# johncai117/Meta-Fine-Tuning

Measured on AMD Instinct MI355X. Metric: episodes/sec at 5-way N-shot (ResNet10+GNN) per GPU and 1/2/4/8-GPU node, higher is better.
Workload: dtype f32

## Files before the change

include/mft_hip.h:

```cpp
#ifndef MFT_HIP_H
#define MFT_HIP_H

#ifdef __cplusplus
extern "C" {
#endif

#define MFT_EINVAL (-22)

enum { MFT_ACT_NONE = 0, MFT_ACT_RELU = 1, MFT_ACT_LRELU = 2 };
enum { MFT_BN_AFFINE_FMA = 0x100 };

int mft_version(void);
int mft_device_info(int* cu_count, int* gcn_arch_is_gfx950);

int mft_stream_create_cumask(const unsigned* mask_words, int n_words, void** stream_out);
int mft_stream_create_priority(int priority, void** stream_out, int* range_out);
int mft_stream_destroy(void* stream);
int mft_stream_probe(float* w, float* m, float* v, long long n, void* stream);
int mft_event_create(void** event_out);
int mft_event_record(void* event, void* stream);
int mft_event_elapsed_ms(void* start, void* stop, float* ms_out);
int mft_event_destroy(void* event);
int mft_probe_placement(unsigned* out, int n_blocks, int spin_cycles, void* stream);

int mft_augment_views(const unsigned char* src, int n_img, int Hs, int Ws, const float* params, int n_views, float* out,
                      long long view_stride, long long img_stride, int size, const float* mean3, const float* std3,
                      void* stream);

int mft_nchw_to_nhwc(const float* src, float* dst, int n_img, int C, int H, int W, void* stream);

long long mft_conv2d_wgrad_adam_dgrad_ws_floats(int n_img, int H, int W, int Cin);
int mft_conv2d_wgrad_adam_dgrad_nhwc(const float* x, int ldx, const float* dy, int ldy, float* w, float* m, float* v,
                                     float* dx_partials, int n_img, int H, int W, int Cin, int Cout, int imgs_per_group,
                                     long long group_stride, int step, float lr, float beta1, float beta2, float eps, void* stream);
int mft_conv2d_wgrad_adam_dgrad_nhwc_dev(const float* x, int ldx, const float* dy, int ldy, float* w, float* m, float* v,
                                         float* dx_partials, int n_img, int H, int W, int Cin, int Cout, int imgs_per_group,
                                         long long group_stride, const float* hyper, float beta1, float beta2, float eps,
                                         void* stream);
int mft_col2im_bn_backward_small(const float* dx_partials, const float* x_raw, const float* relu_out, float* dx, int n_img, int H,
                                 int W, int C, int imgs_per_group, const float* mean, const float* rstd, const float* gamma,
                                 long long gb_group_stride, float* dgamma, float* dbeta, void* stream);

int mft_ce_pool_bn_backward2(const float* feat, const int* labels, int imgs_per_group, int n_groups, int C, int hw,
                             const float* out, const float* xa, const float* xb, float* dxa, float* dxb, const float* mean_a,
                             const float* rstd_a, const float* gamma_a, const float* mean_b, const float* rstd_b,
                             const float* gamma_b, long long gb_group_stride, float* dgamma_a, float* dbeta_a, float* dgamma_b,
                             float* dbeta_b, float* loss, void* stream);

int mft_stem_cache_fill(const float* in, const float* w, int w_ld, int n_img, int H, int W, float* pmax, float* pmin,
                        float* mean_img, float* m2_img, void* stream);
int mft_pool_window_minmax(const float* x, float* ymax, float* ymin, long long n_img, int H, int W, int C, void* stream);
int mft_bn_relu_pooled_gather(const float* pmax, const float* pmin, const int* src_idx, float* y, int n_img, int OH, int OW, int C,
                              int imgs_per_group, const float* mean, const float* rstd, const float* gamma, const float* beta,
                              void* stream);

int mft_bn_apply_planes(const float* x, int ldx, float* y, int ldy, unsigned short* planes, long long plane_stride, int C,
                        int rows_per_group, int n_groups, const float* mean, const float* rstd, const float* gamma,
                        const float* beta, long long gb_group_stride, const float* res, int ldr, const float* res_mean,
                        const float* res_rstd, const float* res_gamma, const float* res_beta, int act, float slope,
                        void* stream);
int mft_bn_relu_maxpool_gather_planes(const float* x, const int* src_idx, float* y, unsigned short* planes,
                                      long long plane_stride, int n_img, int H, int W, int C, int imgs_per_group,
                                      const float* mean, const float* rstd, const float* gamma, const float* beta, void* stream);
int mft_conv2d_nhwc_x3p_bnstats(const unsigned short* in_planes, long long in_plane_elems, int ldi, const unsigned short* w3,
                                long long plane_elems, float* out, int ldo, int n_img, int H, int W, int Cin, int Cout, int KH,
                                int KW, int stride, int pad, int imgs_per_group, float eps, float* stats_ws, float* mean,
                                float* rstd, void* stream);

int mft_ingest_episode_views(const float* const* views, int n_views, int double_first, int n_way, int per_class, int n_support,
                             int C, int H, int W, float* support_store, float* all_store, void* stream);
int mft_pack_oihw(const float* w_oihw, float* w_pk, int Cout, int Cin, int KH, int KW, int k_pad, void* stream);
int mft_pack_oihw_multi(const void* jobs, int n_jobs, long long total_elements, void* stream);
int mft_unpack_oihw(const float* w_pk, float* w_oihw, int Cout, int Cin, int KH, int KW, int k_pad, void* stream);
int mft_pack_dgrad(const float* w_pk, float* wt_pk, int Cout, int Cin, int KH, int KW,
                   int groups, long long w_stride, long long wt_stride, void* stream);

int mft_conv2d_nhwc(const float* in, int ldi, const float* w, const float* bias, float* out, int ldo,
                    int n_img, int H, int W, int Cin, int Cout, int KH, int KW, int stride, int pad,
                    int imgs_per_group, long long w_group_stride, void* stream);

int mft_split_bf16x3(const float* w, unsigned short* planes, long long n, void* stream);
int mft_split_bf16x3_multi(const void* jobs, int n_jobs, long long total_elements, void* stream);
int mft_conv2d_nhwc_x3(const float* in, int ldi, const unsigned short* w3, long long plane_elems, float* out, int ldo,
                       int n_img, int H, int W, int Cin, int Cout, int KH, int KW, int stride, int pad, void* stream);
long long mft_conv2d_x3_stats_ws_floats(int n_img, int H, int W, int Cout, int KH, int KW, int stride, int pad);
int mft_conv2d_nhwc_x3_bnstats(const float* in, int ldi, const unsigned short* w3, long long plane_elems, float* out, int ldo,
                               int n_img, int H, int W, int Cin, int Cout, int KH, int KW, int stride, int pad,
                               int imgs_per_group, float eps, float* stats_ws, float* mean, float* rstd, void* stream);
int mft_conv2d_nhwc_x3_bnin_bnstats(const float* in, int ldi, const float* in_ws, const float* in_gamma, const float* in_beta,
                                    const unsigned short* w3, long long plane_elems, float* out, int ldo, int n_img, int H, int W,
                                    int Cin, int Cout, int imgs_per_group, float eps, float* stats_ws, float* mean, float* rstd,
                                    void* stream);
int mft_split_f16x2(const float* w, unsigned short* planes, long long n, void* stream);
int mft_conv2d_nhwc_h2(const float* in, int ldi, const unsigned short* w2, long long plane_elems, float* out, int ldo,
                       int n_img, int H, int W, int Cin, int Cout, int KH, int KW, int stride, int pad, void* stream);
int mft_conv2d_nhwc_h2_bnstats(const float* in, int ldi, const unsigned short* w2, long long plane_elems, float* out, int ldo,
                               int n_img, int H, int W, int Cin, int Cout, int KH, int KW, int stride, int pad,
                               int imgs_per_group, float eps, float* stats_ws, float* mean, float* rstd, void* stream);
int mft_conv2d_nhwc_h2_bnin_bnstats(const float* in, int ldi, const float* in_ws, const float* in_gamma, const float* in_beta,
                                    const unsigned short* w2, long long plane_elems, float* out, int ldo, int n_img, int H, int W,
                                    int Cin, int Cout, int imgs_per_group, float eps, float* stats_ws, float* mean, float* rstd,
                                    void* stream);
int mft_bn_apply_x3ws(const float* x, int ldx, float* y, int ldy, int C, int rows_per_group, int n_groups, const float* ws,
                      const float* gamma, const float* beta, const float* res, int ldr, const float* res_ws,
                      const float* res_gamma, const float* res_beta, int act, float slope, float eps, float* mean, float* rstd,
                      float* res_mean, float* res_rstd, void* stream);
int mft_bn_running_ema(const float* mean_a, const float* rstd_a, int rows_a, const float* mean_b, const float* rstd_b, int rows_b,
                       const int* order, int n_steps, int C, float eps, float momentum, float* running_mean, float* running_var,
                       void* stream);
int mft_bn_apply_x3ws_fits(int C, int rows_per_group, int with_res_bn);
int mft_bn_relu_pooled_gather_moments(const float* pmax, const float* pmin, const int* src_idx, float* y, int n_img, int OH, int OW,
                                      int C, int imgs_per_group, const float* mean_img, const float* m2_img, int rows_per_img,
                                      float eps, const float* gamma, const float* beta, float* mean, float* rstd, void* stream);

int mft_has_experiments(void);

int mft_conv2d_dgrad_nhwc(const float* dy, int ldy, const float* w, float* dx, int ldx,
                          int n_img, int H, int W, int Cin, int Cout, int KH, int KW, int stride, int pad,
                          int imgs_per_group, long long w_group_stride, void* stream);

long long mft_conv_ksplit_ws_floats(long long rows, int cols, int K);
long long mft_conv_ksplit_grouped_ws_floats(long long rows_per_group, int cols, int K, int groups);
int mft_conv2d_nhwc_ksplit_grouped(const float* in, int ldi, const float* w, float* out, int ldo, int n_img, int H, int W, int Cin,
                                   int Cout, int KH, int KW, int stride, int pad, int imgs_per_group, long long w_group_stride,
                                   float* ws, void* stream);
int mft_conv2d_dgrad_nhwc_ksplit_grouped(const float* dy, int ldy, const float* w, float* dx, int ldx, int n_img, int H, int W, int Cin,
                                         int Cout, int KH, int KW, int stride, int pad, int imgs_per_group, long long w_group_stride,
                                         float* ws, void* stream);
int mft_conv2d_nhwc_ksplit(const float* in, int ldi, const float* w, const float* bias, float* out, int ldo, int n_img, int H, int W,
                           int Cin, int Cout, int KH, int KW, int stride, int pad, float* ws, void* stream);
int mft_conv2d_dgrad_nhwc_ksplit(const float* dy, int ldy, const float* w, float* dx, int ldx, int n_img, int H, int W, int Cin,
                                 int Cout, int KH, int KW, int stride, int pad, float* ws, void* stream);
long long mft_conv2d_wgrad_ws_floats(int n_img, int H, int W, int Cin, int Cout, int KH, int KW, int stride, int pad,
                                     int imgs_per_group);
int mft_conv2d_wgrad_nhwc(const float* in, int ldi, const float* dy, int ldy, float* dw,
                          int n_img, int H, int W, int Cin, int Cout, int KH, int KW, int stride, int pad,
                          int imgs_per_group, long long dw_group_stride, float* ws, void* stream);

long long mft_conv2d_wgrad_oihw_ws_floats(int n_img, int H, int W, int Cin, int Cout, int KH, int KW, int stride, int pad);
int mft_conv2d_wgrad_oihw(const float* in, int ldi, const float* dy, int ldy, float* dw_oihw, int n_img, int H, int W, int Cin,
                          int Cout, int KH, int KW, int stride, int pad, int cin_valid, int cout_valid, float* ws, void* stream);

typedef struct MftWgradJob {
    const float* in; const float* dy; float* dw_oihw; float* ws;
    int ldi, ldy, n_img, H, W, Cin, Cout, KH, KW, stride, pad, cin_valid, cout_valid, reserved;
} MftWgradJob;
int mft_conv2d_wgrad_oihw_multi(const MftWgradJob* jobs, int n_jobs, void* stream);

int mft_conv2d_wgrad_adam_nhwc(const float* in, int ldi, const float* dy, int ldy, float* w, float* m, float* v,
                               float* dw_or_null, int n_img, int H, int W, int Cin, int Cout, int KH, int KW,
                               int stride, int pad, int imgs_per_group, long long group_stride,
                               int step, float lr, float beta1, float beta2, float eps, void* stream);

int mft_wgrad_adam_next_forward(const float* x, int ldx, const float* dy, int ldy, float* w, float* m, float* v,
                                float* dw_or_null, int n_img, int H, int W, int Cin, int Cout, int KH, int KW, int stride,
                                int pad, int imgs_per_group, long long group_stride, int step, const float* hyper, float lr,
                                float beta1, float beta2, float eps, const float* x_next, int mode, float* raw, float* act,
                                const float* gamma, const float* beta, long long gb_group_stride, float* mean, float* rstd,
                                const float* sc_raw, const float* gamma_s, const float* beta_s, float* mean_s, float* rstd_s,
                                float* pooled, float bn_eps, void* stream);


long long mft_bn_stats_ws_floats(int C, int rows_per_group, int n_groups);
int mft_bn_stats(const float* x, int ldx, int C, int rows_per_group, int n_groups, float eps,
                 float* mean, float* rstd, float* ws,
                 float* running_mean, float* running_var, float momentum, long long* num_batches_tracked, void* stream);
typedef struct MftBnStatsJob {
    const float* x; float* mean; float* rstd; float* ws; float* running_mean; float* running_var; long long* num_batches_tracked;
    int ldx, C, rows_per_group, n_groups; float eps, momentum;
} MftBnStatsJob;
int mft_bn_stats_multi(const MftBnStatsJob* jobs, int n_jobs, void* stream);
typedef struct MftBnFwdJob {
    const float* x; float* y; const float* gamma; const float* beta; float* mean; float* rstd;
    float* running_mean; float* running_var; long long* num_batches_tracked;
    const float* res; const float* res_gamma; const float* res_beta; float* res_mean; float* res_rstd;
    float* res_running_mean; float* res_running_var; long long* res_num_batches_tracked;
    int ldx, ldy, ldr, C, rows_per_group, n_groups, act; float eps, momentum, slope;
} MftBnFwdJob;
int mft_bn_forward_small(const MftBnFwdJob* job, void* stream);
int mft_bn_forward_small_max_rows(void);
typedef struct MftBnApplyJob {
    const float* x; float* y; const float* mean; const float* rstd; const float* gamma; const float* beta;
    int ldx, ldy, C, rows_per_group, n_groups, act; float slope; int reserved;
} MftBnApplyJob;
int mft_bn_apply_multi(const MftBnApplyJob* jobs, int n_jobs, void* stream);
// ... 175 lines not shown
```

meta-fine-tuning_amd/_lib.py:

```python
import ctypes
import os

PKG = os.path.dirname(os.path.abspath(__file__))
LIB_PATH = os.path.join(PKG, "libmft_hip.so")

_P = ctypes.c_void_p
_I = ctypes.c_int
_L = ctypes.c_longlong
_F = ctypes.c_float

SIGNATURES = {
    "mft_version": [],
    "mft_device_info": [_P, _P],
    "mft_stream_create_cumask": [_P, _I, _P],
    "mft_stream_destroy": [_P],
    "mft_stream_probe": [_P, _P, _P, _L, _P],
    "mft_probe_placement": [_P, _I, _I, _P],
    "mft_event_create": [_P],
    "mft_event_record": [_P, _P],
    "mft_event_elapsed_ms": [_P, _P, _P],
    "mft_event_destroy": [_P],
    "mft_augment_views": [_P, _I, _I, _I, _P, _I, _P, _L, _L, _I, _P, _P, _P],
    "mft_nchw_to_nhwc": [_P, _P, _I, _I, _I, _I, _P],
    "mft_pack_oihw": [_P, _P, _I, _I, _I, _I, _I, _P],
    "mft_unpack_oihw": [_P, _P, _I, _I, _I, _I, _I, _P],
    "mft_pack_dgrad": [_P, _P, _I, _I, _I, _I, _I, _L, _L, _P],
    "mft_conv2d_nhwc": [_P, _I, _P, _P, _P, _I, _I, _I, _I, _I, _I, _I, _I, _I, _I, _I, _L, _P],
    "mft_has_experiments": [],
    "mft_split_bf16x3": [_P, _P, _L, _P],
    "mft_split_bf16x3_multi": [_P, _I, _L, _P],
    "mft_conv2d_nhwc_x3": [_P, _I, _P, _L, _P, _I, _I, _I, _I, _I, _I, _I, _I, _I, _I, _P],
    "mft_conv2d_x3_stats_ws_floats": [_I, _I, _I, _I, _I, _I, _I, _I],
    "mft_conv2d_nhwc_x3_bnstats": [_P, _I, _P, _L, _P, _I, _I, _I, _I, _I, _I, _I, _I, _I, _I, _I, _F, _P, _P, _P, _P],
    "mft_conv2d_dgrad_nhwc": [_P, _I, _P, _P, _I, _I, _I, _I, _I, _I, _I, _I, _I, _I, _I, _L, _P],
    "mft_conv_ksplit_ws_floats": [_L, _I, _I],
    "mft_conv_ksplit_grouped_ws_floats": [_L, _I, _I, _I],
    "mft_conv2d_nhwc_ksplit_grouped": [_P, _I, _P, _P, _I, _I, _I, _I, _I, _I, _I, _I, _I, _I, _I, _L, _P, _P],
    "mft_conv2d_dgrad_nhwc_ksplit_grouped": [_P, _I, _P, _P, _I, _I, _I, _I, _I, _I, _I, _I, _I, _I, _I, _L, _P, _P],
    "mft_conv2d_nhwc_ksplit": [_P, _I, _P, _P, _P, _I, _I, _I, _I, _I, _I, _I, _I, _I, _I, _P, _P],
    "mft_conv2d_dgrad_nhwc_ksplit": [_P, _I, _P, _P, _I, _I, _I, _I, _I, _I, _I, _I, _I, _I, _P, _P],
    "mft_conv2d_wgrad_oihw_ws_floats": [_I, _I, _I, _I, _I, _I, _I, _I, _I],
    "mft_conv2d_wgrad_oihw": [_P, _I, _P, _I, _P, _I, _I, _I, _I, _I, _I, _I, _I, _I, _I, _I, _P, _P],
    "mft_conv2d_wgrad_oihw_multi": [_P, _I, _P],
    "mft_conv2d_wgrad_ws_floats": [_I, _I, _I, _I, _I, _I, _I, _I, _I, _I],
    "mft_conv2d_wgrad_nhwc": [_P, _I, _P, _I, _P, _I, _I, _I, _I, _I, _I, _I, _I, _I, _I, _L, _P, _P],
    "mft_conv2d_wgrad_adam_nhwc": [_P, _I, _P, _I, _P, _P, _P, _P, _I, _I, _I, _I, _I, _I, _I, _I, _I, _I, _L, _I, _F, _F, _F,
                                   _F, _P],
    "mft_pair_softmax_ut_backward": [_P, _P, _P, _P, _P, _I, _I, _I, _P, _P],
    "mft_pair_bwd_stats_ws_floats": [_L, _I],
    "mft_pair_bn_act_backward": [_P, _I, _P, _I, _P, _P, _P, _P, _P, _P, _I, _L, _I, _L, _F, _P, _P, _P, _P, _P, _P],
    "mft_pair_absdiff_ut": [_P, _I, _P, _P, _I, _I, _I, _L, _L, _P],
    "mft_pair_dx_gather": [_P, _I, _P, _I, _P, _I, _I, _I, _I, _L, _L, _P],
    "mft_pack_oihw_multi": [_P, _I, _L, _P],
    "mft_wgrad_adam_next_forward": [_P, _I, _P, _I, _P, _P, _P, _P, _I, _I, _I, _I, _I, _I, _I, _I, _I, _I, _L, _I, _P, _F, _F, _F,
                                    _F, _P, _I, _P, _P, _P, _P, _L, _P, _P, _P, _P, _P, _P, _P, _P, _F, _P],
    "mft_bn_stats_ws_floats": [_I, _I, _I],
    "mft_bn_stats": [_P, _I, _I, _I, _I, _F, _P, _P, _P, _P, _P, _F, _P, _P],
    "mft_bn_apply": [_P, _I, _P, _I, _I, _I, _I, _P, _P, _P, _P, _L, _P, _I, _P, _P, _P, _P, _I, _F, _P],
    "mft_bn_apply_multi": [_P, _I, _P],
    "mft_bn_stats_multi": [_P, _I, _P],
    "mft_bn_relu_maxpool": [_P, _P, _I, _I, _I, _I, _I, _P, _P, _P, _P, _P],
    "mft_bn_relu_maxpool_gather": [_P, _P, _P, _I, _I, _I, _I, _I, _P, _P, _P, _P, _P],
    "mft_bn_image_moments": [_P, _I, _I, _I, _L, _P, _P, _P],
    "mft_bn_combine_moments": [_P, _P, _P, _I, _I, _I, _I, _F, _P, _P, _P],
    "mft_global_avgpool": [_P, _P, _I, _I, _I, _P],
    "mft_bn_small_forward": [_P, _I, _P, _I, _P, _I, _P, _I, _I, _I, _I, _P, _P, _P, _P, _L, _P, _P, _P, _P, _I, _F, _F, _P, _I, _P],
    "mft_bn_backward2": [_P, _P, _I, _P, _I, _P, _P, _I, _I, _I, _I, _P, _P, _P, _P, _P, _P, _L, _P, _P, _P, _P, _P],
    "mft_ce_pool_backward": [_P, _P, _I, _I, _I, _I, _P, _P, _P, _P],
    "mft_bn_backward": [_P, _I, _P, _I, _P, _I, _P, _I, _I, _I, _I, _P, _P, _P, _L, _P, _P, _P],
    "mft_avgpool_relu_backward": [_P, _P, _P, _I, _I, _I, _P],
    "mft_cross_entropy": [_P, _I, _P, _I, _I, _I, _P, _P, _P],
    "mft_softmax_rows": [_P, _I, _P, _I, _I, _I, _P],
    "mft_proto_scores": [_P, _I, _I, _I, _I, _I, _I, _P, _I, _P],
    "mft_proto_backward": [_P, _I, _I, _I, _I, _I, _I, _P, _I, _P, _I, _P],
    "mft_cross_entropy_mean": [_P, _I, _P, _I, _I, _I, _P, _P, _P],
    "mft_cross_entropy_mean_backward": [_P, _I, _P, _I, _I, _I, _P, _P, _I, _P],
    "mft_adam_step": [_P, _P, _P, _P, _L, _I, _F, _F, _F, _F, _F, _P],
    "mft_sgd_step": [_P, _P, _P, _L, _I, _F, _F, _F, _F, _P],
    "mft_maml_delta": [_P, _P, _P, _L, _P],
    "mft_conv2d_wgrad_adam_dgrad_ws_floats": [_I, _I, _I, _I],
    "mft_conv2d_wgrad_adam_dgrad_nhwc": [_P, _I, _P, _I, _P, _P, _P, _P, _I, _I, _I, _I, _I, _I, _L, _I, _F, _F, _F, _F, _P],
    "mft_conv2d_wgrad_adam_dgrad_nhwc_dev": [_P, _I, _P, _I, _P, _P, _P, _P, _I, _I, _I, _I, _I, _I, _L, _P, _F, _F, _F, _P],
    "mft_col2im_bn_backward_small": [_P, _P, _P, _P, _I, _I, _I, _I, _I, _P, _P, _P, _L, _P, _P, _P],
    "mft_stream_create_priority": [_I, _P, _P],
    "mft_ce_pool_bn_backward2": [_P, _P, _I, _I, _I, _I, _P, _P, _P, _P, _P, _P, _P, _P, _P, _P, _P, _L, _P, _P, _P, _P, _P, _P],
    "mft_pool_window_minmax": [_P, _P, _P, _L, _I, _I, _I, _P],
    "mft_stem_cache_fill": [_P, _P, _I, _I, _I, _I, _P, _P, _P, _P, _P],
    "mft_conv2d_nhwc_x3_bnin_bnstats": [_P, _I, _P, _P, _P, _P, _L, _P, _I, _I, _I, _I, _I, _I, _I, _F, _P, _P, _P, _P],
    "mft_split_f16x2": [_P, _P, _L, _P],
    "mft_conv2d_nhwc_h2": [_P, _I, _P, _L, _P, _I, _I, _I, _I, _I, _I, _I, _I, _I, _I, _P],
    "mft_conv2d_nhwc_h2_bnstats": [_P, _I, _P, _L, _P, _I, _I, _I, _I, _I, _I, _I, _I, _I, _I, _I, _F, _P, _P, _P, _P],
    "mft_conv2d_nhwc_h2_bnin_bnstats": [_P, _I, _P, _P, _P, _P, _L, _P, _I, _I, _I, _I, _I, _I, _I, _F, _P, _P, _P, _P],
    "mft_bn_apply_x3ws": [_P, _I, _P, _I, _I, _I, _I, _P, _P, _P, _P, _I, _P, _P, _P, _I, _F, _F, _P, _P, _P, _P, _P],
    "mft_bn_apply_x3ws_fits": [_I, _I, _I],
    "mft_bn_running_ema": [_P, _P, _I, _P, _P, _I, _P, _I, _I, _F, _F, _P, _P, _P],
    "mft_bn_relu_pooled_gather_moments": [_P, _P, _P, _P, _I, _I, _I, _I, _I, _P, _P, _I, _F, _P, _P, _P, _P, _P],
    "mft_bn_relu_pooled_gather": [_P, _P, _P, _P, _I, _I, _I, _I, _I, _P, _P, _P, _P, _P],
    "mft_bn_apply_planes": [_P, _I, _P, _I, _P, _L, _I, _I, _I, _P, _P, _P, _P, _L, _P, _I, _P, _P, _P, _P, _I, _F, _P],
    "mft_bn_relu_maxpool_gather_planes": [_P, _P, _P, _P, _L, _I, _I, _I, _I, _I, _P, _P, _P, _P, _P],
    "mft_conv2d_nhwc_x3p_bnstats": [_P, _L, _I, _P, _L, _P, _I, _I, _I, _I, _I, _I, _I, _I, _I, _I, _I, _F, _P, _P, _P, _P],
    "mft_ingest_episode_views": [_P, _I, _I, _I, _I, _I, _I, _I, _I, _P, _P, _P],
    "mft_block_entry_small_forward": [_P, _I, _P, _L, _P, _L, _P, _P, _P, _I, _I, _I, _I, _I, _I, _I, _P, _P, _L, _P, _P, _F, _P],
    "mft_block_exit_small_forward": [_P, _P, _L, _P, _P, _P, _P, _I, _I, _I, _I, _I, _P, _P, _P, _P, _L, _P, _P, _P, _P, _F, _P],
    "mft_conv2d_dgrad_bn_backward_small": [_P, _I, _P, _P, _I, _I, _I, _I, _I, _I, _I, _I, _I, _I, _L, _P, _P, _P, _P, _P, _L,
                                           _P, _P, _P],
    "mft_linear_head_sgd_run": [_P, _P, _P, _I, _I, _I, _I, _I, _I, _P, _P, _F, _F, _F, _F, _P],
    "mft_linear_head_adam_run": [_P, _P, _P, _I, _I, _I, _I, _I, _I, _P, _P, _F, _F, _F, _F, _F, _P],
    "mft_adam_multi": [_P, _I, _I, _F, _F, _F, _F, _F, _F, _P],
    "mft_adam_hyper_advance": [_P, _P, _F, _F, _F, _P],
    "mft_adam_step_dev": [_P, _P, _P, _P, _L, _P, _F, _F, _F, _F, _P],
    "mft_conv2d_wgrad_adam_nhwc_dev": [_P, _I, _P, _I, _P, _P, _P, _P, _I, _I, _I, _I, _I, _I, _I, _I, _I, _I, _L, _P, _F, _F,
                                       _F, _P],
    "mft_linear_head_step": [_P, _I, _P, _I, _I, _I, _I, _P, _P, _P, _P, _P, _P, _P, _I, _P, _I, _F, _F, _F, _F, _F, _P],
    "mft_linear_head_scores": [_P, _I, _I, _I, _I, _I, _P, _P, _P, _P],
    "mft_pair_absdiff": [_P, _I, _P, _I, _I, _I, _I, _P],
    "mft_masked_softmax": [_P, _I, _P, _I, _I, _P],
    "mft_pair_mlp_tiles_m": [_I, _I],
    "mft_pair_mlp_layer": [_P, _I, _I, _P, _P, _P, _P, _I, _I, _P, _P, _I, _I, _I, _I, _F, _P, _P, _P, _I, _P],
    "mft_bn_forward_small": [_P, _P],
    "mft_bn_forward_small_max_rows": [],
    "mft_gemm_rk": [_P, _I, _P, _I, _I, _P, _P, _I, _I, _I, _P],
    "mft_pair_mlp_tiles_m_rk": [_I, _I],
    "mft_pair_mlp_layer_rk": [_P, _I, _I, _P, _P, _P, _P, _I, _I, _P, _P, _I, _I, _I, _I, _F, _P, _P, _P, _P],
    "mft_pair_mlp_stats_finalize_rk": [_P, _P, _P, _I, _I, _I, _P, _P, _F, _P, _P, _P, _P, _P],
    "mft_pair_mlp_stats_finalize": [_P, _P, _P, _I, _I, _I, _P, _P, _F, _P, _P, _P, _P, _P],
    "mft_pair_mlp_score": [_P, _I, _P, _P, _P, _P, _F, _P, _I, _I, _I, _P],
    "mft_masked_softmax_ut": [_P, _P, _I, _I, _P],
    "mft_graph_aggregate": [_P, _P, _I, _P, _I, _I, _I, _I, _P],
    "mft_copy_cols": [_P, _I, _P, _I, _I, _I, _I, _I, _F, _P],
    "mft_build_graph_nodes": [_P, _I, _P, _I, _I, _I, _I, _I, _I, _P],
    "mft_gather_query_scores": [_P, _I, _P, _I, _I, _I, _I, _P],
    "mft_gather_rows": [_P, _P, _P, _I, _L, _P],
    "mft_var_to_rstd": [_P, _P, _I, _F, _P],
    "mft_bn_backward_ws_floats": [_I, _I, _I],
    "mft_bn_backward_act": [_P, _I, _P, _I, _P, _I, _P, _I, _I, _I, _I, _P, _P, _P, _L, _P, _P, _I, _F, _P, _P, _P, _P, _P],
    "mft_bn_backward_act_multi": [_P, _I, _P],
    "mft_act_backward": [_P, _I, _P, _I, _P, _I, _I, _L, _I, _F, _I, _P],
    "mft_colsum": [_P, _I, _I, _L, _P, _P, _P],
    "mft_bn_relu_maxpool_arg": [_P, _P, _P, _I, _I, _I, _I, _I, _P, _P, _P, _P, _P],
    "mft_maxpool_relu_backward": [_P, _P, _P, _P, _I, _I, _I, _I, _P],
    "mft_masked_softmax_backward": [_P, _P, _P, _I, _I, _I, _P],
    "mft_pair_absdiff_backward": [_P, _I, _P, _I, _P, _I, _I, _I, _I, _P],
    "mft_graph_aggregate_backward": [_P, _P, _I, _P, _I, _P, _I, _P, _I, _I, _I, _I, _P],
    "mft_build_graph_nodes_backward": [_P, _I, _P, _I, _I, _I, _I, _I, _I, _P],
    "mft_gather_query_scores_backward": [_P, _P, _I, _I, _I, _I, _I, _P, _P],
}
TESTING_SIGNATURES = {
    "mft_debug_set_conv_tile": [_I],
    "mft_debug_set_x3_tile": [_I],
    "mft_debug_reset": [],
    "mft_wgrad_fwd_set_exact": [_I],
    "mft_wgrad_fwd_set_xcd": [_I],
}
_RESTYPE = {"mft_conv2d_x3_stats_ws_floats": _L, "mft_bn_stats_ws_floats": _L, "mft_conv2d_wgrad_ws_floats": _L, "mft_bn_backward_ws_floats": _L,
            "mft_conv2d_wgrad_adam_dgrad_ws_floats": _L, "mft_pair_bwd_stats_ws_floats": _L, "mft_conv_ksplit_ws_floats": _L, "mft_conv2d_wgrad_oihw_ws_floats": _L, "mft_conv_ksplit_grouped_ws_floats": _L}

_lib = None


def lib():
    global _lib
    if _lib is None:
        if not os.path.exists(LIB_PATH):
            raise RuntimeError(
                "libmft_hip.so not found at %s -- build it with `python -c 'import __graft_entry__ as g; g.build()'`; "
                "this package has no CPU or PyTorch fallback" % LIB_PATH)
        import torch
        if torch.cuda.is_available():
            torch.cuda.init()
            torch.empty(1, device="cuda")
        h = ctypes.CDLL(LIB_PATH)
        for name, argtypes in list(SIGNATURES.items()) + list(TESTING_SIGNATURES.items()):
            fn = getattr(h, name)
# ... 87 lines not shown
```

meta-fine-tuning_amd/csrc/bn.hip:

```cpp
#include "mft_common.h"
#include "bn_fold.h"

namespace {

constexpr int ST_ROWS = 16;

__device__ __forceinline__ void bn_stats_partial_body(const float* __restrict__ x, int ldx, int C,
                                                      int rows_per_group, int rows_per_chunk, int chunks,
                                                      float* __restrict__ ws, const int bx, const int by, const int bz) {
    const int cq = threadIdx.x & 15;
    const int rl = threadIdx.x >> 4;
    const int c = by * 64 + cq * 4;
    const int g = bz;
    const int chunk = bx;
    const long long row0 = (long long)g * rows_per_group;
    __shared__ f32x4 red1[ST_ROWS][16];
    __shared__ f32x4 red2[ST_ROWS][16];
    f32x4 s1 = {0.f, 0.f, 0.f, 0.f}, s2 = {0.f, 0.f, 0.f, 0.f};
    if (c < C) {
        const f32x4 sh = *(const f32x4*)(x + row0 * ldx + c);
        const int rbeg = chunk * rows_per_chunk;
        const int rend = min(rbeg + rows_per_chunk, rows_per_group);
#pragma unroll 4
        for (int rr = rbeg + rl; rr < rend; rr += ST_ROWS) {
// ... 369 lines not shown
            if (p.ro) {
                const f32x4 o = *(const f32x4*)(p.ro + (row0 + rr) * p.ldro + c);
#pragma unroll
                for (int e = 0; e < 4; ++e) d[e] = o[e] > 0.f ? d[e] : 0.f;
            }
            const f32x4 xh = (*(const f32x4*)(p.x + (row0 + rr) * p.ldx + c) - mu) * rs;
            s1 += d;
            s2 += d * xh;
        }
    }
    red1[rl][cq] = s1;
    red2[rl][cq] = s2;
    __syncthreads();
    s1 = red1[0][cq];
    s2 = red2[0][cq];
#pragma unroll
    for (int k = 1; k < ST_ROWS; ++k) {
        s1 += red1[k][cq];
        s2 += red2[k][cq];
    }
    if (!ok) return;
    if (rl == 0) {
        if (p.dgamma) *(f32x4*)(p.dgamma + (long long)g * p.C + c) = s2;
        if (p.dbeta) *(f32x4*)(p.dbeta + (long long)g * p.C + c) = s1;
    }
    if (!p.dx) return;
    const float inv = 1.f / (float)p.rows_per_group;
    const f32x4 m1 = s1 * inv, m2 = s2 * inv;
    const f32x4 k = ga * rs;
    for (int rr = rl; rr < p.rows_per_group; rr += ST_ROWS) {
        f32x4 d = *(const f32x4*)(p.dy + (row0 + rr) * p.lddy + c);
        if (p.ro) {
            const f32x4 o = *(const f32x4*)(p.ro + (row0 + rr) * p.ldro + c);
#pragma unroll
            for (int e = 0; e < 4; ++e) d[e] = o[e] > 0.f ? d[e] : 0.f;
        }
        const f32x4 xh = (*(const f32x4*)(p.x + (row0 + rr) * p.ldx + c) - mu) * rs;
        *(f32x4*)(p.dx + (row0 + rr) * p.lddx + c) = k * (d - m1 - xh * m2);
    }
}

__global__ __launch_bounds__(256) void bn_image_moments_kernel(const float* __restrict__ x, int ldx, int C, int rows,
                                                               float* __restrict__ mean_img,
                                                               float* __restrict__ m2_img) {
    const int cq = threadIdx.x & 15;
    const int rl = threadIdx.x >> 4;
    const int c = blockIdx.y * 64 + cq * 4;
    const long long img = blockIdx.x;
    const long long row0 = img * rows;
    __shared__ f32x4 red1[ST_ROWS][16];
    __shared__ f32x4 red2[ST_ROWS][16];
    f32x4 s1 = {0.f, 0.f, 0.f, 0.f}, s2 = {0.f, 0.f, 0.f, 0.f}, sh = s1;
    if (c < C) {
        sh = *(const f32x4*)(x + row0 * ldx + c);
        for (int rr = rl; rr < rows; rr += ST_ROWS) {
            f32x4 v = *(const f32x4*)(x + (row0 + rr) * ldx + c);
            v -= sh;
            s1 += v;
            s2 += v * v;
        }
    }
    red1[rl][cq] = s1;
    red2[rl][cq] = s2;
    __syncthreads();
    if (rl == 0 && c < C) {
#pragma unroll
        for (int k = 1; k < ST_ROWS; ++k) {
            s1 += red1[k][cq];
            s2 += red2[k][cq];
        }
        const float inv = 1.f / (float)rows;
        f32x4 mu, m2;
#pragma unroll
        for (int e = 0; e < 4; ++e) {
            const float d = s1[e] * inv;
            mu[e] = sh[e] + d;
            m2[e] = fmaxf(s2[e] - s1[e] * d, 0.f);
        }
        *(f32x4*)(mean_img + img * C + c) = mu;
        *(f32x4*)(m2_img + img * C + c) = m2;
    }
}

template <class MeanOf, class M2Of>
__device__ __forceinline__ void combine_moments_impl(MeanOf mean_of, M2Of m2_of, int rows_per_img, int imgs_per_group, float eps,
                                                     float& mean, float& rstd) {
    float mu = 0.f;
    for (int i = 0; i < imgs_per_group; ++i) mu += mean_of(i);
    mu /= (float)imgs_per_group;
    float m2 = 0.f, dev = 0.f;
    for (int i = 0; i < imgs_per_group; ++i) {
        const float d = mean_of(i) - mu;
        m2 += m2_of(i);
        dev += d * d;
    }
    const float var = (m2 + (float)rows_per_img * dev) / ((float)rows_per_img * (float)imgs_per_group);
    mean = mu;
    rstd = 1.0f / sqrtf(var + eps);
}

__device__ __forceinline__ void combine_moments(const float* __restrict__ mean_img, const float* __restrict__ m2_img,
                                                const int* __restrict__ id, int C, int c, int rows_per_img, int imgs_per_group,
                                                float eps, float& mean, float& rstd) {
    combine_moments_impl([&](int i) { return mean_img[(long long)id[i] * C + c]; },
                         [&](int i) { return m2_img[(long long)id[i] * C + c]; }, rows_per_img, imgs_per_group, eps, mean, rstd);
}

__device__ __forceinline__ void combine_moments_lds(const float* smean, const float* sm2, int C, int c, int rows_per_img,
                                                    int imgs_per_group, float eps, float& mean, float& rstd) {
    combine_moments_impl([&](int i) { return smean[i * C + c]; }, [&](int i) { return sm2[i * C + c]; }, rows_per_img,
                         imgs_per_group, eps, mean, rstd);
}

__global__ void bn_combine_moments_kernel(const float* __restrict__ mean_img, const float* __restrict__ m2_img,
                                          const int* __restrict__ idx, int C, int rows_per_img, int imgs_per_group,
                                          float eps, float* __restrict__ mean, float* __restrict__ rstd) {
    const int c = blockIdx.x * blockDim.x + threadIdx.x;
    const int g = blockIdx.y;
    if (c >= C) return;
    float mu, rs;
    combine_moments(mean_img, m2_img, idx + (long long)g * imgs_per_group, C, c, rows_per_img, imgs_per_group, eps, mu, rs);
    mean[(long long)g * C + c] = mu;
    rstd[(long long)g * C + c] = rs;
}

inline int grid_for(long long total, int block = 256, int cap = 256 * 8) {
    long long b = (total + block - 1) / block;
    if (b < 1) b = 1;
    if (b > cap) b = cap;
    return (int)b;
}

inline int stats_chunks(int rows_per_group, int n_groups, int C) {
    const int tiles = (C + 63) / 64;
    long long want = (1024 + (long long)n_groups * tiles - 1) / ((long long)n_groups * tiles);
    int maxc = (rows_per_group + 63) / 64;
    if (want > maxc) want = maxc;
    if (want < 1) want = 1;
    return (int)want;
}

struct BnFwdSmallArgs {
    const float* x; float* y; const float* gamma; const float* beta; float* mean; float* rstd;
    float* running_mean; float* running_var; long long* nbt;
    const float* res; const float* rgamma; const float* rbeta; float* rmean; float* rrstd;
    float* rrunning_mean; float* rrunning_var; long long* rnbt;
    int ldx, ldy, ldr, C, rows_per_group, n_groups, act;
    float eps, momentum, slope;
    int y_scalar;
};

__device__ __forceinline__ void bn_small_block_sum(f32x4& a, f32x4& b, float (*red)[8]) {
    const int lane = threadIdx.x & 63, wave = threadIdx.x >> 6;
#pragma unroll
    for (int off = 32; off > 0; off >>= 1)
#pragma unroll
        for (int e = 0; e < 4; ++e) {
            a[e] += __shfl_xor(a[e], off, 64);
            b[e] += __shfl_xor(b[e], off, 64);
        }
    if (lane == 0) {
#pragma unroll
        for (int e = 0; e < 4; ++e) { red[wave][e] = a[e]; red[wave][4 + e] = b[e]; }
    }
    __syncthreads();
#pragma unroll
    for (int e = 0; e < 4; ++e) {
        a[e] = ((red[0][e] + red[1][e]) + red[2][e]) + red[3][e];
        b[e] = ((red[0][4 + e] + red[1][4 + e]) + red[2][4 + e]) + red[3][4 + e];
    }
}

__device__ __forceinline__ void bn_small_finish(const f32x4 s1, const f32x4 s2, const f32x4 pivot, int rows, float eps, f32x4& mu,
                                                f32x4& rs, f32x4& var) {
    const float inv = 1.f / (float)rows;
#pragma unroll
    for (int e = 0; e < 4; ++e) {
        const float d = s1[e] * inv;
        mu[e] = pivot[e] + d;
        var[e] = fmaxf(s2[e] * inv - d * d, 0.f);
        rs[e] = 1.0f / sqrtf(var[e] + eps);
    }
}

__global__ __launch_bounds__(256) void bn_forward_small_kernel(BnFwdSmallArgs p) {
    __shared__ float red[2][4][8];
    const int c = blockIdx.x * 4, g = blockIdx.y, t = threadIdx.x;
    const long long row0 = (long long)g * p.rows_per_group;
    const bool rbn = p.res != nullptr && p.rgamma != nullptr;
    const f32x4 zero4 = {0.f, 0.f, 0.f, 0.f};
    const f32x4 pv = *(const f32x4*)(p.x + row0 * p.ldx + c);
    const f32x4 pr = rbn ? *(const f32x4*)(p.res + row0 * p.ldr + c) : zero4;
    f32x4 s1 = zero4, s2 = zero4, q1 = zero4, q2 = zero4;
    if (rbn) {
// ... 199 lines not shown
                                      const int* __restrict__ order, int n_steps, int C, float eps, float momentum,
                                      float* __restrict__ running_mean, float* __restrict__ running_var) {
    const int c = blockIdx.x * blockDim.x + threadIdx.x;
    if (c >= C) return;
    float rm = running_mean[c], rv = running_var[c];
    for (int t = 0; t < n_steps; ++t) {
        const int o = order[t], g = o & 0xffffff;
        const bool b = (o >> 24) != 0;
        const float m = (b ? mean_b : mean_a)[(long long)g * C + c];
        const float rs = (b ? rstd_b : rstd_a)[(long long)g * C + c];
        const float var = fmaxf(1.0f / (rs * rs) - eps, 0.f);
        rm = (1.f - momentum) * rm + momentum * m;
        rv = (1.f - momentum) * rv + momentum * (var * (b ? unb_b : unb_a));
    }
    running_mean[c] = rm;
    running_var[c] = rv;
}
}

extern "C" int mft_bn_running_ema(const float* mean_a, const float* rstd_a, int rows_a, const float* mean_b, const float* rstd_b,
                                  int rows_b, const int* order, int n_steps, int C, float eps, float momentum, float* running_mean,
                                  float* running_var, void* stream) {
    if (!mean_a || !rstd_a || rows_a < 1 || !order || n_steps < 1 || C < 1 || !running_mean || !running_var) return MFT_EINVAL;
    const float ua = (float)rows_a / (float)(rows_a > 1 ? rows_a - 1 : 1);
    const float ub = (float)rows_b / (float)(rows_b > 1 ? rows_b - 1 : 1);
    hipLaunchKernelGGL(bn_running_ema_kernel, dim3((C + 63) / 64), dim3(64), 0, (hipStream_t)stream, mean_a, rstd_a, ua, mean_b, rstd_b, ub,
                       order, n_steps, C, eps, momentum, running_mean, running_var);
    return mft_launch_status();
}

extern "C" int mft_bn_apply_x3ws_fits(int C, int rows_per_group, int with_res_bn) {
    if (C % 4 != 0 || C > 1024 || rows_per_group < 128) return 0;
    return (size_t)4 * C * sizeof(float) + (with_res_bn ? 2 : 1) * mft_x3_stage_bytes_host(mft_x3_max_group_tiles(rows_per_group, 128), C) <=
           64 * 1024;
}

extern "C" int mft_bn_apply_planes(const float* x, int ldx, float* y, int ldy, unsigned short* planes, long long plane_stride,
                                   int C, int rows_per_group, int n_groups, const float* mean, const float* rstd,
                                   const float* gamma, const float* beta, long long gb_group_stride, const float* res, int ldr,
                                   const float* res_mean, const float* res_rstd, const float* res_gamma,
                                   const float* res_beta, int act, float slope, void* stream) {
    if (C % 4 != 0 || ldx % 4 != 0 || (y && ldy % 4 != 0) || (res && ldr % 4 != 0) || !planes) return MFT_EINVAL;
    if (plane_stride < (long long)n_groups * rows_per_group * C) return MFT_EINVAL;
    ApplyArgs p{x, y, ldx, ldy, C, rows_per_group, n_groups, mean, rstd, gamma, beta, gb_group_stride,
                res, ldr, res_mean, res_rstd, res_gamma, res_beta, act, slope, planes, plane_stride};
    const long long total = (long long)n_groups * rows_per_group * (C / 4);
    hipLaunchKernelGGL(bn_apply_kernel<true>, dim3(grid_for(total)), dim3(256), 0, (hipStream_t)stream, p);
    return mft_launch_status();
}

namespace {
__global__ __launch_bounds__(256) void pool_window_minmax_kernel(const float* __restrict__ x, float* __restrict__ ymax,
                                                                 float* __restrict__ ymin, long long n_img, int H, int W, int C,
                                                                 int OH, int OW) {
    const int cq = C >> 2;
    const long long total = n_img * OH * OW * cq;
    for (long long i = (long long)blockIdx.x * blockDim.x + threadIdx.x; i < total; i += (long long)gridDim.x * blockDim.x) {
        const int c = (int)(i % cq) * 4;
        long long t = i / cq;
        const int ow = (int)(t % OW); t /= OW;
        const int oh = (int)(t % OH);
        const long long n = t / OH;
        f32x4 hi = {-3.4e38f, -3.4e38f, -3.4e38f, -3.4e38f}, lo = {3.4e38f, 3.4e38f, 3.4e38f, 3.4e38f};
#pragma unroll
        for (int dh = 0; dh < 3; ++dh) {
            const int ih = oh * 2 - 1 + dh;
            if (ih < 0 || ih >= H) continue;
#pragma unroll
            for (int dw = 0; dw < 3; ++dw) {
                const int iw = ow * 2 - 1 + dw;
                if (iw < 0 || iw >= W) continue;
                const f32x4 v = *(const f32x4*)(x + ((n * H + ih) * W + iw) * C + c);
#pragma unroll
                for (int e = 0; e < 4; ++e) { hi[e] = fmaxf(hi[e], v[e]); lo[e] = fminf(lo[e], v[e]); }
            }
        }
        *(f32x4*)(ymax + i * 4) = hi;
        *(f32x4*)(ymin + i * 4) = lo;
    }
}

__device__ __forceinline__ f32x4 pooled_bn_relu(const float* __restrict__ pmax, const float* __restrict__ pmin, long long src,
                                                const f32x4 mu, const f32x4 rs, const f32x4 ga, const f32x4 be) {
    const bool all_pos = ga[0] >= 0.f && ga[1] >= 0.f && ga[2] >= 0.f && ga[3] >= 0.f;
    const bool all_neg = ga[0] < 0.f && ga[1] < 0.f && ga[2] < 0.f && ga[3] < 0.f;
    f32x4 v;
    if (all_pos) v = *(const f32x4*)(pmax + src);
    else if (all_neg) v = *(const f32x4*)(pmin + src);
    else {
        const f32x4 a = *(const f32x4*)(pmax + src), b = *(const f32x4*)(pmin + src);
#pragma unroll
        for (int e = 0; e < 4; ++e) v[e] = ga[e] >= 0.f ? a[e] : b[e];
    }
    f32x4 o = __builtin_elementwise_fma((v - mu) * rs, ga, be);
#pragma unroll
    for (int e = 0; e < 4; ++e) o[e] = fmaxf(o[e], 0.f);
    return o;
}

__global__ __launch_bounds__(256) void bn_relu_pooled_gather_kernel(const float* __restrict__ pmax, const float* __restrict__ pmin,
                                                                    const int* __restrict__ src_idx, float* __restrict__ y,
                                                                    int n_img, int HW, int C, int imgs_per_group,
                                                                    const float* __restrict__ mean, const float* __restrict__ rstd,
                                                                    const float* __restrict__ gamma, const float* __restrict__ beta) {
    const int cq = C >> 2;
    const long long total = (long long)n_img * HW * cq;
    for (long long i = (long long)blockIdx.x * blockDim.x + threadIdx.x; i < total; i += (long long)gridDim.x * blockDim.x) {
        const int c = (int)(i % cq) * 4;
        const long long t = i / cq;
        const int pix = (int)(t % HW);
        const int n = (int)(t / HW);
        const int g = n / imgs_per_group;
        const long long src = ((long long)src_idx[n] * HW + pix) * C + c;
        const f32x4 mu = *(const f32x4*)(mean + (long long)g * C + c);
        const f32x4 rs = *(const f32x4*)(rstd + (long long)g * C + c);
        *(f32x4*)(y + i * 4) = pooled_bn_relu(pmax, pmin, src, mu, rs, *(const f32x4*)(gamma + c), *(const f32x4*)(beta + c));
    }
}

__global__ __launch_bounds__(256) void bn_relu_pooled_gather_moments_kernel(
    const float* __restrict__ pmax, const float* __restrict__ pmin, const int* __restrict__ src_idx, float* __restrict__ y, int HW,
    int C, int imgs_per_group, const float* __restrict__ mean_img, const float* __restrict__ m2_img, int rows_per_img, float eps,
    const float* __restrict__ gamma, const float* __restrict__ beta, float* __restrict__ mean, float* __restrict__ rstd) {
    extern __shared__ __attribute__((aligned(16))) float tab[];
    const int g = blockIdx.y;
    const int* id = src_idx + (long long)g * imgs_per_group;
    float* smean = tab + 2 * C;
    float* sm2 = smean + imgs_per_group * C;
    for (int i = threadIdx.x; i < imgs_per_group * C; i += 256) {
        const int im = i / C, c = i - im * C;
        const long long src = (long long)id[im] * C + c;
        smean[i] = mean_img[src];
        sm2[i] = m2_img[src];
    }
    __syncthreads();
    for (int c = threadIdx.x; c < C; c += 256) {
        float mu, rs;
        combine_moments_lds(smean, sm2, C, c, rows_per_img, imgs_per_group, eps, mu, rs);
        tab[c] = mu; tab[C + c] = rs;
        if (blockIdx.x == 0 && mean) { mean[(long long)g * C + c] = mu; rstd[(long long)g * C + c] = rs; }
    }
    __syncthreads();
    const int cq = C >> 2;
    const int total = imgs_per_group * HW * cq;
    for (int i = blockIdx.x * 256 + threadIdx.x; i < total; i += gridDim.x * 256) {
        const int c = (i % cq) * 4;
        const int t = i / cq;
        const int pix = t % HW;
        const int n = t / HW;
        const long long src = ((long long)id[n] * HW + pix) * C + c;
        const long long dst = ((long long)g * imgs_per_group * HW * cq + i) * 4;
        *(f32x4*)(y + dst) = pooled_bn_relu(pmax, pmin, src, *(const f32x4*)(tab + c), *(const f32x4*)(tab + C + c),
                                            *(const f32x4*)(gamma + c), *(const f32x4*)(beta + c));
    }
}
}

extern "C" int mft_pool_window_minmax(const float* x, float* ymax, float* ymin, long long n_img, int H, int W, int C, void* stream) {
    if (C % 4 != 0 || n_img <= 0) return MFT_EINVAL;
    const int OH = (H + 2 - 3) / 2 + 1, OW = (W + 2 - 3) / 2 + 1;
    const long long total = n_img * OH * OW * (C / 4);
    hipLaunchKernelGGL(pool_window_minmax_kernel, dim3(grid_for(total, 256, 256 * 16)), dim3(256), 0, (hipStream_t)stream, x, ymax,
                       ymin, n_img, H, W, C, OH, OW);
    return mft_launch_status();
}

extern "C" int mft_bn_relu_pooled_gather(const float* pmax, const float* pmin, const int* src_idx, float* y, int n_img, int OH,
                                         int OW, int C, int imgs_per_group, const float* mean, const float* rstd,
                                         const float* gamma, const float* beta, void* stream) {
    if (C % 4 != 0 || !src_idx) return MFT_EINVAL;
    if (imgs_per_group <= 0) imgs_per_group = n_img;
    const long long total = (long long)n_img * OH * OW * (C / 4);
    hipLaunchKernelGGL(bn_relu_pooled_gather_kernel, dim3(grid_for(total, 256, 256 * 16)), dim3(256), 0, (hipStream_t)stream, pmax,
                       pmin, src_idx, y, n_img, OH * OW, C, imgs_per_group, mean, rstd, gamma, beta);
    return mft_launch_status();
}

extern "C" int mft_bn_relu_pooled_gather_moments(const float* pmax, const float* pmin, const int* src_idx, float* y, int n_img,
                                                 int OH, int OW, int C, int imgs_per_group, const float* mean_img,
                                                 const float* m2_img, int rows_per_img, float eps, const float* gamma,
                                                 const float* beta, float* mean, float* rstd, void* stream) {
    if (C % 4 != 0 || C > 1024 || !src_idx || imgs_per_group <= 0 || n_img % imgs_per_group != 0 || rows_per_img <= 0 ||
        (mean == nullptr) != (rstd == nullptr))
        return MFT_EINVAL;
    const int groups = n_img / imgs_per_group;
    const long long per_group = (long long)imgs_per_group * OH * OW * (C / 4);
    if (per_group > 0x7fffffffLL) return MFT_EINVAL;
    int sub = (int)((per_group + 256 * 16 - 1) / (256 * 16));
    const int cap = (2048 + groups - 1) / groups;
    if (sub > cap) sub = cap;
    if (sub < 1) sub = 1;
    const size_t lds = (size_t)(2 + 2 * imgs_per_group) * C * sizeof(float);
    if (lds > 64 * 1024) return MFT_EINVAL;
    hipLaunchKernelGGL(bn_relu_pooled_gather_moments_kernel, dim3(sub, groups), dim3(256), lds, (hipStream_t)stream,
                       pmax, pmin, src_idx, y, OH * OW, C, imgs_per_group, mean_img, m2_img, rows_per_img, eps, gamma, beta, mean,
                       rstd);
    return mft_launch_status();
}

extern "C" int mft_bn_relu_maxpool_gather_planes(const float* x, const int* src_idx, float* y, unsigned short* planes,
                                                 long long plane_stride, int n_img, int H, int W, int C, int imgs_per_group,
                                                 const float* mean, const float* rstd, const float* gamma, const float* beta,
                                                 void* stream) {
    if (C % 4 != 0) return MFT_EINVAL;
    if (imgs_per_group <= 0) imgs_per_group = n_img;
    const int OH = (H + 2 - 3) / 2 + 1, OW = (W + 2 - 3) / 2 + 1;
    const long long total = (long long)n_img * OH * OW * (C / 4);
    if (planes)
        hipLaunchKernelGGL(bn_relu_maxpool_kernel<true>, dim3(grid_for(total, 256, 256 * 16)), dim3(256), 0, (hipStream_t)stream,
                           x, y, n_img, H, W, C, OH, OW, imgs_per_group, mean, rstd, gamma, beta, src_idx, planes, plane_stride);
    else
        hipLaunchKernelGGL(bn_relu_maxpool_kernel<false>, dim3(grid_for(total, 256, 256 * 16)), dim3(256), 0, (hipStream_t)stream,
                           x, y, n_img, H, W, C, OH, OW, imgs_per_group, mean, rstd, gamma, beta, src_idx, planes, plane_stride);
    return mft_launch_status();
}

extern "C" int mft_bn_relu_maxpool_gather(const float* x, const int* src_idx, float* y, int n_img, int H, int W, int C,
                                          int imgs_per_group, const float* mean, const float* rstd, const float* gamma,
                                          const float* beta, void* stream) {
    return mft_bn_relu_maxpool_gather_planes(x, src_idx, y, nullptr, 0, n_img, H, W, C, imgs_per_group, mean, rstd, gamma, beta,
                                             stream);
// ... 347 lines not shown
```

meta-fine-tuning_amd/csrc/bn_fold.h:

```cpp
#pragma once
#include "mft_common.h"

typedef float mft_f32x2 __attribute__((ext_vector_type(2)));

struct MftTileSpan { int t0, t1; };
struct MftTileW { float inv_nt, w1, w2, pad; };

__device__ __forceinline__ MftTileSpan mft_x3_group_tiles(int g, int M, int R, int BM) {
    const int r0 = g * R, r1 = min(r0 + R, M);
    return {r0 / BM, (r1 - 1) / BM};
}

__device__ __forceinline__ int mft_x3_tile_seg(int t, int g, int R, int BM) { return ((t * BM) / R == g) ? 0 : 1; }

__device__ __forceinline__ MftTileW mft_x3_tile_weights(int t, int g, int M, int R, int BM) {
    const int r0 = g * R, r1 = min(r0 + R, M);
    const int lo = max(t * BM, r0), hi = min(t * BM + BM, r1);
    const float nt = (float)(hi - lo), n = (float)(lo - r0), tot = (float)(hi - r0);
    return {1.0f / nt, nt / tot, n * nt / tot, 0.f};
}

template <class Get, class Weights>
__device__ __forceinline__ void mft_x3_stats_chain(Get get, Weights weights, int g, int M, int R, int BM, float eps, float& mean,
                                                   float& rstd) {
    const int r0 = g * R, r1 = min(r0 + R, M);
    const MftTileSpan sp = mft_x3_group_tiles(g, M, R, BM);
    float mu = 0.f, m2 = 0.f;
    for (int t = sp.t0; t <= sp.t1; ++t) {
        const MftTileW w = weights(t);
        const mft_f32x2 o = get(t, mft_x3_tile_seg(t, g, R, BM));
        const float mt = o[0] * w.inv_nt;
        const float m2t = fmaxf(__builtin_fmaf(-o[0], mt, o[1]), 0.f);
        const float d = mt - mu;
        m2 += __builtin_fmaf(d * d, w.w2, m2t);
        mu = __builtin_fmaf(d, w.w1, mu);
    }
    mean = mu;
    rstd = 1.0f / sqrtf(m2 / (float)(r1 - r0) + eps);
}

__device__ __forceinline__ void mft_x3_stats_merge(const float* __restrict__ ws, int C, int c, int g, int M, int R, int BM,
                                                   float eps, float& mean, float& rstd) {
    mft_x3_stats_chain([&](int t, int seg) { return *(const mft_f32x2*)(ws + (((long long)t * 2 + seg) * C + c) * 2); },
                       [&](int t) { return mft_x3_tile_weights(t, g, M, R, BM); }, g, M, R, BM, eps, mean, rstd);
}

__device__ __forceinline__ size_t mft_x3_stage_bytes(int max_tiles, int C) {
    return (size_t)max_tiles * (sizeof(MftTileW) + (size_t)C * sizeof(mft_f32x2));
}

__device__ __forceinline__ void mft_x3_stats_stage(const float* __restrict__ ws, int C, int g, int M, int R, int BM, int max_tiles,
                                                   void* stage, int tid, int nthreads) {
    MftTileW* wt = reinterpret_cast<MftTileW*>(stage);
    mft_f32x2* part = reinterpret_cast<mft_f32x2*>(wt + max_tiles);
    const MftTileSpan sp = mft_x3_group_tiles(g, M, R, BM);
    const int nt = sp.t1 - sp.t0 + 1;
    for (int i = tid; i < nt; i += nthreads) wt[i] = mft_x3_tile_weights(sp.t0 + i, g, M, R, BM);
    const int total = nt * C;
    for (int i = tid; i < total; i += nthreads) {
        const int tt = i / C, c = i - tt * C, t = sp.t0 + tt;
        part[i] = *(const mft_f32x2*)(ws + (((long long)t * 2 + mft_x3_tile_seg(t, g, R, BM)) * C + c) * 2);
    }
}

__device__ __forceinline__ void mft_x3_stats_staged(const void* stage, int max_tiles, int C, int c, int g, int M, int R, int BM,
                                                    float eps, float& mean, float& rstd) {
    const MftTileW* wt = reinterpret_cast<const MftTileW*>(stage);
    const mft_f32x2* part = reinterpret_cast<const mft_f32x2*>(wt + max_tiles);
    const int t0 = mft_x3_group_tiles(g, M, R, BM).t0;
    mft_x3_stats_chain([&](int t, int) { return part[(t - t0) * C + c]; }, [&](int t) { return wt[t - t0]; }, g, M, R, BM, eps, mean,
                       rstd);
}

inline int mft_x3_max_group_tiles(int R, int BM) { return (R + BM - 1) / BM + 1; }
inline size_t mft_x3_stage_bytes_host(int max_tiles, int C) { return (size_t)max_tiles * (16 + (size_t)C * 8); }

__device__ __forceinline__ void mft_bn_fold(float mean, float rstd, float gamma, float beta, float& scale, float& shift) {
    scale = rstd * gamma;
    shift = __builtin_fmaf(-mean, scale, beta);
}

__device__ __forceinline__ f32x4 mft_bn_affine4(const f32x4 v, const f32x4 scale, const f32x4 shift) {
    return __builtin_elementwise_fma(v, scale, shift);
}

__device__ __forceinline__ void mft_bn_fold4(const f32x4 mean, const f32x4 rstd, const f32x4 gamma, const f32x4 beta, f32x4& scale,
                                             f32x4& shift) {
    scale = rstd * gamma;
    shift = __builtin_elementwise_fma(-mean, scale, beta);
}
```

meta-fine-tuning_amd/csrc/conv_x3.hip:

```cpp
#include "mft_common.h"
#include "bn_fold.h"

namespace {

typedef __bf16 bf16x8 __attribute__((ext_vector_type(8)));
typedef __bf16 bf16x2 __attribute__((ext_vector_type(2)));
typedef _Float16 f16x8 __attribute__((ext_vector_type(8)));
typedef _Float16 f16x4 __attribute__((ext_vector_type(4)));
typedef float f32x2 __attribute__((ext_vector_type(2)));
typedef unsigned u32x2 __attribute__((ext_vector_type(2)));
typedef unsigned u32x4 __attribute__((ext_vector_type(4)));

struct X3Args {
    const float* in;
    const unsigned short* w3;
    long long plane;
    float* out;
    int ldi, ldo;
    int H, W, Cin, OH, OW, Cout, KH, KW, stride, pad;
    int Kpad;
    int M;
    int tiles_n;
    unsigned in_bytes, w_bytes;
    int xcd_swizzle;
    int row_swz;
    const unsigned short* in3;
    unsigned in_plane_bytes;
    float* stats_ws;
    int rows_per_group;
    int s1_rows;
    const float* bn_ws; const float* bn_gamma; const float* bn_beta;
    float bn_eps;
    int bn_max_tiles;
};

constexpr int X3_RS = 40;

__device__ __forceinline__ unsigned pk_bf16(float a, float b) {
    f32x2 v = {a, b};
    return __builtin_bit_cast(unsigned, __builtin_convertvector(v, bf16x2));
}

__device__ __forceinline__ void split4(const f32x4 x, u32x2& p1, u32x2& p2, u32x2& p3) {
    f32x4 r;
    p1[0] = pk_bf16(x[0], x[1]);
    p1[1] = pk_bf16(x[2], x[3]);
    r[0] = x[0] - __builtin_bit_cast(float, p1[0] << 16);
    r[1] = x[1] - __builtin_bit_cast(float, p1[0] & 0xffff0000u);
    r[2] = x[2] - __builtin_bit_cast(float, p1[1] << 16);
    r[3] = x[3] - __builtin_bit_cast(float, p1[1] & 0xffff0000u);
    p2[0] = pk_bf16(r[0], r[1]);
    p2[1] = pk_bf16(r[2], r[3]);
    r[0] -= __builtin_bit_cast(float, p2[0] << 16);
    r[1] -= __builtin_bit_cast(float, p2[0] & 0xffff0000u);
    r[2] -= __builtin_bit_cast(float, p2[1] << 16);
    r[3] -= __builtin_bit_cast(float, p2[1] & 0xffff0000u);
    p3[0] = pk_bf16(r[0], r[1]);
    p3[1] = pk_bf16(r[2], r[3]);
}

__device__ __forceinline__ void split4_h2(const f32x4 x, u32x2& p1, u32x2& p2) {
    const f16x4 hi = __builtin_convertvector(x, f16x4);
    const f32x4 r = (x - __builtin_convertvector(hi, f32x4)) * 2048.f;
    const f16x4 lo = __builtin_convertvector(r, f16x4);
    p1 = __builtin_bit_cast(u32x2, hi);
    p2 = __builtin_bit_cast(u32x2, lo);
}
constexpr float X3_H2_LO_SCALE = 1.0f / 2048.f;

template <int BM, int BN, bool AP, bool DB, int HOIST = 0, int DBG = 0, bool XS = false, int NP = 3>
__global__ __launch_bounds__(256) __attribute__((amdgpu_waves_per_eu(NP == 2 ? 3 : 1))) void conv_x3_kernel(X3Args p) {
    static_assert(NP == 3 || (NP == 2 && !AP && !DB && HOIST == 0 && DBG == 0 && !XS), "f16x2: the plain single-buffer form only");
    constexpr int NACC = NP == 3 ? 1 : 2;
    constexpr int TM = BM / 64;
    constexpr int TN = BN / 64;
    constexpr int PA = AP ? BM / 64 : BM / 32;
    constexpr int PB = BN / 64;
    constexpr int RS = XS ? 32 : X3_RS;
    constexpr int A_PLANE = BM * RS;
    constexpr int B_PLANE = BN * RS;
    auto lo = [](int row, int c) -> int {
        if constexpr (XS) return row * 32 + ((((c >> 3) ^ (row >> 2)) & 3) << 3) + (c & 7);
        else return row * X3_RS + c;
    };
    extern __shared__ __attribute__((aligned(16))) unsigned short smem[];
    unsigned short* As = smem;
    unsigned short* Bs = smem + NP * A_PLANE;
    constexpr int BUF = NP * (A_PLANE + B_PLANE);

    const int tid = threadIdx.x;
    const int lane = tid & 63, wave = tid >> 6;
    const int wm = wave >> 1, wn = wave & 1;
    const int r = lane & 31, h = lane >> 5;
    const bool g_swz = !XS && p.row_swz != 0;
    int tile_id = blockIdx.x;
    if (p.xcd_swizzle) {
        const int nwg = gridDim.x, q = nwg >> 3, rmd = nwg & 7;
        const int xcd = tile_id & 7, slot = tile_id >> 3;
        tile_id = xcd * q + (xcd < rmd ? xcd : rmd) + slot;
    }
    const int nt = tile_id % p.tiles_n;
    const int mt = tile_id / p.tiles_n;
    const int m0 = mt * BM, n0 = nt * BN;

    const int g_id = AP ? tid >> 4 : tid >> 5;
    const int g_rr = AP ? (tid >> 2) & 3 : (tid >> 3) & 3;
    const int lrow = g_swz ? g_rr * 4 + (g_id & 3) + 16 * (g_id >> 2) : (AP ? tid >> 2 : tid >> 3);
    const int c4 = AP ? (tid & 3) * 8 : (tid & 7) * 4;
    constexpr int RPP = AP ? 64 : 32;
    constexpr int ESZ = AP ? 2 : 4;
    const int ohw = p.OH * p.OW;
    const __amdgpu_buffer_rsrc_t rA = AP ? __builtin_amdgcn_make_buffer_rsrc((void*)p.in3, 0, 3 * p.in_plane_bytes, 0x00020000)
                                         : __builtin_amdgcn_make_buffer_rsrc((void*)p.in, 0, p.in_bytes, 0x00020000);
    const __amdgpu_buffer_rsrc_t rB = __builtin_amdgcn_make_buffer_rsrc((void*)p.w3, 0, p.w_bytes, 0x00020000);
    int a_off[PA];
    int a_ih0[PA], a_iw0[PA];
    bool a_ok[PA];
#pragma unroll
    for (int j = 0; j < PA; ++j) {
        const int m = m0 + lrow + RPP * j;
        a_ok[j] = m < p.M;
        const int mm = a_ok[j] ? m : 0;
        const int img = mm / ohw;
        const int rem = mm - img * ohw;
        const int oh = rem / p.OW, ow = rem - oh * p.OW;
        a_ih0[j] = oh * p.stride - p.pad;
        a_iw0[j] = ow * p.stride - p.pad;
        a_off[j] = (((img * p.H + a_ih0[j]) * p.W + a_iw0[j]) * p.ldi + c4) * ESZ;
    }
    const int bseg = tid & 3;
    const int brow = g_swz ? ((tid >> 2) & 3) * 4 + ((tid >> 4) & 3) + 16 * (tid >> 6) : tid >> 2;
    int b_off[PB];
#pragma unroll
    for (int j = 0; j < PB; ++j) b_off[j] = ((n0 + brow + 64 * j) * p.Kpad + bseg * 8) * 2;
    const int plane_bytes = (int)(p.plane * 2);

    f32x16 accs[NACC][TM][TN];
#pragma unroll
    for (int q = 0; q < NACC; ++q)
#pragma unroll
        for (int i = 0; i < TM; ++i)
#pragma unroll
            for (int j = 0; j < TN; ++j)
#pragma unroll
                for (int e = 0; e < 16; ++e) accs[q][i][j][e] = 0.f;
    auto& acc = accs[0];
    auto val = [&](int i, int j, int e) -> float {
        if constexpr (NP == 3) return accs[0][i][j][e];
        else return __builtin_fmaf(accs[NACC - 1][i][j][e], X3_H2_LO_SCALE, accs[0][i][j][e]);
    };

    struct Stage {
        f32x4 ra[AP ? 1 : PA];
        u32x4 ra3[AP ? PA : 1][3];
        u32x4 rb[PB][NP];
    };
    Stage st0;
    const int nk = p.Kpad / 32;

    int t_kt = 0, t_ci0 = 0, t_kh = 0, t_kw = 0;
    auto load_tile = [&](int kt, Stage& S) {
        const int k0 = kt * 32;
        while (t_kt < kt) {
            ++t_kt;
            t_ci0 += 32;
            if (t_ci0 == p.Cin) { t_ci0 = 0; if (++t_kw == p.KW) { t_kw = 0; ++t_kh; } }
        }
        const int ci0 = t_ci0, kh = t_kh, kw = t_kw;
        const int tap_off = ((kh * p.W + kw) * p.ldi + ci0) * ESZ;
#pragma unroll
        for (int j = 0; j < PA; ++j) {
            const bool ok = a_ok[j] && (unsigned)(a_ih0[j] + kh) < (unsigned)p.H && (unsigned)(a_iw0[j] + kw) < (unsigned)p.W;
            const unsigned voff = ok ? (unsigned)(a_off[j] + tap_off) : 0x80000000u;
            if constexpr (AP) {
#pragma unroll
                for (int pl = 0; pl < 3; ++pl)
                    S.ra3[j][pl] = __builtin_amdgcn_raw_buffer_load_b128(rA, voff, pl * (int)p.in_plane_bytes, 0);
            } else {
                S.ra[j] = __builtin_bit_cast(f32x4, __builtin_amdgcn_raw_buffer_load_b128(rA, voff, 0, 0));
            }
// ... 167 lines not shown
            mm(1);
            __builtin_amdgcn_sched_barrier(0);
        }
    };
    if constexpr (DB) {
        load_tile(0, st0);
        store_tile(st0, 0);
        __syncthreads();
        load_tile(nk > 1 ? 1 : 0, st0);
        for (int kt = 0; kt + 1 < nk; ++kt) {
            compute(kt & 1);
            store_tile(st0, (kt + 1) & 1);
            load_tile(kt + 2 < nk ? kt + 2 : nk - 1, st0);
            __syncthreads();
        }
        compute((nk - 1) & 1);
    } else {
        load_tile(0, st0);
        store_tile(st0, 0);
        __syncthreads();
        for (int kt = 0; kt < nk; ++kt) {
            if constexpr (!(DBG & 4)) { if (kt + 1 < nk) load_tile(kt + 1, st0); }
            if constexpr (!(DBG & 16)) compute(0);
            if constexpr (!(DBG & 32)) __syncthreads();
            if constexpr (!(DBG & 8)) { if (kt + 1 < nk) store_tile(st0, 0); }
            if constexpr (!(DBG & 32)) __syncthreads();
        }
    }

#pragma unroll
    for (int i = 0; i < TM; ++i)
#pragma unroll
        for (int j = 0; j < TN; ++j) {
            const int n = n0 + wn * (BN / 2) + j * 32 + r;
#pragma unroll
            for (int e = 0; e < 16; ++e) {
                const int row = (e & 3) + 8 * (e >> 2) + 4 * h;
                const int m = m0 + wm * (BM / 2) + i * 32 + row;
                if (m < p.M) p.out[(long long)m * p.ldo + n] = val(i, j, e);
            }
        }
    if (p.stats_ws != nullptr) {
        static_assert(TN == 1 || TN == 2, "stats epilogue");
        const int split = (m0 / p.rows_per_group + 1) * p.rows_per_group;
        float* sred = reinterpret_cast<float*>(smem);
        __syncthreads();
#pragma unroll
        for (int j = 0; j < TN; ++j) {
            float a1 = 0.f, a2 = 0.f, b1 = 0.f, b2 = 0.f;
#pragma unroll
            for (int i = 0; i < TM; ++i)
#pragma unroll
                for (int e = 0; e < 16; ++e) {
                    const int m = m0 + wm * (BM / 2) + i * 32 + (e & 3) + 8 * (e >> 2) + 4 * h;
                    const float v = val(i, j, e);
                    if (m < p.M) {
                        if (m < split) { a1 += v; a2 += v * v; }
                        else { b1 += v; b2 += v * v; }
                    }
                }
            a1 += __shfl_xor(a1, 32, 64); a2 += __shfl_xor(a2, 32, 64);
            b1 += __shfl_xor(b1, 32, 64); b2 += __shfl_xor(b2, 32, 64);
            if (h == 0) {
                float* o = sred + ((((wm * 2 + wn) * TN + j) * 32 + r) << 2);
                o[0] = a1; o[1] = a2; o[2] = b1; o[3] = b2;
            }
        }
        __syncthreads();
        if (wm == 0 && h == 0) {
#pragma unroll
            for (int j = 0; j < TN; ++j) {
                const float* o0 = sred + ((((0 * 2 + wn) * TN + j) * 32 + r) << 2);
                const float* o1 = sred + ((((1 * 2 + wn) * TN + j) * 32 + r) << 2);
                const int n = n0 + wn * (BN / 2) + j * 32 + r;
                float* w0 = p.stats_ws + (((long long)mt * 2 + 0) * p.Cout + n) * 2;
                float* w1 = p.stats_ws + (((long long)mt * 2 + 1) * p.Cout + n) * 2;
                w0[0] = o0[0] + o1[0]; w0[1] = o0[1] + o1[1];
                w1[0] = o0[2] + o1[2]; w1[1] = o0[3] + o1[3];
            }
        }
    }
}

#ifdef MFT_EXPERIMENTS
#include "../../tools/experiments/conv_x3_pingpong.inc"
#endif

template <int BM, int BN, bool BNIN, int NP = 3, bool BDB = true>
__device__ __forceinline__ void conv_x3_s1_body(const X3Args& p) {
    static_assert(NP == 3 || NP == 2, "3 bf16 pieces (six products) or 2 fp16 pieces (three products)");
    constexpr int NACC = NP == 3 ? 1 : 2;
    constexpr int TM = BM / 64, TN = BN / 64;
    constexpr int PA = BM / 32, PB = BN / 64;
    constexpr int RS = X3_RS;
    constexpr int B_PLANE = BN * RS;
    const int A_PLANE = p.s1_rows * RS;
    extern __shared__ __attribute__((aligned(16))) unsigned short smem[];
    constexpr int NBB = (NP == 2 && BDB) ? 2 : 1;
    unsigned short* As = smem;
    unsigned short* Bs = smem + NP * A_PLANE;
    float* bn_tab = reinterpret_cast<float*>(Bs + NBB * NP * B_PLANE);

    const int tid = threadIdx.x;
    const int lane = tid & 63, wave = tid >> 6;
    const int wm = wave >> 1, wn = wave & 1;
    const int r = lane & 31, h = lane >> 5;
    int tile_id = blockIdx.x;
    if (p.xcd_swizzle) {
        const int nwg = gridDim.x, q = nwg >> 3, rmd = nwg & 7;
        const int xcd = tile_id & 7, slot = tile_id >> 3;
        tile_id = xcd * q + (xcd < rmd ? xcd : rmd) + slot;
    }
    const int nt = tile_id % p.tiles_n;
    const int mt = tile_id / p.tiles_n;
    const int m0 = mt * BM, n0 = nt * BN;
    const int W = p.W, H = p.H;
    const int fr0 = m0 / W;
    const int g0 = BNIN ? m0 / p.rows_per_group : 0;
    const bool bn_two = BNIN && (m0 + (BM < p.M - m0 ? BM : p.M - m0) - 1) / p.rows_per_group > g0;
    if constexpr (BNIN) {
        char* stage = reinterpret_cast<char*>(smem);
        const size_t gstride = mft_x3_stage_bytes(p.bn_max_tiles, p.Cin);
        const bool two = bn_two;
        mft_x3_stats_stage(p.bn_ws, p.Cin, g0, p.M, p.rows_per_group, BM, p.bn_max_tiles, stage, tid, 256);
        if (two) mft_x3_stats_stage(p.bn_ws, p.Cin, g0 + 1, p.M, p.rows_per_group, BM, p.bn_max_tiles, stage + gstride, tid, 256);
        __syncthreads();
        for (int i = tid; i < 2 * p.Cin; i += 256) {
            const int gi = i >= p.Cin ? 1 : 0, c = i - gi * p.Cin;
            if (gi == 0 || two) {
                float mu, rs, sc, sh;
                mft_x3_stats_staged(stage + gi * gstride, p.bn_max_tiles, p.Cin, c, g0 + gi, p.M, p.rows_per_group, BM, p.bn_eps, mu, rs);
                mft_bn_fold(mu, rs, p.bn_gamma[c], p.bn_beta[c], sc, sh);
                bn_tab[(gi * 2 + 0) * p.Cin + c] = sc;
                bn_tab[(gi * 2 + 1) * p.Cin + c] = sh;
            }
        }
        __syncthreads();
    }
    const int g_id = tid >> 5, g_rr = (tid >> 3) & 3;
    const int lrow = p.row_swz ? g_rr * 4 + (g_id & 3) + 16 * (g_id >> 2) : tid >> 3;
    const int c4 = (tid & 7) * 4;
    const __amdgpu_buffer_rsrc_t rA = __builtin_amdgcn_make_buffer_rsrc((void*)p.in, 0, p.in_bytes, 0x00020000);
    const __amdgpu_buffer_rsrc_t rB = __builtin_amdgcn_make_buffer_rsrc((void*)p.w3, 0, p.w_bytes, 0x00020000);
    int a_off[PA], a_oh[PA], a_lds[PA], a_tab[PA];
    bool a_ok[PA];
#pragma unroll
    for (int j = 0; j < PA; ++j) {
        const int t = lrow + 32 * j, m = m0 + t;
        const int fr = m / W;
        a_ok[j] = m < p.M;
        a_oh[j] = fr - (fr / H) * H;
        a_off[j] = ((a_ok[j] ? m : 0) * p.ldi + c4) * 4;
        a_lds[j] = (t + 1) * RS + c4;
        a_tab[j] = BNIN ? ((a_ok[j] ? m / p.rows_per_group - g0 : 0) * 2 * p.Cin + c4) : 0;
    }
    const int hside = (tid >> 3) & 1;
    const int mh = hside ? m0 + BM : m0 - 1;
    const int frh = (mh > 0 ? mh : 0) / W;
    const bool h_ok = tid < 16 && (hside ? (mh < p.M && mh - frh * W != 0) : (m0 > 0 && m0 - fr0 * W != 0));
    const int h_oh = frh - (frh / H) * H;
    const int h_off = ((h_ok ? mh : 0) * p.ldi + c4) * 4;
    const int h_lds = (hside ? BM + 1 : 0) * RS + c4;
    const int h_tab = BNIN ? (((hside && h_ok) ? (m0 + BM - 1) / p.rows_per_group - g0 : 0) * 2 * p.Cin + c4) : 0;

    const int bseg = tid & 3;
    const int brow = p.row_swz ? ((tid >> 2) & 3) * 4 + ((tid >> 4) & 3) + 16 * (tid >> 6) : tid >> 2;
    int b_off[PB];
#pragma unroll
    for (int j = 0; j < PB; ++j) b_off[j] = ((n0 + brow + 64 * j) * p.Kpad + bseg * 8) * 2;
    const int plane_bytes = (int)(p.plane * 2);

    int fa[TM], fl[TM], fr_[TM];
    constexpr int Z0 = BM + 2;
#pragma unroll
    for (int i = 0; i < TM; ++i) {
        const int t = wm * (BM / 2) + i * 32 + r;
        const int ow = (m0 + t) - ((m0 + t) / W) * W;
        fa[i] = (t + 1) * RS;
        fl[i] = ow == 0 ? (Z0 + ((t - Z0) & 15)) * RS : fa[i] - RS;
        fr_[i] = ow == W - 1 ? (Z0 + ((t + 2 - Z0) & 15)) * RS : fa[i] + RS;
    }

    f32x16 acc[NACC][TM][TN];
#pragma unroll
    for (int q = 0; q < NACC; ++q)
#pragma unroll
        for (int i = 0; i < TM; ++i)
#pragma unroll
            for (int j = 0; j < TN; ++j)
#pragma unroll
                for (int e = 0; e < 16; ++e) acc[q][i][j][e] = 0.f;
    auto val = [&](int i, int j, int e) -> float {
        if constexpr (NP == 3) return acc[0][i][j][e];
        else return __builtin_fmaf(acc[1][i][j][e], X3_H2_LO_SCALE, acc[0][i][j][e]);
    };

    struct Stage {
        f32x4 ra[PA];
        f32x4 rh;
        u32x4 rb[PB][NP];
    };
    Stage st;
    const int n_ci = p.Cin / 32;
    const int n_ms = 3 * n_ci;
    auto load_a = [&](int ms, Stage& S) {
        const int kh = ms / n_ci, ci0 = (ms - kh * n_ci) * 32;
        const int shift = ((kh - 1) * W * p.ldi + ci0) * 4;
#pragma unroll
        for (int j = 0; j < PA; ++j) {
            const bool ok = a_ok[j] && (unsigned)(a_oh[j] + kh - 1) < (unsigned)H;
            S.ra[j] = __builtin_bit_cast(f32x4, __builtin_amdgcn_raw_buffer_load_b128(rA, ok ? (unsigned)(a_off[j] + shift) : 0x80000000u, 0, 0));
        }
        const bool okh = h_ok && (unsigned)(h_oh + kh - 1) < (unsigned)H;
        S.rh = __builtin_bit_cast(f32x4, __builtin_amdgcn_raw_buffer_load_b128(rA, okh ? (unsigned)(h_off + shift) : 0x80000000u, 0, 0));
    };
    auto load_b = [&](int ms, int kw, Stage& S) {
        const int kh = ms / n_ci, ci0 = (ms - kh * n_ci) * 32;
        const int k0 = (kh * 3 + kw) * p.Cin + ci0;
#pragma unroll
        for (int j = 0; j < PB; ++j)
#pragma unroll
            for (int pl = 0; pl < NP; ++pl)
                S.rb[j][pl] = __builtin_amdgcn_raw_buffer_load_b128(rB, b_off[j] + pl * plane_bytes, k0 * 2, 0);
    };
    auto put_a = [&](const f32x4 v, int off) {
        if constexpr (NP == 3) {
            u32x2 p1, p2, p3;
            split4(v, p1, p2, p3);
            *(u32x2*)(As + off) = p1;
            *(u32x2*)(As + A_PLANE + off) = p2;
            *(u32x2*)(As + 2 * A_PLANE + off) = p3;
        } else {
            u32x2 p1, p2;
            split4_h2(v, p1, p2);
            *(u32x2*)(As + off) = p1;
            *(u32x2*)(As + A_PLANE + off) = p2;
        }
    };
    auto bn_relu = [&](const f32x4 v, const f32x4 sc, const f32x4 sh, bool ok) {
        f32x4 o = mft_bn_affine4(v, sc, sh);
#pragma unroll
        for (int e = 0; e < 4; ++e) o[e] = ok ? fmaxf(o[e], 0.f) : 0.f;
        return o;
    };
    auto store_a = [&](const Stage& S, int ms) {
        if constexpr (BNIN) {
            const int kh = ms / n_ci, ci0 = (ms - kh * n_ci) * 32;
            const bool okh = h_ok && (unsigned)(h_oh + kh - 1) < (unsigned)H;
            if (!bn_two) {
                const f32x4 sc = *(const f32x4*)(bn_tab + ci0 + c4), sh = *(const f32x4*)(bn_tab + p.Cin + ci0 + c4);
#pragma unroll
                for (int j = 0; j < PA; ++j)
                    put_a(bn_relu(S.ra[j], sc, sh, a_ok[j] && (unsigned)(a_oh[j] + kh - 1) < (unsigned)H), a_lds[j]);
                if (tid < 16) put_a(bn_relu(S.rh, sc, sh, okh), h_lds);
            } else {
#pragma unroll
                for (int j = 0; j < PA; ++j)
                    put_a(bn_relu(S.ra[j], *(const f32x4*)(bn_tab + a_tab[j] + ci0), *(const f32x4*)(bn_tab + a_tab[j] + p.Cin + ci0),
                                  a_ok[j] && (unsigned)(a_oh[j] + kh - 1) < (unsigned)H), a_lds[j]);
                if (tid < 16)
                    put_a(bn_relu(S.rh, *(const f32x4*)(bn_tab + h_tab + ci0), *(const f32x4*)(bn_tab + h_tab + p.Cin + ci0), okh), h_lds);
            }
        } else {
#pragma unroll
            for (int j = 0; j < PA; ++j) put_a(S.ra[j], a_lds[j]);
            if (tid < 16) put_a(S.rh, h_lds);
        }
    };
    auto store_b = [&](const Stage& S, int bb = 0) {
#pragma unroll
        for (int j = 0; j < PB; ++j)
#pragma unroll
            for (int pl = 0; pl < NP; ++pl)
                *(u32x4*)(Bs + (bb * NP + pl) * B_PLANE + (brow + 64 * j) * RS + bseg * 8) = S.rb[j][pl];
    };
    auto compute = [&](int kw, int bb = 0) {
        const unsigned short* const Bc = Bs + bb * NP * B_PLANE;
#pragma unroll
        for (int kk = 0; kk < 2; ++kk) {
            if constexpr (NP == 3) {
                bf16x8 a[TM][3], b[TN][3];
#pragma unroll
                for (int i = 0; i < TM; ++i)
#pragma unroll
                    for (int pl = 0; pl < 3; ++pl)
                        a[i][pl] = *(const bf16x8*)(As + pl * A_PLANE + (kw == 0 ? fl[i] : (kw == 1 ? fa[i] : fr_[i])) + kk * 16 + h * 8);
#pragma unroll
                for (int j = 0; j < TN; ++j)
#pragma unroll
                    for (int pl = 0; pl < 3; ++pl)
                        b[j][pl] = *(const bf16x8*)(Bc + pl * B_PLANE + (wn * (BN / 2) + j * 32 + r) * RS + kk * 16 + h * 8);
                constexpr int TA[6] = {2, 0, 1, 1, 0, 0};
                constexpr int TB[6] = {0, 2, 1, 0, 1, 0};
#pragma unroll
                for (int t = 0; t < 6; ++t)
#pragma unroll
                    for (int i = 0; i < TM; ++i)
#pragma unroll
                        for (int j = 0; j < TN; ++j)
                            acc[0][i][j] = __builtin_amdgcn_mfma_f32_32x32x16_bf16(a[i][TA[t]], b[j][TB[t]], acc[0][i][j], 0, 0, 0);
            } else {
                f16x8 a[TM][2], b[TN][2];
#pragma unroll
                for (int i = 0; i < TM; ++i)
#pragma unroll
                    for (int pl = 0; pl < 2; ++pl)
                        a[i][pl] = *(const f16x8*)(As + pl * A_PLANE + (kw == 0 ? fl[i] : (kw == 1 ? fa[i] : fr_[i])) + kk * 16 + h * 8);
#pragma unroll
                for (int j = 0; j < TN; ++j)
#pragma unroll
                    for (int pl = 0; pl < 2; ++pl)
                        b[j][pl] = *(const f16x8*)(Bc + pl * B_PLANE + (wn * (BN / 2) + j * 32 + r) * RS + kk * 16 + h * 8);
                constexpr int TA[3] = {0, 1, 0};
                constexpr int TB[3] = {1, 0, 0};
                constexpr int TQ[3] = {1, 1, 0};
#pragma unroll
                for (int t = 0; t < 3; ++t)
#pragma unroll
                    for (int i = 0; i < TM; ++i)
#pragma unroll
                        for (int j = 0; j < TN; ++j)
                            acc[TQ[t]][i][j] = __builtin_amdgcn_mfma_f32_32x32x16_f16(a[i][TA[t]], b[j][TB[t]], acc[TQ[t]][i][j], 0, 0, 0);
            }
        }
    };

    for (int i = tid; i < NP * A_PLANE / 8; i += 256) ((u32x4*)As)[i] = (u32x4){0u, 0u, 0u, 0u};
    load_a(0, st);
    load_b(0, 0, st);
// ... 29 lines not shown
            compute(0);
            __syncthreads();
            store_b(st);
            __syncthreads();
            load_b(ms, 2, st);
            compute(1);
            __syncthreads();
            store_b(st);
            __syncthreads();
            load_a(msn, st);
            load_b(msn, 0, st);
            compute(2);
            __syncthreads();
            store_a(st, msn);
            store_b(st);
            __syncthreads();
        }
    }

#pragma unroll
    for (int i = 0; i < TM; ++i)
#pragma unroll
        for (int j = 0; j < TN; ++j) {
            const int n = n0 + wn * (BN / 2) + j * 32 + r;
#pragma unroll
            for (int e = 0; e < 16; ++e) {
                const int row = (e & 3) + 8 * (e >> 2) + 4 * h;
                const int m = m0 + wm * (BM / 2) + i * 32 + row;
                if (m < p.M) p.out[(long long)m * p.ldo + n] = val(i, j, e);
            }
        }
    if (p.stats_ws != nullptr) {
        static_assert(TN == 1 || TN == 2, "stats epilogue");
        const int split = (m0 / p.rows_per_group + 1) * p.rows_per_group;
        float* sred = reinterpret_cast<float*>(smem);
        __syncthreads();
#pragma unroll
        for (int j = 0; j < TN; ++j) {
            float a1 = 0.f, a2 = 0.f, b1 = 0.f, b2 = 0.f;
#pragma unroll
            for (int i = 0; i < TM; ++i)
#pragma unroll
                for (int e = 0; e < 16; ++e) {
                    const int m = m0 + wm * (BM / 2) + i * 32 + (e & 3) + 8 * (e >> 2) + 4 * h;
                    const float v = val(i, j, e);
                    if (m < p.M) {
                        if (m < split) { a1 += v; a2 += v * v; }
                        else { b1 += v; b2 += v * v; }
                    }
                }
            a1 += __shfl_xor(a1, 32, 64); a2 += __shfl_xor(a2, 32, 64);
            b1 += __shfl_xor(b1, 32, 64); b2 += __shfl_xor(b2, 32, 64);
            if (h == 0) {
                float* o = sred + ((((wm * 2 + wn) * TN + j) * 32 + r) << 2);
                o[0] = a1; o[1] = a2; o[2] = b1; o[3] = b2;
            }
        }
        __syncthreads();
        if (wm == 0 && h == 0) {
#pragma unroll
            for (int j = 0; j < TN; ++j) {
                const float* o0 = sred + ((((0 * 2 + wn) * TN + j) * 32 + r) << 2);
                const float* o1 = sred + ((((1 * 2 + wn) * TN + j) * 32 + r) << 2);
                const int n = n0 + wn * (BN / 2) + j * 32 + r;
                float* w0 = p.stats_ws + (((long long)mt * 2 + 0) * p.Cout + n) * 2;
                float* w1 = p.stats_ws + (((long long)mt * 2 + 1) * p.Cout + n) * 2;
                w0[0] = o0[0] + o1[0]; w0[1] = o0[1] + o1[1];
                w1[0] = o0[2] + o1[2]; w1[1] = o0[3] + o1[3];
            }
        }
    }
}

template <int BM, int BN, int NP = 3, bool BDB = true>
__global__ __launch_bounds__(256) __attribute__((amdgpu_waves_per_eu(NP == 2 ? 3 : 1))) void conv_x3_s1_kernel(X3Args p) {
    conv_x3_s1_body<BM, BN, false, NP, BDB>(p);
}

template <int BM, int BN, int NP = 3, bool BDB = true>
__global__ __launch_bounds__(256) __attribute__((amdgpu_waves_per_eu(3, 3))) void conv_x3_s1_bnin_kernel(X3Args p) {
    conv_x3_s1_body<BM, BN, true, NP, BDB>(p);
}

__global__ void x3_stats_finalize_kernel(const float* __restrict__ ws, int C, int M, int R, int BM, float eps,
                                         float* __restrict__ mean, float* __restrict__ rstd) {
    const int c = blockIdx.x * blockDim.x + threadIdx.x;
    const int g = blockIdx.y;
    if (c >= C) return;
    float mu, rs;
    mft_x3_stats_merge(ws, C, c, g, M, R, BM, eps, mu, rs);
    mean[(long long)g * C + c] = mu;
    rstd[(long long)g * C + c] = rs;
}

__global__ __launch_bounds__(256) void split_bf16x3_kernel(const float* __restrict__ w, unsigned short* __restrict__ out,
                                                           long long n) {
    for (long long i = (long long)blockIdx.x * blockDim.x + threadIdx.x; i < n; i += (long long)gridDim.x * blockDim.x) {
        const float x = w[i];
        const unsigned q1 = pk_bf16(x, 0.f) & 0xffffu;
        const float r1 = x - __builtin_bit_cast(float, q1 << 16);
        const unsigned q2 = pk_bf16(r1, 0.f) & 0xffffu;
        const float r2 = r1 - __builtin_bit_cast(float, q2 << 16);
        const unsigned q3 = pk_bf16(r2, 0.f) & 0xffffu;
        out[i] = (unsigned short)q1;
        out[n + i] = (unsigned short)q2;
        out[2 * n + i] = (unsigned short)q3;
    }
}

struct SplitJob { const float* src; unsigned short* dst; long long n, Cout, Cin, taps, transposed, start; };

__global__ __launch_bounds__(256) void split_bf16x3_multi_kernel(const SplitJob* __restrict__ jobs, int n_jobs, long long total) {
    for (long long i = (long long)blockIdx.x * blockDim.x + threadIdx.x; i < total; i += (long long)gridDim.x * blockDim.x) {
        int lo = 0, hi = n_jobs - 1;
        while (lo < hi) {
            const int mid = (lo + hi + 1) >> 1;
            if (jobs[mid].start <= i) lo = mid; else hi = mid - 1;
        }
        const SplitJob j = jobs[lo];
        const long long l = i - j.start;
        long long src = l;
        if (j.transposed) {
            const long long co = l % j.Cout, t = l / j.Cout;
            const long long tp = t % j.taps, ci = t / j.taps;
            src = (co * j.taps + (j.taps - 1 - tp)) * j.Cin + ci;
        }
        const float x = j.src[src];
        const unsigned q1 = pk_bf16(x, 0.f) & 0xffffu;
        const float r1 = x - __builtin_bit_cast(float, q1 << 16);
        const unsigned q2 = pk_bf16(r1, 0.f) & 0xffffu;
        const float r2 = r1 - __builtin_bit_cast(float, q2 << 16);
        const unsigned q3 = pk_bf16(r2, 0.f) & 0xffffu;
        j.dst[l] = (unsigned short)q1;
        j.dst[j.n + l] = (unsigned short)q2;
        j.dst[2 * j.n + l] = (unsigned short)q3;
    }
}

__global__ __launch_bounds__(256) void split_f16x2_kernel(const float* __restrict__ w, unsigned short* __restrict__ out, long long n) {
    for (long long i = (long long)blockIdx.x * blockDim.x + threadIdx.x; i < n; i += (long long)gridDim.x * blockDim.x) {
        const float x = w[i];
        const _Float16 hi = (_Float16)x;
        const _Float16 lo = (_Float16)((x - (float)hi) * 2048.f);
        out[i] = __builtin_bit_cast(unsigned short, hi);
        out[n + i] = __builtin_bit_cast(unsigned short, lo);
    }
}

int g_x3_db = 0;
int g_x3_dbg = 0;
int g_x3_hoist = 0;
int g_x3_row_swz = 1;
int g_x3_xcd = 1;
int g_x3_min_lds_kb = 0;

template <int BM, int BN, bool AP, bool DB>
int launch_x3(X3Args p, hipStream_t s, int np = 3) {
    const int tiles_m = (p.M + BM - 1) / BM;
    p.tiles_n = p.Cout / BN;
    p.xcd_swizzle = g_x3_xcd;
    p.row_swz = g_x3_row_swz;
    if (np == 2) {
        if constexpr (!AP && !DB) {
            p.row_swz = g_x3_row_swz != 0;
            const size_t lds2 = (size_t)2 * (BM + BN) * X3_RS * sizeof(unsigned short);
            hipLaunchKernelGGL((conv_x3_kernel<BM, BN, false, false, 0, 0, false, 2>), dim3((unsigned)(tiles_m * p.tiles_n)), dim3(256), lds2, s, p);
            return mft_launch_status();
        }
        return MFT_EINVAL;
    }
#ifdef MFT_EXPERIMENTS
    const bool xs = g_x3_row_swz == 2 && !AP && !DB && g_x3_hoist == 0 && g_x3_dbg == 0;
#else
    constexpr bool xs = false;
#endif
    size_t lds = (size_t)(DB ? 2 : 1) * 3 * (BM + BN) * (xs ? 32 : X3_RS) * sizeof(unsigned short);
#ifdef MFT_EXPERIMENTS
    if ((size_t)g_x3_min_lds_kb * 1024 > lds) lds = (size_t)g_x3_min_lds_kb * 1024;
    if (xs) {
        if constexpr (!AP && !DB) {
            hipLaunchKernelGGL((conv_x3_kernel<BM, BN, false, false, 0, 0, true>), dim3((unsigned)(tiles_m * (p.Cout / BN))), dim3(256), lds, s,
                               ([&] { X3Args q = p; q.tiles_n = p.Cout / BN; q.xcd_swizzle = g_x3_xcd; q.row_swz = 0; return q; })());
            return mft_launch_status();
        }
    }
    auto kern = g_x3_hoist == 1 ? conv_x3_kernel<BM, BN, AP, DB, 1> : (g_x3_hoist == 2 ? conv_x3_kernel<BM, BN, AP, DB, 2> : conv_x3_kernel<BM, BN, AP, DB, 0>);
    if (g_x3_dbg && !AP && !DB) {
        switch (g_x3_dbg) {
            case 1: kern = conv_x3_kernel<BM, BN, AP, DB, 0, 1>; break;
            case 2: kern = conv_x3_kernel<BM, BN, AP, DB, 0, 2>; break;
            case 4: kern = conv_x3_kernel<BM, BN, AP, DB, 0, 4>; break;
            case 8: kern = conv_x3_kernel<BM, BN, AP, DB, 0, 8>; break;
            case 12: kern = conv_x3_kernel<BM, BN, AP, DB, 0, 12>; break;
            case 13: kern = conv_x3_kernel<BM, BN, AP, DB, 0, 13>; break;
            case 16: kern = conv_x3_kernel<BM, BN, AP, DB, 0, 16>; break;
            case 28: kern = conv_x3_kernel<BM, BN, AP, DB, 0, 28>; break;
            case 32: kern = conv_x3_kernel<BM, BN, AP, DB, 0, 32>; break;
            case 34: kern = conv_x3_kernel<BM, BN, AP, DB, 0, 34>; break;
            case 36: kern = conv_x3_kernel<BM, BN, AP, DB, 0, 36>; break;
            case 33: kern = conv_x3_kernel<BM, BN, AP, DB, 0, 33>; break;
            default: break;
        }
    }
#else
    auto kern = conv_x3_kernel<BM, BN, AP, DB, 0>;
#endif
    if (lds > 64 * 1024) {
        hipError_t e = hipFuncSetAttribute((const void*)kern, hipFuncAttributeMaxDynamicSharedMemorySize, 160 * 1024);
        if (e != hipSuccess) return (int)e;
    }
    hipLaunchKernelGGL(kern, dim3((unsigned)(tiles_m * p.tiles_n)), dim3(256), lds, s, p);
    return mft_launch_status();
}

int g_x3_s1 = 1;

constexpr size_t X3_S1_LDS_3PER_CU = 160 * 1024 / 3;

int g_x3_bdb = 1;

inline size_t x3_s1_lds(int BM, int BN, int W, int bn_cin, int np = 3) {
    (void)W;
    return (size_t)np * (BM + 18 + ((np == 2 && g_x3_bdb) ? 2 : 1) * BN) * X3_RS * sizeof(unsigned short) + (size_t)4 * bn_cin * sizeof(float);
}

template <int BM, int BN>
int launch_x3_s1(X3Args p, hipStream_t s, int np = 3) {
    const int tiles_m = (p.M + BM - 1) / BM;
    p.tiles_n = p.Cout / BN;
    p.xcd_swizzle = g_x3_xcd;
    p.row_swz = g_x3_row_swz != 0;
    p.s1_rows = BM + 18;
    const size_t lds = x3_s1_lds(BM, BN, p.W, p.bn_ws ? p.Cin : 0, np);
    const dim3 grid((unsigned)(tiles_m * p.tiles_n));
    if (np == 2 && g_x3_bdb) {
        if (p.bn_ws) hipLaunchKernelGGL((conv_x3_s1_bnin_kernel<BM, BN, 2, true>), grid, dim3(256), lds, s, p);
        else hipLaunchKernelGGL((conv_x3_s1_kernel<BM, BN, 2, true>), grid, dim3(256), lds, s, p);
    } else if (np == 2) {
        if (p.bn_ws) hipLaunchKernelGGL((conv_x3_s1_bnin_kernel<BM, BN, 2, false>), grid, dim3(256), lds, s, p);
        else hipLaunchKernelGGL((conv_x3_s1_kernel<BM, BN, 2, false>), grid, dim3(256), lds, s, p);
    } else if (p.bn_ws) {
        hipLaunchKernelGGL((conv_x3_s1_bnin_kernel<BM, BN>), grid, dim3(256), lds, s, p);
    } else {
        hipLaunchKernelGGL((conv_x3_s1_kernel<BM, BN>), grid, dim3(256), lds, s, p);
    }
    return mft_launch_status();
}

int g_x3_pp = 0;
#ifdef MFT_EXPERIMENTS

template <int BM, int BN>
int launch_x3_pp(X3Args p, hipStream_t s) {
    const int tiles_m = (p.M + BM - 1) / BM;
    p.tiles_n = p.Cout / BN;
    p.xcd_swizzle = g_x3_xcd;
    p.row_swz = 1;
    const size_t lds = (size_t)2 * 3 * (BM + BN) * X3_RS * sizeof(unsigned short);
    static MftPerDeviceOnce attr_once;
    if (attr_once.need()) {
        hipError_t e = hipFuncSetAttribute((const void*)conv_x3_pp_kernel<BM, BN>, hipFuncAttributeMaxDynamicSharedMemorySize, 160 * 1024);
        if (e != hipSuccess) return (int)e;
        attr_once.mark();
    }
    hipLaunchKernelGGL((conv_x3_pp_kernel<BM, BN>), dim3((unsigned)(tiles_m * p.tiles_n)), dim3(512), lds, s, p);
    return mft_launch_status();
}

#endif

#ifdef MFT_EXPERIMENTS
#include "../../tools/experiments/conv3x3_patch_x3.inc"
#endif
int g_x3_patch = 0;
int g_x3_tile = 0;

}

extern "C" int mft_split_bf16x3(const float* w, unsigned short* planes, long long n, void* stream) {
    if (n <= 0) return MFT_EINVAL;
    long long blocks = (n + 255) / 256;
    if (blocks > 4096) blocks = 4096;
    hipLaunchKernelGGL(split_bf16x3_kernel, dim3((unsigned)blocks), dim3(256), 0, (hipStream_t)stream, w, planes, n);
    return mft_launch_status();
}

extern "C" int mft_split_bf16x3_multi(const void* jobs, int n_jobs, long long total_elements, void* stream) {
    if (n_jobs < 1 || total_elements < 1) return MFT_EINVAL;
    long long blocks = (total_elements + 255) / 256;
    if (blocks > 4096) blocks = 4096;
    hipLaunchKernelGGL(split_bf16x3_multi_kernel, dim3((unsigned)blocks), dim3(256), 0, (hipStream_t)stream, (const SplitJob*)jobs, n_jobs,
                       total_elements);
    return mft_launch_status();
}

extern "C" int mft_debug_set_x3_tile(int t) {
#ifndef MFT_EXPERIMENTS
    const bool off = (t == 10 || t == 60 || t == 70 || t == 80 || t == 100 || t == 200);
    if (!off && ((t >= 10 && t < 20) || t == 42 || (t >= 60 && t < 90) || t >= 100)) return MFT_EINVAL;
#endif
    if (t >= 200) g_x3_dbg = t - 200;
    else if (t >= 100) g_x3_min_lds_kb = t - 100;
    else if (t >= 90) g_x3_s1 = t - 90;
    else if (t >= 80) g_x3_hoist = t - 80;
    else if (t >= 70) g_x3_pp = t - 70;
    else if (t >= 60) g_x3_db = t - 60;
    else if (t >= 40) g_x3_row_swz = t - 40;
    else if (t >= 30) g_x3_bdb = t - 30;
    else if (t >= 20) g_x3_xcd = t - 20;
    else if (t >= 10) g_x3_patch = t - 10;
    else g_x3_tile = t;
    return 0;
}

static int x3_dispatch(const float* in, int ldi, const unsigned short* w3, long long plane_elems, float* out, int ldo,
                       int n_img, int H, int W, int Cin, int Cout, int KH, int KW, int stride, int pad, float* stats_ws,
                       int rows_per_group, void* stream, const unsigned short* in3 = nullptr, long long in_plane_elems = 0,
                       const float* bn_ws = nullptr, const float* bn_gamma = nullptr, const float* bn_beta = nullptr,
                       float bn_eps = 0.f, int np = 3) {
    if (n_img <= 0 || Cin % 32 != 0 || Cout % 64 != 0 || ldi % 4 != 0 || (np != 3 && np != 2)) return MFT_EINVAL;
    if (np == 2 && (in3 != nullptr || g_x3_tile > 1 || g_x3_db || g_x3_pp || g_x3_dbg || g_x3_hoist || g_x3_row_swz == 2 || g_x3_min_lds_kb ||
                    g_x3_patch))
        return MFT_EINVAL;
    X3Args p;
    p.bn_ws = bn_ws; p.bn_gamma = bn_gamma; p.bn_beta = bn_beta; p.bn_eps = bn_eps;
    p.bn_max_tiles = bn_ws ? mft_x3_max_group_tiles(rows_per_group, 128) : 0;
    if (bn_ws != nullptr && (in3 != nullptr || !bn_gamma || !bn_beta || rows_per_group < 128 || KH != 3 || KW != 3 || stride != 1 ||
                             pad != 1 || x3_s1_lds(128, 64, W, Cin, np) > X3_S1_LDS_3PER_CU ||
                             2 * mft_x3_stage_bytes_host(p.bn_max_tiles, Cin) >
                                 (size_t)np * (128 + 18) * X3_RS * sizeof(unsigned short)))
        return MFT_EINVAL;
    p.in3 = in3;
    p.in_plane_bytes = 0;
    p.stats_ws = stats_ws;
    p.rows_per_group = rows_per_group;
    p.in = in; p.w3 = w3; p.plane = plane_elems; p.out = out; p.ldi = ldi; p.ldo = ldo;
    p.H = H; p.W = W; p.Cin = Cin; p.Cout = Cout; p.KH = KH; p.KW = KW; p.stride = stride; p.pad = pad;
    p.OH = (H + 2 * pad - KH) / stride + 1;
    p.OW = (W + 2 * pad - KW) / stride + 1;
    p.Kpad = KH * KW * Cin;
    const long long M = (long long)n_img * p.OH * p.OW;
    if (M > 0x7fffffffLL) return MFT_EINVAL;
    p.M = (int)M;
    p.tiles_n = 0;
    hipStream_t s = (hipStream_t)stream;
    int G = 0, R = 0;
    double eff = 0.0;
    if (in3 != nullptr) {
        const long long need = (long long)n_img * H * W * ldi;
        if (ldi % 8 != 0 || in_plane_elems < need || 3 * in_plane_elems * 2 >= 0x7fff0000LL || 3 * plane_elems * 2 >= 0x7fff0000LL)
            return MFT_EINVAL;
        if (stats_ws != nullptr && rows_per_group < 128) return MFT_EINVAL;
        p.in_plane_bytes = (unsigned)(in_plane_elems * 2);
        p.in_bytes = 0;
        p.w_bytes = (unsigned)(3 * plane_elems * 2);
        return launch_x3<128, 64, true, false>(p, (hipStream_t)stream);
    }
#ifdef MFT_EXPERIMENTS
    if (stats_ws == nullptr && g_x3_patch && KH == 3 && KW == 3 && stride == 1 && pad == 1 && ldi == Cin && ldo == Cout &&
        patch_geometry(H, W, &G, &R, &eff) && (g_x3_patch >= 2 || eff >= 0.9)) {
        P3Args q;
        q.in = in; q.w3 = w3; q.plane = plane_elems; q.out = out;
        q.n_img = n_img; q.H = H; q.W = W; q.Cin = Cin; q.Cout = Cout; q.G = G; q.R = R;
        q.row_blocks = (H + R - 1) / R;
        q.tiles_n = Cout / 64;
        const int img_groups = (n_img + G - 1) / G;
        const size_t lds = (size_t)3 * G * (R + 2) * (W + 2) * X3_RS * sizeof(unsigned short);
        static MftPerDeviceOnce attr_once;
        if (attr_once.need()) {
            hipError_t e = hipFuncSetAttribute((const void*)conv3x3_patch_x3_kernel, hipFuncAttributeMaxDynamicSharedMemorySize,
                                               64 * 1024);
            if (e != hipSuccess) return (int)e;
            attr_once.mark();
        }
        if (lds <= 64 * 1024) {
            hipLaunchKernelGGL(conv3x3_patch_x3_kernel, dim3((unsigned)(img_groups * q.row_blocks * q.tiles_n)), dim3(256), lds, s, q);
            return mft_launch_status();
        }
    }
#else
    (void)G; (void)R; (void)eff;
#endif
    int tile = g_x3_tile;
    if (tile == 0) tile = 1;
    p.w_bytes = (unsigned)(np * plane_elems * 2);
    const long long img_bytes = (long long)H * W * ldi * 4;
    const long long max_imgs = 0x7fff0000LL / img_bytes;
    if (max_imgs < 1 || 3 * plane_elems * 2 >= 0x7fff0000LL) return MFT_EINVAL;
    if ((stats_ws != nullptr || bn_ws != nullptr) && (max_imgs < n_img || rows_per_group < 128)) return MFT_EINVAL;
    if (stats_ws != nullptr && tile != 3) tile = 1;
    if (stats_ws != nullptr && tile == 3 && rows_per_group < 64) return MFT_EINVAL;
    for (long long i0 = 0; i0 < n_img; i0 += max_imgs) {
        const long long ni = (n_img - i0 < max_imgs) ? (n_img - i0) : max_imgs;
        X3Args q = p;
        q.in = in + i0 * H * W * ldi;
        q.out = out + i0 * p.OH * p.OW * ldo;
        q.M = (int)(ni * p.OH * p.OW);
        q.in_bytes = (unsigned)(ni * img_bytes);
        const bool s1 = g_x3_s1 && tile == 1 && KH == 3 && KW == 3 && stride == 1 && pad == 1 && !g_x3_db && !g_x3_pp && !g_x3_dbg &&
                        g_x3_hoist == 0 && g_x3_row_swz != 2 && g_x3_min_lds_kb == 0 &&
                        x3_s1_lds(128, 64, W, 0, np) <= 64 * 1024;
        if (bn_ws != nullptr && !s1) return MFT_EINVAL;
        const int rc = s1 ? launch_x3_s1<128, 64>(q, s, np)
                       : np == 2 ? launch_x3<128, 64, false, false>(q, s, 2)
                       : (tile == 2 && Cout % 128 == 0) ? launch_x3<128, 128, false, false>(q, s)
                       : (tile == 3)                  ? launch_x3<64, 64, false, false>(q, s)
#ifdef MFT_EXPERIMENTS
                       : g_x3_db                      ? launch_x3<128, 64, false, true>(q, s)
                       : (g_x3_pp && !g_x3_dbg)       ? launch_x3_pp<128, 64>(q, s)
#endif
                                                      : launch_x3<128, 64, false, false>(q, s);
        if (rc != 0) return rc;
    }
    return 0;
}

extern "C" int mft_conv2d_nhwc_x3(const float* in, int ldi, const unsigned short* w3, long long plane_elems, float* out,
                                  int ldo, int n_img, int H, int W, int Cin, int Cout, int KH, int KW, int stride,
                                  int pad, void* stream) {
    return x3_dispatch(in, ldi, w3, plane_elems, out, ldo, n_img, H, W, Cin, Cout, KH, KW, stride, pad, nullptr, 0, stream);
}

extern "C" int mft_split_f16x2(const float* w, unsigned short* planes, long long n, void* stream) {
    if (n <= 0) return MFT_EINVAL;
    long long blocks = (n + 255) / 256;
    if (blocks > 4096) blocks = 4096;
    hipLaunchKernelGGL(split_f16x2_kernel, dim3((unsigned)blocks), dim3(256), 0, (hipStream_t)stream, w, planes, n);
    return mft_launch_status();
}

extern "C" int mft_conv2d_nhwc_h2(const float* in, int ldi, const unsigned short* w2, long long plane_elems, float* out,
                                  int ldo, int n_img, int H, int W, int Cin, int Cout, int KH, int KW, int stride,
                                  int pad, void* stream) {
    return x3_dispatch(in, ldi, w2, plane_elems, out, ldo, n_img, H, W, Cin, Cout, KH, KW, stride, pad, nullptr, 0, stream, nullptr, 0,
                       nullptr, nullptr, nullptr, 0.f, 2);
}

extern "C" long long mft_conv2d_x3_stats_ws_floats(int n_img, int H, int W, int Cout, int KH, int KW, int stride, int pad) {
    const long long OH = (H + 2 * pad - KH) / stride + 1, OW = (W + 2 * pad - KW) / stride + 1;
    return ((long long)n_img * OH * OW + 63) / 64 * 2 * Cout * 2;
}

static int x3_bnstats(int np, const float* in, int ldi, const unsigned short* w3, long long plane_elems,
                      float* out, int ldo, int n_img, int H, int W, int Cin, int Cout, int KH, int KW,
                      int stride, int pad, int imgs_per_group, float eps, float* stats_ws,
                      float* mean, float* rstd, void* stream) {
    if (imgs_per_group <= 0 || n_img % imgs_per_group != 0 || stats_ws == nullptr) return MFT_EINVAL;
    const int OH = (H + 2 * pad - KH) / stride + 1, OW = (W + 2 * pad - KW) / stride + 1;
    const int R = imgs_per_group * OH * OW;
    const int rc = x3_dispatch(in, ldi, w3, plane_elems, out, ldo, n_img, H, W, Cin, Cout, KH, KW, stride, pad, stats_ws, R,
                               stream, nullptr, 0, nullptr, nullptr, nullptr, 0.f, np);
    if (rc != 0) return rc;
    if (mean == nullptr && rstd == nullptr) return g_x3_tile == 3 ? MFT_EINVAL : 0;
    const int groups = n_img / imgs_per_group;
    hipLaunchKernelGGL(x3_stats_finalize_kernel, dim3((Cout + 63) / 64, groups), dim3(64), 0, (hipStream_t)stream,
                       (const float*)stats_ws, Cout, n_img * OH * OW, R, g_x3_tile == 3 ? 64 : 128, eps, mean, rstd);
    return mft_launch_status();
}

extern "C" int mft_conv2d_nhwc_x3_bnstats(const float* in, int ldi, const unsigned short* w3, long long plane_elems,
                                          float* out, int ldo, int n_img, int H, int W, int Cin, int Cout, int KH, int KW,
                                          int stride, int pad, int imgs_per_group, float eps, float* stats_ws,
                                          float* mean, float* rstd, void* stream) {
    return x3_bnstats(3, in, ldi, w3, plane_elems, out, ldo, n_img, H, W, Cin, Cout, KH, KW, stride, pad, imgs_per_group, eps, stats_ws, mean,
                      rstd, stream);
}

extern "C" int mft_conv2d_nhwc_h2_bnstats(const float* in, int ldi, const unsigned short* w2, long long plane_elems,
                                          float* out, int ldo, int n_img, int H, int W, int Cin, int Cout, int KH, int KW,
                                          int stride, int pad, int imgs_per_group, float eps, float* stats_ws,
                                          float* mean, float* rstd, void* stream) {
    return x3_bnstats(2, in, ldi, w2, plane_elems, out, ldo, n_img, H, W, Cin, Cout, KH, KW, stride, pad, imgs_per_group, eps, stats_ws, mean,
                      rstd, stream);
}

static int x3_bnin_bnstats(int np, const float* in, int ldi, const float* in_ws, const float* in_gamma,
                           const float* in_beta, const unsigned short* w3, long long plane_elems, float* out,
                           int ldo, int n_img, int H, int W, int Cin, int Cout, int imgs_per_group, float eps,
                           float* stats_ws, float* mean, float* rstd, void* stream) {
    if (imgs_per_group <= 0 || n_img % imgs_per_group != 0 || stats_ws == nullptr || in_ws == nullptr ||
        (mean == nullptr) != (rstd == nullptr) || g_x3_tile == 3)
        return MFT_EINVAL;
    const int R = imgs_per_group * H * W;
    const int rc = x3_dispatch(in, ldi, w3, plane_elems, out, ldo, n_img, H, W, Cin, Cout, 3, 3, 1, 1, stats_ws, R, stream, nullptr, 0,
                               in_ws, in_gamma, in_beta, eps, np);
    if (rc != 0 || mean == nullptr) return rc;
    hipLaunchKernelGGL(x3_stats_finalize_kernel, dim3((Cout + 63) / 64, n_img / imgs_per_group), dim3(64), 0, (hipStream_t)stream,
                       (const float*)stats_ws, Cout, n_img * H * W, R, 128, eps, mean, rstd);
    return mft_launch_status();
}

extern "C" int mft_conv2d_nhwc_x3_bnin_bnstats(const float* in, int ldi, const float* in_ws, const float* in_gamma,
                                               const float* in_beta, const unsigned short* w3, long long plane_elems, float* out,
                                               int ldo, int n_img, int H, int W, int Cin, int Cout, int imgs_per_group, float eps,
                                               float* stats_ws, float* mean, float* rstd, void* stream) {
    return x3_bnin_bnstats(3, in, ldi, in_ws, in_gamma, in_beta, w3, plane_elems, out, ldo, n_img, H, W, Cin, Cout, imgs_per_group, eps,
                           stats_ws, mean, rstd, stream);
}

extern "C" int mft_conv2d_nhwc_h2_bnin_bnstats(const float* in, int ldi, const float* in_ws, const float* in_gamma,
                                               const float* in_beta, const unsigned short* w2, long long plane_elems, float* out,
                                               int ldo, int n_img, int H, int W, int Cin, int Cout, int imgs_per_group, float eps,
                                               float* stats_ws, float* mean, float* rstd, void* stream) {
    return x3_bnin_bnstats(2, in, ldi, in_ws, in_gamma, in_beta, w2, plane_elems, out, ldo, n_img, H, W, Cin, Cout, imgs_per_group, eps,
                           stats_ws, mean, rstd, stream);
}

extern "C" int mft_conv2d_nhwc_x3p_bnstats(const unsigned short* in_planes, long long in_plane_elems, int ldi,
                                           const unsigned short* w3, long long plane_elems, float* out, int ldo, int n_img,
                                           int H, int W, int Cin, int Cout, int KH, int KW, int stride, int pad,
                                           int imgs_per_group, float eps, float* stats_ws, float* mean, float* rstd,
                                           void* stream) {
    if (imgs_per_group <= 0 || n_img % imgs_per_group != 0 || stats_ws == nullptr || in_planes == nullptr) return MFT_EINVAL;
    const int OH = (H + 2 * pad - KH) / stride + 1, OW = (W + 2 * pad - KW) / stride + 1;
    const int R = imgs_per_group * OH * OW;
    const int rc = x3_dispatch(nullptr, ldi, w3, plane_elems, out, ldo, n_img, H, W, Cin, Cout, KH, KW, stride, pad, stats_ws, R,
                               stream, in_planes, in_plane_elems);
    if (rc != 0) return rc;
    const int groups = n_img / imgs_per_group;
    hipLaunchKernelGGL(x3_stats_finalize_kernel, dim3((Cout + 63) / 64, groups), dim3(64), 0, (hipStream_t)stream,
                       (const float*)stats_ws, Cout, n_img * OH * OW, R, 128, eps, mean, rstd);
    return mft_launch_status();
}
```

meta-fine-tuning_amd/functional.py:

```python
import os

import numpy as np

import torch

from . import ops
from . import settings

FUSED_DGRAD = settings.current().fused_dgrad
FUSED_LAST_BLOCK = settings.current().fused_last_block
X3_PLANES = settings.current().x3_planes
X3_FUSED_STATS = settings.current().x3_fused_stats
X3_FOLD_BN = settings.current().x3_fold_bn
TRUNK_F16X2 = settings.current().trunk_f16x2
TRAIN_X3 = settings.current().train_x3
TRAIN_X3_MIN_ROWS = settings.current().train_x3_min_rows
FUSE_NEXT_C2_ONLY = settings.current().fuse_next_c2_only
F16X2_BOUND = 3.0e4
F16X2_FLOOR = 2.0 ** -10
F16X2_MAX_ROWS = 1 << 20


def stem_rows_bound(ipg, image_size):
    oh = (image_size + 6 - 7) // 2 + 1
    ph = (oh + 2 - 3) // 2 + 1
    h6 = (ph + 2 - 3) // 2 + 1
    side = max(oh, 2 * ph, 4 * h6)
    return int(ipg) * side * side


def f16x2_safe(sd, prefix="", max_rows=None):
    import math
    max_rows = F16X2_MAX_ROWS if max_rows is None else int(max_rows)

    def arr(key):
        return np.abs(sd[prefix + key].detach().float().cpu().numpy())

    def g(name):
        w, b = arr(name + ".weight"), arr(name + ".bias")
        if not float(np.median(w)) >= F16X2_FLOOR:
            return float("inf")
        return float(w.max()) * math.sqrt(max_rows) + float(b.max())

    try:
        x_in = g("trunk.1")
        for idx, (cin, cout, _s) in STAGES.items():
            if idx == 7:
                break
            p = "trunk.%d" % idx
            for cname in (".C1", ".C2") + ((".shortcut",) if cin != cout else ()):
                w = arr(p + cname + ".weight")
                if not (float(w.max()) < F16X2_BOUND and float(np.sqrt(np.mean(np.square(w, dtype=np.float64)))) >= F16X2_FLOOR):
                    return False
            r1 = g(p + ".BN1")
            x_out = g(p + ".BN2") + (g(p + ".BNshortcut") if cin != cout else x_in)
            if not (x_in < F16X2_BOUND and r1 < F16X2_BOUND):
                return False
            x_in = x_out
        return True
    except KeyError:
        return False

STAGES = {4: (64, 64, 1), 5: (64, 128, 2), 6: (128, 256, 2), 7: (256, 512, 2)}

ADAPT_KEYS = [
    "trunk.7.C1.weight", "trunk.7.BN1.weight", "trunk.7.BN1.bias",
    "trunk.7.C2.weight", "trunk.7.BN2.weight", "trunk.7.BN2.bias",
    "trunk.7.shortcut.weight", "trunk.7.BNshortcut.weight", "trunk.7.BNshortcut.bias",
]
ADAPT_SHAPES = {
    "trunk.7.C1.weight": (512, 256, 3, 3), "trunk.7.C2.weight": (512, 512, 3, 3),
    "trunk.7.shortcut.weight": (512, 256, 1, 1),
    "trunk.7.BN1.weight": (512,), "trunk.7.BN1.bias": (512,), "trunk.7.BN2.weight": (512,),
    "trunk.7.BN2.bias": (512,), "trunk.7.BNshortcut.weight": (512,), "trunk.7.BNshortcut.bias": (512,),
}
ADAPT_NUMEL = sum(int(torch.Size(s).numel()) for s in ADAPT_SHAPES.values())


class Arena:

    def __init__(self, device):
        self.device = device
        self.bufs = {}

    def get(self, name, shape, dtype=torch.float32):
        key = (name, tuple(shape), dtype)
        t = self.bufs.get(key)
        if t is None:
            t = torch.empty(tuple(shape), device=self.device, dtype=dtype)
            self.bufs[key] = t
        return t

    def existing(self, name, shape, dtype=torch.float32):
        key = (name, tuple(shape), dtype)
        if key not in self.bufs:
            near = sorted(str(k) for k in self.bufs if k[0] == name)
# ... 80 lines not shown

    ORDER = [("c1w", 512 * 2304), ("c2w", 512 * 4608), ("scw", 512 * 256),
             ("bn1g", 512), ("bn1b", 512), ("bn2g", 512), ("bn2b", 512), ("bnsg", 512), ("bnsb", 512)]
    KEY = {"c1w": "trunk.7.C1.weight", "c2w": "trunk.7.C2.weight", "scw": "trunk.7.shortcut.weight",
           "bn1g": "trunk.7.BN1.weight", "bn1b": "trunk.7.BN1.bias", "bn2g": "trunk.7.BN2.weight",
           "bn2b": "trunk.7.BN2.bias", "bnsg": "trunk.7.BNshortcut.weight", "bnsb": "trunk.7.BNshortcut.bias"}

    def __init__(self, E, device, zero=True, flat=None):
        self.E = E
        total = E * ADAPT_NUMEL
        if flat is not None:
            assert flat.numel() == total and flat.dtype == torch.float32 and flat.is_contiguous()
            self.flat = flat.zero_() if zero else flat
        else:
            self.flat = torch.zeros(total, device=device) if zero else torch.empty(total, device=device)
        off = 0
        for name, n in self.ORDER:
            v = self.flat[off:off + E * n]
            if name.endswith("w"):
                cout = 512
                v = v.view(E, cout, n // cout)
            else:
                v = v.view(E, n)
            setattr(self, name, v)
            off += E * n
        assert off == total

    def load_shared(self, W):
        self.c1w.copy_(W.conv["trunk.7.C1"].unsqueeze(0).expand_as(self.c1w))
        self.c2w.copy_(W.conv["trunk.7.C2"].unsqueeze(0).expand_as(self.c2w))
        self.scw.copy_(W.conv["trunk.7.shortcut"].unsqueeze(0).expand_as(self.scw))
        for nm, bnname in (("bn1", "trunk.7.BN1"), ("bn2", "trunk.7.BN2"), ("bns", "trunk.7.BNshortcut")):
            g, b = W.bn[bnname]
            getattr(self, nm + "g").copy_(g.unsqueeze(0).expand(self.E, -1))
            getattr(self, nm + "b").copy_(b.unsqueeze(0).expand(self.E, -1))

    def export(self, e):
        out = {}
        for name, _ in self.ORDER:
            key = self.KEY[name]
            t = getattr(self, name)[e]
            if name.endswith("w"):
                out[key] = ops.unpack_conv_weight(t.contiguous(), ADAPT_SHAPES[key])
            else:
                out[key] = t.clone()
        return out


def _bn_stats4(arena, tag, x, ipg, groups, running=None, fixed=None):
    if fixed is not None:
        return fixed
    n, H, W, C = x.shape
    mean = arena.get(tag + ".mean", (groups, C))
    rstd = arena.get(tag + ".rstd", (groups, C))
    rows = ipg * H * W
    nws = max(int(ops._lib.lib().mft_bn_stats_ws_floats(C, rows, groups)), 1)
    ws = arena.get("bn.ws", (max(nws, 1 << 16),)) if nws <= (1 << 16) else arena.get(tag + ".ws", (nws,))
    rm = rv = nbt = None
    if running is not None:
        rm, rv, nbt = running if len(running) == 3 else (running + (None,))
    rc = ops._lib.lib().mft_bn_stats(ops._p(x), C, C, rows, groups, ops.BN_EPS, ops._p(mean), ops._p(rstd), ops._p(ws),
                                     ops._p(rm), ops._p(rv), 0.1, ops._p(nbt), ops._stream())
    ops._lib.check(rc, "mft_bn_stats")
    return mean, rstd


class StemCache:

    def __init__(self, W, n_slots, H, device, chunk=8192, pooled=None):
        self.W = W
        self.n_slots = n_slots
        self.OH = (H + 6 - 7) // 2 + 1
        self.PH = (self.OH + 2 - 3) // 2 + 1
        cfg = settings.current()
        self.pooled = cfg.stem_pooled if pooled is None else bool(pooled)
        chunk = chunk if cfg.stem_chunk is None else cfg.stem_chunk
        self.chunk = min(chunk, n_slots)
        self.mean = torch.empty((n_slots, 64), device=device)
        self.m2 = torch.empty((n_slots, 64), device=device)
        self.fused_fill = bool(self.pooled and cfg.stem_fused_fill and H == 84)
        if self.pooled:
            self.c0 = None
            self._buf = None if self.fused_fill else torch.empty((self.chunk, self.OH, self.OH, 64), device=device)
            self.pmax = torch.empty((n_slots, self.PH, self.PH, 64), device=device)
            self.pmin = torch.empty((n_slots, self.PH, self.PH, 64), device=device)
        else:
            self.c0 = torch.empty((n_slots, self.OH, self.OH, 64), device=device)

    def nbytes(self):
        ts = [self.mean, self.m2] + ([self._buf, self.pmax, self.pmin] if self.pooled else [self.c0])
        return sum(t.numel() * 4 for t in ts if t is not None)

    @staticmethod
    def bytes_needed(n_slots, H, pooled=None, chunk=8192):
        cfg = settings.current()
        pooled = cfg.stem_pooled if pooled is None else bool(pooled)
        chunk = min(chunk if cfg.stem_chunk is None else cfg.stem_chunk, n_slots)
        oh = (H + 6 - 7) // 2 + 1
        ph = (oh + 2 - 3) // 2 + 1
        per = 2 * 64 + (2 * ph * ph * 64 if pooled else oh * oh * 64)
        fused = bool(pooled and cfg.stem_fused_fill and H == 84)
        return 4 * (n_slots * per + (chunk * oh * oh * 64 if (pooled and not fused) else 0))

    def fill(self, x_nhwc):
        lib = ops._lib.lib()
        n = x_nhwc.shape[0]
        assert n == self.n_slots
        if self.fused_fill:
            wpk = self.W.conv["trunk.0"]
            rc = lib.mft_stem_cache_fill(ops._p(x_nhwc), ops._p(wpk), wpk.shape[-1], n, x_nhwc.shape[1], x_nhwc.shape[2],
                                         ops._p(self.pmax), ops._p(self.pmin), ops._p(self.mean), ops._p(self.m2), ops._stream())
            if rc != ops._lib.MFT_EINVAL:
                ops._lib.check(rc, "mft_stem_cache_fill")
                return
            self.fused_fill = False
            self._buf = torch.empty((self.chunk, self.OH, self.OH, 64), device=x_nhwc.device)
        for i in range(0, n, self.chunk):
            j = min(i + self.chunk, n)
            c0 = self._buf[:j - i] if self.pooled else self.c0[i:j]
            ops.conv2d(x_nhwc[i:j], self.W.conv["trunk.0"], 64, 7, 7, 2, 3, out=c0)
            ops._lib.check(lib.mft_bn_image_moments(ops._p(c0), 64, 64, self.OH * self.OH, j - i,
                                                    ops._p(self.mean[i:j]), ops._p(self.m2[i:j]), ops._stream()),
                           "mft_bn_image_moments")
            if self.pooled:
                ops._lib.check(lib.mft_pool_window_minmax(ops._p(c0), ops._p(self.pmax[i:j]), ops._p(self.pmin[i:j]), j - i,
                                                          self.OH, self.OH, 64, ops._stream()), "mft_pool_window_minmax")

    def gather(self, idx, n, m, s, g, b, ipg, out, planes=None):
        if self.pooled and planes is None:
            ops._lib.check(ops._lib.lib().mft_bn_relu_pooled_gather(ops._p(self.pmax), ops._p(self.pmin), ops._p(idx), ops._p(out), n,
                                                                    self.PH, self.PH, 64, ipg, ops._p(m), ops._p(s), ops._p(g),
                                                                    ops._p(b), ops._stream()), "mft_bn_relu_pooled_gather")
            return out
        assert self.c0 is not None, "this path needs the full-resolution stem cache (StemCache(pooled=False))"
        return ops.bn_relu_maxpool_gather(self.c0, idx, n, m, s, g, b, ipg, out=out, planes=planes)

    def gather_moments(self, idx, n, g, b, ipg, out, stats=None):
        assert self.pooled
        m, s = stats if stats is not None else (None, None)
        ops._lib.check(ops._lib.lib().mft_bn_relu_pooled_gather_moments(
            ops._p(self.pmax), ops._p(self.pmin), ops._p(idx), ops._p(out), n, self.PH, self.PH, 64, ipg, ops._p(self.mean),
            ops._p(self.m2), self.OH * self.OH, ops.BN_EPS, ops._p(g), ops._p(b), ops._p(m), ops._p(s), ops._stream()),
            "mft_bn_relu_pooled_gather_moments")
        return out


def resnet10_trunk(W, x, arena, ipg, upto=7, running=None, tag="t", stem=None, fixed=None):

    def run(name):
        return None if running is None else running.get(name)

    def fix(name):
        return None if fixed is None else fixed[name]

    g, b = W.bn["trunk.1"]
    if stem is not None:
        cache, idx = stem
        n = idx.numel()
        groups = n // ipg
        PH = (cache.OH + 2 - 3) // 2 + 1
        fold = X3_FOLD_BN and cache.pooled and not X3_PLANES and running is None and fixed is None
        if not fold:
            m = arena.get(tag + ".bn0.mean", (groups, 64))
            s = arena.get(tag + ".bn0.rstd", (groups, 64))
            ops.bn_combine_moments(cache.mean, cache.m2, idx, cache.OH * cache.OH, ipg, groups, mean=m, rstd=s)
        if (X3_PLANES and cache.c0 is not None and X3_FUSED_STATS and upto == 7 and running is None and fixed is None and ipg * ((PH + 3) // 4) ** 2 >= 128
                and all(("trunk.%d.C1" % i) in W.conv3 for i in (4, 5, 6))):
            ap = arena.get(tag + ".p0p", (3, n * PH * PH, 64), torch.int16)
            a = cache.gather(idx, n, m, s, g, b, ipg, arena.get(tag + ".p0", (n, PH, PH, 64)), planes=ap)
            shape = (n, PH, PH, 64)
            for bi in (4, 5, 6):
                cin, cout, stride = STAGES[bi]
                p = "trunk.%d" % bi
                mode = "f32" if bi == 6 else "planes"
                r = simple_block(W, p, a if bi == 4 else None, arena, ipg, cin, cout, stride, None, tag + "." + p, xp=ap,
                                 xshape=shape, out_mode=mode)
                if mode == "f32":
                    return r
                _, ap = r
                OHb = (shape[1] + 2 - 3) // stride + 1
                shape = (n, OHb, OHb, cout)
        if fold:
            a = cache.gather_moments(idx, n, g, b, ipg, arena.get(tag + ".p0", (n, PH, PH, 64)))
        else:
            a = cache.gather(idx, n, m, s, g, b, ipg, arena.get(tag + ".p0", (n, PH, PH, 64)))
    else:
        n = x.shape[0]
        groups = n // ipg
        c0 = ops.conv2d(x, W.conv["trunk.0"], 64, 7, 7, 2, 3, out=arena.get(tag + ".c0", (n, (x.shape[1] + 6 - 7) // 2 + 1, (x.shape[2] + 6 - 7) // 2 + 1, 64)))
        m, s = _bn_stats4(arena, tag + ".bn0", c0, ipg, groups, run("trunk.1"), fix("trunk.1"))
        a = ops.bn_relu_maxpool(c0, m, s, g, b, imgs_per_group=ipg)
    for idx in (4, 5, 6, 7):
        if idx >= upto:
            break
        cin, cout, stride = STAGES[idx]
        p = "trunk.%d" % idx
        a = simple_block(W, p, a, arena, ipg, cin, cout, stride, running, tag + "." + p, fixed=fixed)
    return a


def _bn_small(arena, tag, x1, g1, b1, rows, groups, C, gbs, out, x2=None, g2=None, b2=None, res=None, pooled=None, hw=0, stats=None,
              stats2=None):
    m1, s1 = stats if stats is not None else (arena.get(tag + ".mean", (groups, C)), arena.get(tag + ".rstd", (groups, C)))
    m2 = s2 = None
    if x2 is not None:
        m2, s2 = stats2 if stats2 is not None else (arena.get(tag + ".mean2", (groups, C)), arena.get(tag + ".rstd2", (groups, C)))
    rc = ops._lib.lib().mft_bn_small_forward(ops._p(x1), C, ops._p(x2), C, ops._p(res), C, ops._p(out), C, C, rows, groups,
                                             ops._p(g1), ops._p(b1), ops._p(g2), ops._p(b2), gbs, ops._p(m1), ops._p(s1),
                                             ops._p(m2), ops._p(s2), ops.ACT_RELU, 0.0, ops.BN_EPS, ops._p(pooled), hw,
                                             ops._stream())
    ops._lib.check(rc, "mft_bn_small_forward")
    return m1, s1, m2, s2


def simple_block(W, p, x, arena, ipg, cin, cout, stride, running=None, tag="b", slab=None, tape=None, pooled=None, fixed=None,
                 xp=None, xshape=None, out_mode="f32", stats_out=None):
    n, H, Wd, _ = x.shape if x is not None else xshape
    groups = n // ipg
    OH = (H + 2 - 3) // stride + 1

    def run(name):
        return None if running is None else running.get(name)

    def fix(name):
        return None if fixed is None else fixed[name]

    if slab is None:
        c1w, c2w = W.conv[p + ".C1"], W.conv[p + ".C2"]
        (g1, b1), (g2, b2) = W.bn[p + ".BN1"], W.bn[p + ".BN2"]
        scw = W.conv.get(p + ".shortcut")
        gs, bs = W.bn.get(p + ".BNshortcut", (None, None))
        gbs = 0
    else:
        c1w, c2w, scw = slab.c1w, slab.c2w, slab.scw
        g1, b1, g2, b2, gs, bs = slab.bn1g, slab.bn1b, slab.bn2g, slab.bn2b, slab.bnsg, slab.bnsb
        gbs = cout
    wipg = ipg if slab is not None else 0
    w3 = W.planes(p, ipg, H, fixed, running) if slab is None else {}

    def conv(name, inp, wpk, k, s, pd, out):
        if (p + name) in w3:
            return ops.conv2d_x3(inp, w3[p + name], cout, k, k, s, pd, out=out)
        return ops.conv2d(inp, wpk, cout, k, k, s, pd, imgs_per_group=wipg, out=out)

    rows = ipg * OH * OH
    if slab is not None and rows <= 64 and cout % 64 == 0 and cin != cout and running is None:
        so = stats_out or {}
        c1 = arena.get(tag + ".c1", (n, OH, OH, cout))
        r1 = arena.get(tag + ".r1", (n * OH * OH, cout))
        sc = arena.get(tag + ".sc", (n, OH, OH, cout))
        rc = ops._lib.MFT_EINVAL
        if FUSED_LAST_BLOCK and c1w.dim() == 3 and scw.dim() == 3 and groups > ops.SMALL_GROUPS and not so:
            m1 = arena.get(tag + ".bn1.mean", (groups, cout))
            s1 = arena.get(tag + ".bn1.rstd", (groups, cout))
            rc = ops._lib.lib().mft_block_entry_small_forward(
                ops._p(x), x.shape[-1], ops._p(c1w), c1w.shape[1] * c1w.shape[2], ops._p(scw), scw.shape[1] * scw.shape[2],
                ops._p(c1), ops._p(r1), ops._p(sc), n, H, Wd, cin, cout, stride, ipg, ops._p(g1), ops._p(b1), gbs, ops._p(m1),
                ops._p(s1), ops.BN_EPS, ops._stream())
            if rc != ops._lib.MFT_EINVAL:
                ops._lib.check(rc, "mft_block_entry_small_forward")
        if rc == ops._lib.MFT_EINVAL:
            conv(".C1", x, c1w, 3, stride, 1, c1)
            m1, s1, _, _ = _bn_small(arena, tag + ".bn1", c1, g1, b1, rows, groups, cout, gbs, r1, stats=so.get("bn1"))
            conv(".shortcut", x, scw, 1, stride, 0, sc)
        r1 = r1.view(n, OH, OH, cout)
        c2 = arena.get(tag + ".c2", (n, OH, OH, cout))
        out = arena.get(tag + ".out", (n * OH * OH, cout))
        rc = ops._lib.MFT_EINVAL
        if FUSED_LAST_BLOCK and pooled is not None and c2w.dim() == 3 and groups > ops.SMALL_GROUPS and not so:
            m2, s2, ms, ss = (arena.get(tag + ".bn2." + k, (groups, cout)) for k in ("mean", "rstd", "mean2", "rstd2"))
            rc = ops._lib.lib().mft_block_exit_small_forward(
                ops._p(r1), ops._p(c2w), c2w.shape[1] * c2w.shape[2], ops._p(sc), ops._p(c2), ops._p(out), ops._p(pooled), n, OH,
                OH, cout, ipg, ops._p(g2), ops._p(b2), ops._p(gs), ops._p(bs), gbs, ops._p(m2), ops._p(s2), ops._p(ms),
                ops._p(ss), ops.BN_EPS, ops._stream())
            if rc != ops._lib.MFT_EINVAL:
                ops._lib.check(rc, "mft_block_exit_small_forward")
        if rc == ops._lib.MFT_EINVAL:
# ... 2 lines not shown
                                       pooled=pooled, hw=OH * OH, stats=so.get("bn2"), stats2=so.get("bns"))
        out = out.view(n, OH, OH, cout)
        if tape is not None:
            tape.update(x=x, c1=c1, m1=m1, s1=s1, r1=r1, c2=c2, m2=m2, s2=s2, sc=sc, ms=ms, ss=ss, out=out,
                        pooled=pooled is not None)
        return out
    fuse_stats = (slab is None and running is None and fixed is None and rows >= 128 and X3_FUSED_STATS)

    def conv_bn(name, bnname, inp, wpk, k, s, pd, obuf, stag):
        if fuse_stats and (p + name) in w3:
            H_in = inp.shape[1]
            nws = int(ops._lib.lib().mft_conv2d_x3_stats_ws_floats(n, H_in, H_in, cout, k, k, s, pd))
            ws = arena.get("x3.statws", (max(nws, 1 << 20),)) if nws <= (1 << 20) else arena.get(stag + ".statws", (nws,))
            mean = arena.get(stag + ".mean", (groups, cout))
            rstd = arena.get(stag + ".rstd", (groups, cout))
            r = ops.conv2d_x3_bnstats(inp, w3[p + name], cout, k, k, s, pd, ipg, obuf, ws, mean, rstd)
            if r is not None:
                return r
        o = conv(name, inp, wpk, k, s, pd, obuf)
        mm, ss_ = _bn_stats4(arena, stag, o, ipg, groups, run(p + bnname), fix(p + bnname))
        return o, mm, ss_

    if (X3_FOLD_BN and xp is None and fuse_stats and tape is None and out_mode == "f32"
            and all((p + nm) in w3 for nm in ((".C1", ".C2", ".shortcut") if cin != cout else (".C1", ".C2")))):
        r = _frozen_block_folded(W, p, x, arena, ipg, cin, cout, stride, tag)
        if r is not None:
            return r

    if xp is not None and fuse_stats and tape is None and all((p + nm) in w3 for nm in ((".C1", ".C2", ".shortcut") if cin != cout
                                                                                      else (".C1", ".C2"))):
        def conv_bn_p(name, inp_p, h_in, k, s, pd, obuf, stag):
            nws = int(ops._lib.lib().mft_conv2d_x3_stats_ws_floats(n, h_in, h_in, cout, k, k, s, pd))
            ws = arena.get("x3.statws", (max(nws, 1 << 20),)) if nws <= (1 << 20) else arena.get(stag + ".statws", (nws,))
            mean = arena.get(stag + ".mean", (groups, cout))
            rstd = arena.get(stag + ".rstd", (groups, cout))
            return ops.conv2d_x3p_bnstats(inp_p, n, h_in, h_in, w3[p + name], cout, k, k, s, pd, ipg, obuf, ws, mean, rstd)

        c1, m1, s1 = conv_bn_p(".C1", xp, H, 3, stride, 1, arena.get(tag + ".c1", (n, OH, OH, cout)), tag + ".bn1")
        r1p = arena.get(tag + ".r1p", (3, n * OH * OH, cout), torch.int16)
        ops.bn_apply(c1.view(-1, cout), cout, rows, groups, m1, s1, g1, b1, act=ops.ACT_RELU, fma_affine=True, gb_group_stride=gbs, planes=r1p,
                     write_y=False)
        c2, m2, s2 = conv_bn_p(".C2", r1p, OH, 3, 1, 1, arena.get(tag + ".c2", (n, OH, OH, cout)), tag + ".bn2")
        want_f32 = out_mode in ("f32", "both")
        out = arena.get(tag + ".out", (n * OH * OH, cout)) if want_f32 else None
        outp = arena.get(tag + ".outp", (3, n * OH * OH, cout), torch.int16) if out_mode in ("planes", "both") else None
        if cin != cout:
            sc, ms, ss = conv_bn_p(".shortcut", xp, H, 1, stride, 0, arena.get(tag + ".sc", (n, OH, OH, cout)), tag + ".bns")
            res, res_bn = sc.view(-1, cout), (ms, ss, gs, bs)
        else:
            res, res_bn = x.view(-1, cin), None
        if outp is not None:
            ops.bn_apply(c2.view(-1, cout), cout, rows, groups, m2, s2, g2, b2, act=ops.ACT_RELU, fma_affine=True, res=res, res_bn=res_bn, out=out,
                         gb_group_stride=gbs, planes=outp, write_y=want_f32)
        else:
            ops.bn_apply(c2.view(-1, cout), cout, rows, groups, m2, s2, g2, b2, act=ops.ACT_RELU, fma_affine=True, res=res, res_bn=res_bn, out=out,
                         gb_group_stride=gbs)
        out = out.view(n, OH, OH, cout) if out is not None else None
        return out if out_mode == "f32" else (out, outp)
    assert out_mode == "f32" or xp is None or not fuse_stats, "planes output requested outside the pre-split chain"

    c1, m1, s1 = conv_bn(".C1", ".BN1", x, c1w, 3, stride, 1, arena.get(tag + ".c1", (n, OH, OH, cout)), tag + ".bn1")
    r1 = ops.bn_apply(c1.view(-1, cout), cout, rows, groups, m1, s1, g1, b1, act=ops.ACT_RELU, fma_affine=fuse_stats,
                      out=arena.get(tag + ".r1", (n * OH * OH, cout)), gb_group_stride=gbs).view(n, OH, OH, cout)
    c2, m2, s2 = conv_bn(".C2", ".BN2", r1, c2w, 3, 1, 1, arena.get(tag + ".c2", (n, OH, OH, cout)), tag + ".bn2")
    out = arena.get(tag + ".out", (n * OH * OH, cout))
    sc = ms = ss = None
    if cin != cout:
        sc, ms, ss = conv_bn(".shortcut", ".BNshortcut", x, scw, 1, stride, 0, arena.get(tag + ".sc", (n, OH, OH, cout)),
                             tag + ".bns")
        ops.bn_apply(c2.view(-1, cout), cout, rows, groups, m2, s2, g2, b2, act=ops.ACT_RELU, fma_affine=fuse_stats, res=sc.view(-1, cout),
                     res_bn=(ms, ss, gs, bs), out=out, gb_group_stride=gbs)
    else:
        ops.bn_apply(c2.view(-1, cout), cout, rows, groups, m2, s2, g2, b2, act=ops.ACT_RELU, fma_affine=fuse_stats, res=x.view(-1, cin),
                     out=out, gb_group_stride=gbs)
    out = out.view(n, OH, OH, cout)
    if tape is not None:
        tape.update(x=x, c1=c1, m1=m1, s1=s1, r1=r1, c2=c2, m2=m2, s2=s2, sc=sc, ms=ms, ss=ss, out=out)
    return out


_X3WS_FITS = {}


def _frozen_block_folded(W, p, x, arena, ipg, cin, cout, stride, tag):
    n, H, _, _ = x.shape
    groups = n // ipg
    OH = (H + 2 - 3) // stride + 1
    rows = ipg * OH * OH
    lib = ops._lib.lib()
    fits = _X3WS_FITS.get((cout, rows))
    if fits is None:
        fits = _X3WS_FITS[(cout, rows)] = bool(lib.mft_bn_apply_x3ws_fits(cout, rows, 1))
    if not fits:
        return None
    (g1, b1), (g2, b2) = W.bn[p + ".BN1"], W.bn[p + ".BN2"]
    w3 = W.conv3

    def partials(name, inp, k, s, pd, obuf, stag):
        ws = arena.get(stag + ".statws", (int(lib.mft_conv2d_x3_stats_ws_floats(n, inp.shape[1], inp.shape[1], cout, k, k, s, pd)),))
        r = ops.conv2d_x3_bnstats(inp, w3[p + name], cout, k, k, s, pd, ipg, obuf, ws, None, None)
        return None if r is None else ws

    c1 = arena.get(tag + ".c1", (n, OH, OH, cout))
    ws1 = partials(".C1", x, 3, stride, 1, c1, tag + ".bn1")
    if ws1 is None:
        return None
    c2 = arena.get(tag + ".c2", (n, OH, OH, cout))
    ws2 = arena.get(tag + ".bn2.statws", (int(lib.mft_conv2d_x3_stats_ws_floats(n, OH, OH, cout, 3, 3, 1, 1)),))
    if ops.conv2d_x3_bnin_bnstats(c1, ws1, g1, b1, w3[p + ".C2"], cout, ipg, c2, ws2) is None:
        r1 = ops.bn_apply_x3ws(c1.view(-1, cout), cout, rows, groups, ws1, g1, b1, arena.get(tag + ".r1", (n * OH * OH, cout)),
                               act=ops.ACT_RELU).view(n, OH, OH, cout)
        if ops.conv2d_x3_bnstats(r1, w3[p + ".C2"], cout, 3, 3, 1, 1, ipg, c2, ws2, None, None) is None:
            raise RuntimeError("frozen block %s: C2 outside the bf16x3 domain after C1 was inside it" % p)
    out = arena.get(tag + ".out", (n * OH * OH, cout))
    if cin != cout:
        gs, bs = W.bn[p + ".BNshortcut"]
        sc = arena.get(tag + ".sc", (n, OH, OH, cout))
        wss = partials(".shortcut", x, 1, stride, 0, sc, tag + ".bns")
        if wss is None:
            raise RuntimeError("frozen block %s: shortcut outside the bf16x3 domain after C1 was inside it" % p)
        ops.bn_apply_x3ws(c2.view(-1, cout), cout, rows, groups, ws2, g2, b2, out, act=ops.ACT_RELU, res=sc.view(-1, cout),
                          res_ws=wss, res_gamma=gs, res_beta=bs)
    else:
        ops.bn_apply_x3ws(c2.view(-1, cout), cout, rows, groups, ws2, g2, b2, out, act=ops.ACT_RELU, res=x.view(-1, cin))
    return out.view(n, OH, OH, cout)


def last_block_forward(W, a, arena, ipg, slab=None, tape=None, running=None, tag="f", fixed=None, stats_out=None):
    n = a.shape[0]
    feat = arena.get(tag + ".feat", (n, 512))
    info = tape if tape is not None else {}
    out = simple_block(W, "trunk.7", a, arena, ipg, 256, 512, 2, running, tag + ".trunk.7", slab=slab, tape=info, pooled=feat,
                       fixed=fixed, stats_out=stats_out)
    if not info.get("pooled", False):
        ops._lib.check(ops._lib.lib().mft_global_avgpool(ops._p(out), ops._p(feat), n, out.shape[1] * out.shape[2], 512,
                                                         ops._stream()), "mft_global_avgpool")
    return feat


def resnet10_forward(W, x, arena, ipg=0, slab=None, tape=None, running=None, tag="f", fixed=None):
    n = x.shape[0]
    if ipg <= 0 or fixed is not None:
        ipg = n
    a = resnet10_trunk(W, x, arena, ipg, upto=7, running=running, tag=tag, fixed=fixed)
    return last_block_forward(W, a, arena, ipg, slab=slab, tape=tape, running=running, tag=tag, fixed=fixed)


def _dgrad_c2_bn1(lib, tape, params, grads, arena, tag, dc2, c1, r1, n, oh, ow, C, ipg, bn_bwd):
    rc = ops._lib.MFT_EINVAL
    if FUSED_LAST_BLOCK and n // ipg > ops.SMALL_GROUPS:
        dc1 = arena.get(tag + ".dc1", tuple(c1.shape))
        w2 = params.c2w
        rc = lib.mft_conv2d_dgrad_bn_backward_small(ops._p(dc2), C, ops._p(w2), ops._p(dc1), C, n, oh, ow, C, C, 3, 3, 1, ipg,
                                                    w2.shape[1] * w2.shape[2], ops._p(c1), ops._p(r1), ops._p(tape["m1"]),
                                                    ops._p(tape["s1"]), ops._p(params.bn1g), C, ops._p(grads.bn1g),
                                                    ops._p(grads.bn1b), ops._stream())
        if rc != ops._lib.MFT_EINVAL:
            ops._lib.check(rc, "mft_conv2d_dgrad_bn_backward_small")
    if rc == ops._lib.MFT_EINVAL:
        dr1 = ops.conv2d_dgrad(dc2, params.c2w, 512, 3, 3, 1, imgs_per_group=ipg, out=arena.get(tag + ".dr1", (n, oh, ow, C)))
        dc1 = bn_bwd(c1, dr1, tape["m1"], tape["s1"], params.bn1g, grads.bn1g, grads.bn1b, r1, "dc1")
    return dc1


def next_step_tape(arena, tag, n, oh, ow, C, groups):
    rows = n * oh * ow
    t = {k: arena.get(tag + "." + k, (n, oh, ow, C)) for k in ("c1", "r1", "c2", "sc", "out")}
    for k in ("m1", "s1", "m2", "s2", "ms", "ss"):
        t[k] = arena.get(tag + "." + k, (groups, C))
    t["feat"] = arena.get(tag + ".feat", (n, C))
    t["pooled"] = True
    assert t["c1"].numel() == rows * C
    return t


def last_block_backward(tape, dfeat, params, grads, arena, ipg, tag="bw", adam=None, ce=None, nxt=None, before_next_read=None):
    x, c1, r1, c2, sc, out = tape["x"], tape["c1"], tape["r1"], tape["c2"], tape["sc"], tape["out"]
    n, oh, ow, C = out.shape
    groups = n // ipg
    rows = ipg * oh * ow
    lib = ops._lib.lib()
    fused_ce = FUSED_LAST_BLOCK and ce is not None and C % 64 == 0 and ipg <= 16
    d_out = None
    if fused_ce:
        pass
    elif ce is not None:
        d_out = arena.get(tag + ".dout", (n, oh, ow, C))
        feat, labels, loss = ce
        ops._lib.check(lib.mft_ce_pool_backward(ops._p(feat), ops._p(labels), ipg, groups, C, oh * ow, ops._p(out), ops._p(d_out),
                                                ops._p(loss), ops._stream()), "mft_ce_pool_backward")
    else:
        d_out = arena.get(tag + ".dout", (n, oh, ow, C))
        ops._lib.check(lib.mft_avgpool_relu_backward(ops._p(dfeat), ops._p(out), ops._p(d_out), n, oh * ow, C,
                                                     ops._stream()), "mft_avgpool_relu_backward")

    def bn_bwd(xraw, dy, mean, rstd, gamma, dgamma, dbeta, relu_out, name, need_dx=True):
        dx = arena.get(tag + "." + name, tuple(xraw.shape)) if need_dx else None
        rc = lib.mft_bn_backward(ops._p(xraw), C, ops._p(dy), C, ops._p(relu_out), C, ops._p(dx), C, C, rows, groups,
                                 ops._p(mean), ops._p(rstd), ops._p(gamma), C, ops._p(dgamma), ops._p(dbeta),
                                 ops._stream())
        ops._lib.check(rc, "mft_bn_backward")
# ... 311 lines not shown
```

meta-fine-tuning_amd/ops.py:

```python
import ctypes
import os

import torch

from . import _lib
from . import settings

ACT_NONE, ACT_RELU, ACT_LRELU = 0, 1, 2
BN_EPS = 1e-5
LRELU_SLOPE = 0.01


import threading

_tls = threading.local()


def _stream(t=None):
    dev = getattr(_tls, "dev", None)
    _tls.dev = None
    if t is not None:
        dev = t.device.index if torch.is_tensor(t) else (t.index if isinstance(t, torch.device) else int(t))
    return ctypes.c_void_p(torch.cuda.current_stream(dev).cuda_stream)

# ... 138 lines not shown


def conv2d(x, w_pk, Cout, KH, KW, stride, pad, imgs_per_group=0, bias=None, out=None):
    _f32c(x)
    n, H, W, Cin = x.shape
    OH = (H + 2 * pad - KH) // stride + 1
    OW = (W + 2 * pad - KW) // stride + 1
    if out is None:
        out = torch.empty((n, OH, OW, Cout), device=x.device, dtype=torch.float32)
    wgs = 0
    if w_pk.dim() == 3:
        wgs = w_pk.shape[1] * w_pk.shape[2]
        if imgs_per_group <= 0 or n // imgs_per_group != w_pk.shape[0]:
            raise RuntimeError("per-group weights need imgs_per_group with n/imgs_per_group == groups")
    if ((wgs == 0 and imgs_per_group <= 0) or (w_pk.dim() == 3 and w_pk.shape[0] == 1)) and Cin != 3:
        nws = _ksplit_ws(n * OH * OW, Cout, w_pk.shape[-1])
        if nws:
            ws = torch.empty((nws,), device=x.device, dtype=torch.float32)
            rc = _lib.lib().mft_conv2d_nhwc_ksplit(_p(x), Cin, _p(w_pk), _p(bias), _p(out), Cout, n, H, W, Cin, Cout, KH, KW,
                                                   stride, pad, _p(ws), _stream())
            _lib.check(rc, "mft_conv2d_nhwc_ksplit")
            return out
    if w_pk.dim() == 3 and 1 < w_pk.shape[0] <= SMALL_GROUPS and bias is None and Cin != 3:
        G = w_pk.shape[0]
        nws = _ksplit_ws(imgs_per_group * OH * OW, Cout, w_pk.shape[-1], G)
        if nws:
            ws = torch.empty((nws,), device=x.device, dtype=torch.float32)
            rc = _lib.lib().mft_conv2d_nhwc_ksplit_grouped(_p(x), Cin, _p(w_pk), _p(out), Cout, n, H, W, Cin, Cout, KH, KW, stride, pad,
                                                           imgs_per_group, wgs, _p(ws), _stream())
            _lib.check(rc, "mft_conv2d_nhwc_ksplit_grouped")
            return out
    rc = _lib.lib().mft_conv2d_nhwc(_p(x), Cin, _p(w_pk), _p(bias), _p(out), Cout, n, H, W, Cin, Cout, KH, KW,
                                    stride, pad, imgs_per_group, wgs, _stream())
    _lib.check(rc, "mft_conv2d_nhwc")
    return out


SMALL_GROUPS = settings.current().small_groups
_KSPLIT_WS = {}


def _ksplit_ws(rows, cols, K, groups=1):
    key = (rows, cols, K, groups)
    v = _KSPLIT_WS.get(key)
    if v is None:
        v = _KSPLIT_WS[key] = int(_lib.lib().mft_conv_ksplit_ws_floats(rows, cols, K) if groups == 1 else
                                  _lib.lib().mft_conv_ksplit_grouped_ws_floats(rows, cols, K, groups))
    return v


def split_weight_x3(w_pk):
    _f32c(w_pk)
    planes = torch.empty((3,) + tuple(w_pk.shape), device=w_pk.device, dtype=torch.int16)
    _lib.check(_lib.lib().mft_split_bf16x3(_p(w_pk), _p(planes), w_pk.numel(), _stream()), "mft_split_bf16x3")
    return planes


def split_weight_h2(w_pk):
    _f32c(w_pk)
    planes = torch.empty((2,) + tuple(w_pk.shape), device=w_pk.device, dtype=torch.int16)
    _lib.check(_lib.lib().mft_split_f16x2(_p(w_pk), _p(planes), w_pk.numel(), _stream()), "mft_split_f16x2")
    return planes


def _x3_fn(w3, stem):
    kind = {3: "x3", 2: "h2"}[int(w3.shape[0])]
    name = "mft_conv2d_nhwc_%s%s" % (kind, stem)
    return getattr(_lib.lib(), name), name


def conv2d_x3(x, w3, Cout, KH, KW, stride, pad, out=None):
    _f32c(x)
    n, H, W, Cin = x.shape
    OH = (H + 2 * pad - KH) // stride + 1
    OW = (W + 2 * pad - KW) // stride + 1
    if out is None:
        out = torch.empty((n, OH, OW, Cout), device=x.device, dtype=torch.float32)
    fn, name = _x3_fn(w3, "")
    rc = fn(_p(x), Cin, _p(w3), w3.shape[1] * w3.shape[2], _p(out), Cout, n, H, W, Cin, Cout, KH, KW, stride, pad, _stream())
    _lib.check(rc, name)
    return out


def conv2d_x3_bnstats(x, w3, Cout, KH, KW, stride, pad, imgs_per_group, out, ws, mean, rstd, eps=BN_EPS):
    _f32c(x)
    n, H, W, Cin = x.shape
    fn, name = _x3_fn(w3, "_bnstats")
    rc = fn(_p(x), Cin, _p(w3), w3.shape[1] * w3.shape[2], _p(out), Cout, n, H, W, Cin, Cout, KH, KW, stride, pad, imgs_per_group, eps,
            _p(ws), _p(mean), _p(rstd), _stream())
    if rc == _lib.MFT_EINVAL:
        return None
    _lib.check(rc, name)
    return out, mean, rstd


def conv2d_x3_bnin_bnstats(c_raw, in_ws, in_gamma, in_beta, w3, Cout, imgs_per_group, out, ws, mean=None, rstd=None, eps=BN_EPS):
    _f32c(c_raw)
    n, H, W, Cin = c_raw.shape
    fn, name = _x3_fn(w3, "_bnin_bnstats")
    rc = fn(_p(c_raw), Cin, _p(in_ws), _p(in_gamma), _p(in_beta), _p(w3), w3.shape[1] * w3.shape[2], _p(out), Cout, n, H, W, Cin, Cout,
            imgs_per_group, eps, _p(ws), _p(mean), _p(rstd), _stream())
    if rc == _lib.MFT_EINVAL:
        return None
    _lib.check(rc, name)
    return out


def bn_apply_x3ws(x2d, C, rows_per_group, n_groups, ws, gamma, beta, out, act=ACT_NONE, res=None, res_ws=None, res_gamma=None,
                  res_beta=None, slope=LRELU_SLOPE, eps=BN_EPS, stats=None, res_stats=None):
    _f32c(x2d)
    m, r = stats if stats is not None else (None, None)
    rm, rr = res_stats if res_stats is not None else (None, None)
    rc = _lib.lib().mft_bn_apply_x3ws(_p(x2d), x2d.shape[-1], _p(out), out.shape[-1], C, rows_per_group, n_groups, _p(ws), _p(gamma),
                                      _p(beta), _p(res), 0 if res is None else res.shape[-1], _p(res_ws), _p(res_gamma),
                                      _p(res_beta), act, slope, eps, _p(m), _p(r), _p(rm), _p(rr), _stream())
    _lib.check(rc, "mft_bn_apply_x3ws")
    return out


def conv2d_x3p_bnstats(xp, n, H, W, w3, Cout, KH, KW, stride, pad, imgs_per_group, out, ws, mean, rstd, eps=BN_EPS):
    Cin = xp.shape[2]
    if w3.shape[0] != 3:
        raise ValueError("pre-split activation planes exist for the bf16x3 kernels only")
    rc = _lib.lib().mft_conv2d_nhwc_x3p_bnstats(_p(xp), xp.shape[1] * Cin, Cin, _p(w3), w3.shape[1] * w3.shape[2], _p(out), Cout,
                                                n, H, W, Cin, Cout, KH, KW, stride, pad, imgs_per_group, eps, _p(ws), _p(mean),
                                                _p(rstd), _stream())
    _lib.check(rc, "mft_conv2d_nhwc_x3p_bnstats")
    return out, mean, rstd


def gemm(a, K, w_pk, N, bias=None, out=None, ldo=None, rows_per_group=0):
    _f32c(a)
    M, lda = a.shape
    if out is None:
        ldo = N if ldo is None else ldo
        out = torch.empty((M, ldo), device=a.device, dtype=torch.float32)
    else:
        ldo = out.shape[1]
    wgs = 0
    if w_pk.dim() == 3:
        wgs = w_pk.shape[1] * w_pk.shape[2]
    rc = _lib.lib().mft_conv2d_nhwc(_p(a), lda, _p(w_pk), _p(bias), _p(out), ldo, M, 1, 1, K, N, 1, 1, 1, 0,
                                    rows_per_group, wgs, _stream())
    _lib.check(rc, "mft_conv2d_nhwc(gemm)")
    return out


def gemm_rk(a, K, w_pk, N, bias=None, out=None, ldo=None):
    _f32c(a)
    M, lda = a.shape
    assert w_pk.dim() == 2 and w_pk.shape[1] == K and w_pk.shape[0] >= N and K % 16 == 0 and K <= 512, (tuple(w_pk.shape), K, N)
    if out is None:
        ldo = N if ldo is None else ldo
        out = torch.empty((M, ldo), device=a.device, dtype=torch.float32)
    else:
        ldo = out.shape[1]
    _lib.check(_lib.lib().mft_gemm_rk(_p(a), lda, _p(w_pk), w_pk.shape[0], K, _p(bias), _p(out), ldo, M, N, _stream()), "mft_gemm_rk")
    return out


def conv2d_dgrad(dy, w_pk, Cin, KH, KW, pad, imgs_per_group=0, out=None, stride=1, in_hw=None):
    _f32c(dy)
    n, OH, OW, Cout = dy.shape
    H, W = (OH, OW) if in_hw is None else in_hw
    if out is None:
        out = torch.empty((n, H, W, Cin), device=dy.device, dtype=torch.float32)
    wgs = w_pk.shape[1] * w_pk.shape[2] if w_pk.dim() == 3 else 0
    if ((wgs == 0 and imgs_per_group <= 0) or (w_pk.dim() == 3 and w_pk.shape[0] == 1)) and Cin % 64 == 0:
        nws = _ksplit_ws(n * H * W, Cin, KH * KW * Cout)
# ... 531 lines not shown
```

meta-fine-tuning_amd/settings.py:

```python
import dataclasses
import os


def _flag(v):
    lv = v.strip().lower()
    if lv in ("1", "true", "yes", "on"):
        return True
    if lv in ("0", "false", "no", "off"):
        return False
    raise ValueError("expected 0 / 1 (or true / false), got %r" % (v,))


def _opt_int(v):
    return None if v in ("", "none", "None") else int(v)


def _fuse(v):
    if v not in ("auto", "0", "1"):
        raise ValueError("expected auto, 0 or 1, got %r" % (v,))
    return v


KNOBS = (
    ("fuse_next", "MFT_FUSE_NEXT", _fuse, "auto", "fused weight-gradient + Adam + next-step forward launches: auto = engine.fuse_next_policy | 1 | 0"),
    ("wf_xcd", "MFT_WF_XCD", _flag, True, "fused launch: all workgroups of an episode on one XCD (A/B hook; read once per process)"),
    ("slab_candidates", "MFT_SLAB_CANDIDATES", _opt_int, None, "candidate buffers of the w/m/v placement scan (None: engine default 12; 0: off)"),
    ("slab_ballast_gb", "MFT_SLAB_BALLAST_GB", float, 12.0, "throw-away allocation between groups of placement candidates, GB"),
    ("slab_hints", "MFT_SLAB_HINTS", _flag, True, "re-use an earlier scan's placement when one probe confirms it"),
    ("trunk_chunk", "MFT_TRUNK_CHUNK", _opt_int, None, "inner steps per frozen-trunk launch set (None: 32 at E = 1, else 1)"),
    ("trunk_priority", "MFT_TRUNK_PRIORITY", int, 1, "HIP priority of the frozen-trunk stream (1 = the device's least)"),
    ("last_priority", "MFT_LAST_PRIORITY", int, -1, "torch priority of the last-block stream"),
    ("trunk_cus_per_xcd", "MFT_TRUNK_CUS_PER_XCD", int, 0, "CU-masked streams: CUs per XCD for the trunk stream (0 = no partition; measured slower)"),
    ("trunk_cus_only", "MFT_TRUNK_CUS_ONLY", _flag, False, "with trunk_cus_per_xcd: confine only the trunk stream"),
    ("debug_skip_trunk", "MFT_DEBUG_SKIP_TRUNK", _flag, False, "measurement aid: reuse one cached trunk output (results are WRONG)"),
    ("adapt_graph", "MFT_ADAPT_GRAPH", _flag, True, "adapt_last_block: replay the meta-fine-tuning inner loop from one hipGraph"),
    ("adapt_batched_trunk", "MFT_ADAPT_BATCHED_TRUNK", _flag, True, "adapt_last_block: frozen trunk of all steps as two grouped passes"),
    ("fused_dgrad", "MFT_FUSED_DGRAD", _flag, False, "one-pass trunk.7.C2 weight gradient + Adam + data gradient (measured slower in the step)"),
    ("x3_planes", "MFT_X3_PLANES", _flag, False, "trunk activations pre-split into bf16x3 planes (measured slower)"),
    ("x3_fused_stats", "MFT_X3_FUSED_STATS", _flag, True, "BatchNorm statistics from the split-precision convolution epilogue"),
    ("x3_fold_bn", "MFT_X3_FOLD_BN", _flag, True, "frozen blocks without helper launches (per-tile partials merged by the consumers)"),
    ("trunk_f16x2", "MFT_TRUNK_F16X2", _flag, True, "frozen trunk.4-6 on two fp16 pieces per operand (0: three bf16 pieces)"),
    ("fuse_next_c2_only", "MFT_FUSE_NEXT_C2_ONLY", _flag, False, "only trunk.7.C2's launch fused (measured slower)"),
    ("stem_pooled", "MFT_STEM_POOLED", _flag, True, "stem cache keeps per-window (max, min) instead of the full-resolution output"),
    ("stem_fused_fill", "MFT_STEM_FUSED_FILL", _flag, True, "stem cache filled by ONE launch (convolution + moments + window min/max; 0: three launches through a full-resolution buffer)"),
    ("stem_chunk", "MFT_STEM_CHUNK", _opt_int, None, "images per stem-cache fill launch (None: StemCache's default)"),
    ("fused_last_block", "MFT_FUSED_LAST_BLOCK", _flag, True, "conv + BatchNorm fusions of the adapted block (csrc/skinny.hip)"),
    ("small_groups", "MFT_SMALL_GROUPS", int, 12, "up to this many per-episode weight sets take the K-sliced GEMM route"),
    ("fused_pair_mlp", "MFT_FUSED_PAIR_MLP", _flag, True, "Wcompute on the fused upper-triangle pair-MLP kernels"),
    ("pair_mlp_gb", "MFT_PAIR_MLP_GB", float, 6.0, "memory budget of the fused pair-MLP's hidden activations per chunk, GB"),
    ("train_graph", "MFT_TRAIN_GRAPH", _flag, True, "MetaTemplate episode loop: loss + backward replayed from one hipGraph"),
    ("train_x3", "MFT_TRAIN_X3", _flag, True, "meta-training: 3x3 layers with >= 8192 output rows on the bf16x3 kernels, forward and stride-1 data gradient (0: fp32 MFMA everywhere)"),
    ("train_x3_min_rows", "MFT_TRAIN_X3_MIN_ROWS", int, 6000, "meta-training: output rows from which a 3x3 layer takes the bf16x3 kernels (below: fp32 MFMA with K slices; measured at 3,780 / 945 rows in profiles/r06_q_train_x3_min_rows.txt)"),
    ("wgrad_batch", "MFT_WGRAD_BATCH", _flag, True, "meta-training backward: every layer's weight gradient deferred to the end of the pass and run in one multi-problem launch pair per 16 layers (0: one launch pair per layer, as round 5; bit-identical)"),
    ("pair_f16x2", "MFT_PAIR_F16X2", _flag, False, "GNN pair-MLP layers (Wcompute) as f16x2 products on the fp16 matrix cores (fp32-accurate; 0: fp32 MFMA)"),
    ("gemm_rk_rows", "MFT_GEMM_RK_ROWS", int, 4096, "meta-training: head linear layers (fc, Gconv.fc) of at most this many rows take the skinny register-K GEMM (0: the tile kernel always)"),
    ("pair_rk_rows", "MFT_PAIR_RK_ROWS", int, 16384, "meta-training: Wcompute layers over at most this many pair rows (all episodes of the step) take the register-K small-problem kernel, 32-row tiles, no LDS staging (0: the 128-row tile kernel always)"),
    ("train_source", "MFT_TRAIN_SOURCE", str, "pool", "train.main --dataset miniImageNet: 'pool' = resident uint8 class pool, 'synthetic' = host fp32 episodes"),
    ("standin_weights", "MFT_STANDIN_WEIGHTS", _flag, False, "allow synthetic stand-in weights when no checkpoint is found (explicit opt-in)"),
    ("image_size", "MFT_IMAGE_SIZE", int, 84, "image side the CLI evaluates at (84 = BASELINE; 224 = the reference's)"),
    ("episodes", "MFT_EPISODES", _opt_int, None, "override of the CLI's episode count (None: 600)"),
    ("episodes_per_batch", "MFT_EPISODES_PER_BATCH", _opt_int, None, "override of the CLI's lockstep batch (None: 128 / 96 / 64 by n_shot)"),
    ("timings", "MFT_TIMINGS", _flag, False, "print the drivers' phase timings to stderr"),
    ("pool_per_class", "MFT_POOL_PER_CLASS", _opt_int, None, "images per class of the dataset-shaped resident pool (None: the dataset's)"),
    ("synth_on_host", "MFT_SYNTH_ON_HOST", _flag, False, "generate synthetic test episodes with numpy on the host instead of on the device"),
    ("balance_batches", "MFT_BALANCE_BATCHES", _flag, True, "equalise the lockstep batch sizes of an evaluation"),
    ("force_collectives", "MFT_FORCE_COLLECTIVES", _flag, False, "run the N-rank collectives even with one rank (1-GPU RCCL tests)"),
    ("one_device", "MFT_ONE_DEVICE", _flag, False, "test hook: W ranks share device 0, gloo for the gathers"),
)


@dataclasses.dataclass(frozen=True)
class Settings:
    fuse_next: str = "auto"
    wf_xcd: bool = True
    slab_candidates: "int | None" = None
    slab_ballast_gb: float = 12.0
    slab_hints: bool = True
    trunk_chunk: "int | None" = None
    trunk_priority: int = 1
    last_priority: int = -1
    trunk_cus_per_xcd: int = 0
    trunk_cus_only: bool = False
    debug_skip_trunk: bool = False
    adapt_graph: bool = True
    adapt_batched_trunk: bool = True
    fused_dgrad: bool = False
    x3_planes: bool = False
    x3_fused_stats: bool = True
    x3_fold_bn: bool = True
    trunk_f16x2: bool = True
    fuse_next_c2_only: bool = False
    stem_pooled: bool = True
    stem_fused_fill: bool = True
    stem_chunk: "int | None" = None
    fused_last_block: bool = True
    small_groups: int = 12
    fused_pair_mlp: bool = True
    pair_mlp_gb: float = 6.0
    train_graph: bool = True
    train_x3: bool = True
    train_x3_min_rows: int = 6000
    wgrad_batch: bool = True
    pair_f16x2: bool = False
    gemm_rk_rows: int = 4096
    pair_rk_rows: int = 16384
    train_source: str = "pool"
    standin_weights: bool = False
    image_size: int = 84
    episodes: "int | None" = None
    episodes_per_batch: "int | None" = None
    timings: bool = False
    pool_per_class: "int | None" = None
    synth_on_host: bool = False
    balance_batches: bool = True
    force_collectives: bool = False
    one_device: bool = False

    @classmethod
    def from_env(cls, env=None):
        env = os.environ if env is None else env
        kw = {}
        for field, var, parse, default, _ in KNOBS:
            raw = env.get(var)
            if raw is None:
                kw[field] = default
                continue
            try:
                kw[field] = parse(raw)
            except (TypeError, ValueError) as e:
                raise ValueError("%s=%r: %s" % (var, raw, e)) from None
        s = cls(**kw)
        if s.train_source not in ("pool", "synthetic"):
            raise ValueError("MFT_TRAIN_SOURCE=%r: expected pool or synthetic" % (s.train_source,))
        if s.image_size < 32 or not 0 <= s.trunk_cus_per_xcd < 32:
            raise ValueError("MFT_IMAGE_SIZE / MFT_TRUNK_CUS_PER_XCD out of range")
        return s


assert tuple(f.name for f in dataclasses.fields(Settings)) == tuple(k[0] for k in KNOBS), "KNOBS and Settings fields must match"
_VARS = tuple(k[1] for k in KNOBS)
_cache = (None, None)


def current():
    global _cache
    key = tuple(os.environ.get(v) for v in _VARS)
    if _cache[0] != key:
        _cache = (key, Settings.from_env())
    return _cache[1]


IMPORT_TIME = frozenset((
    "debug_skip_trunk", "adapt_graph", "adapt_batched_trunk", "fused_dgrad", "fused_last_block", "x3_planes", "x3_fused_stats",
    "x3_fold_bn", "trunk_f16x2", "train_x3", "train_x3_min_rows", "fuse_next_c2_only", "fused_pair_mlp", "pair_f16x2", "pair_rk_rows", "gemm_rk_rows", "pair_mlp_gb", "wgrad_batch",
    "train_graph", "small_groups", "wf_xcd",
))
assert IMPORT_TIME <= set(k[0] for k in KNOBS), IMPORT_TIME - set(k[0] for k in KNOBS)


def describe():
    return "\n".join("%-26s %-22s %-7s default %-8r %s" % (var, field, "import" if field in IMPORT_TIME else "live", default, doc)
                     for field, var, _, default, doc in KNOBS)
```

Baseline: 89.53.

## Fuse pooled-stem BN-ReLU gather into trunk.4 C1 loader and pair shortcut with C1

Adds a STEM variant of the stride-1 split-precision conv kernel. For trunk.4.C1 it reads the pooled max/min stem cache directly, combines per-image moments in LDS and applies BN+ReLU in the loader, so the separate gather launch and its activation round trip are no longer needed first. It also adds a pair kernel that runs the 1x1 shortcut and C1 of downsampling blocks in one launch. The aim is fewer launches and less memory traffic, at the cost of more complex loader code and register pressure. Both paths are on by default behind new import-time flags.

```diff
diff --git a/include/mft_hip.h b/include/mft_hip.h
--- a/include/mft_hip.h
+++ b/include/mft_hip.h
@@ -101,6 +101,10 @@
                                     const unsigned short* w2, long long plane_elems, float* out, int ldo, int n_img, int H, int W,
                                     int Cin, int Cout, int imgs_per_group, float eps, float* stats_ws, float* mean, float* rstd,
                                     void* stream);
+int mft_conv2d_x3_next_stem(const float* pmax, const float* pmin, int n_slots, const int* src_idx, const float* mean_img,
+                            const float* m2_img, int rows_per_img, const float* gamma, const float* beta, float* act);
+int mft_conv2d_x3_next_companion(const unsigned short* w, long long plane_elems, float* out, int ldo, int KH, int KW, int stride,
+                                 int pad, float* stats_ws);
 int mft_bn_apply_x3ws(const float* x, int ldx, float* y, int ldy, int C, int rows_per_group, int n_groups, const float* ws,
                       const float* gamma, const float* beta, const float* res, int ldr, const float* res_ws,
                       const float* res_gamma, const float* res_beta, int act, float slope, float eps, float* mean, float* rstd,
diff --git a/meta-fine-tuning_amd/_lib.py b/meta-fine-tuning_amd/_lib.py
--- a/meta-fine-tuning_amd/_lib.py
+++ b/meta-fine-tuning_amd/_lib.py
@@ -89,6 +89,8 @@
     "mft_conv2d_nhwc_x3_bnin_bnstats": [_P, _I, _P, _P, _P, _P, _L, _P, _I, _I, _I, _I, _I, _I, _I, _F, _P, _P, _P, _P],
     "mft_split_f16x2": [_P, _P, _L, _P],
     "mft_conv2d_nhwc_h2": [_P, _I, _P, _L, _P, _I, _I, _I, _I, _I, _I, _I, _I, _I, _I, _P],
+    "mft_conv2d_x3_next_stem": [_P, _P, _I, _P, _P, _P, _I, _P, _P, _P],
+    "mft_conv2d_x3_next_companion": [_P, _L, _P, _I, _I, _I, _I, _I, _P],
     "mft_conv2d_nhwc_h2_bnstats": [_P, _I, _P, _L, _P, _I, _I, _I, _I, _I, _I, _I, _I, _I, _I, _I, _F, _P, _P, _P, _P],
     "mft_conv2d_nhwc_h2_bnin_bnstats": [_P, _I, _P, _P, _P, _P, _L, _P, _I, _I, _I, _I, _I, _I, _I, _F, _P, _P, _P, _P],
     "mft_bn_apply_x3ws": [_P, _I, _P, _I, _I, _I, _I, _P, _P, _P, _P, _I, _P, _P, _P, _I, _F, _F, _P, _P, _P, _P, _P],
diff --git a/meta-fine-tuning_amd/csrc/bn.hip b/meta-fine-tuning_amd/csrc/bn.hip
--- a/meta-fine-tuning_amd/csrc/bn.hip
+++ b/meta-fine-tuning_amd/csrc/bn.hip
@@ -475,34 +475,11 @@
     }
 }
 
-template <class MeanOf, class M2Of>
-__device__ __forceinline__ void combine_moments_impl(MeanOf mean_of, M2Of m2_of, int rows_per_img, int imgs_per_group, float eps,
-                                                     float& mean, float& rstd) {
-    float mu = 0.f;
-    for (int i = 0; i < imgs_per_group; ++i) mu += mean_of(i);
-    mu /= (float)imgs_per_group;
-    float m2 = 0.f, dev = 0.f;
-    for (int i = 0; i < imgs_per_group; ++i) {
-        const float d = mean_of(i) - mu;
-        m2 += m2_of(i);
-        dev += d * d;
-    }
-    const float var = (m2 + (float)rows_per_img * dev) / ((float)rows_per_img * (float)imgs_per_group);
-    mean = mu;
-    rstd = 1.0f / sqrtf(var + eps);
-}
-
 __device__ __forceinline__ void combine_moments(const float* __restrict__ mean_img, const float* __restrict__ m2_img,
                                                 const int* __restrict__ id, int C, int c, int rows_per_img, int imgs_per_group,
                                                 float eps, float& mean, float& rstd) {
-    combine_moments_impl([&](int i) { return mean_img[(long long)id[i] * C + c]; },
+    mft_combine_moments_impl([&](int i) { return mean_img[(long long)id[i] * C + c]; },
                          [&](int i) { return m2_img[(long long)id[i] * C + c]; }, rows_per_img, imgs_per_group, eps, mean, rstd);
-}
-
-__device__ __forceinline__ void combine_moments_lds(const float* smean, const float* sm2, int C, int c, int rows_per_img,
-                                                    int imgs_per_group, float eps, float& mean, float& rstd) {
-    combine_moments_impl([&](int i) { return smean[i * C + c]; }, [&](int i) { return sm2[i * C + c]; }, rows_per_img,
-                         imgs_per_group, eps, mean, rstd);
 }
 
 __global__ void bn_combine_moments_kernel(const float* __restrict__ mean_img, const float* __restrict__ m2_img,
@@ -868,20 +845,12 @@
 
 __device__ __forceinline__ f32x4 pooled_bn_relu(const float* __restrict__ pmax, const float* __restrict__ pmin, long long src,
                                                 const f32x4 mu, const f32x4 rs, const f32x4 ga, const f32x4 be) {
-    const bool all_pos = ga[0] >= 0.f && ga[1] >= 0.f && ga[2] >= 0.f && ga[3] >= 0.f;
-    const bool all_neg = ga[0] < 0.f && ga[1] < 0.f && ga[2] < 0.f && ga[3] < 0.f;
+    const int sign = mft_pooled_sign4(ga);
     f32x4 v;
-    if (all_pos) v = *(const f32x4*)(pmax + src);
-    else if (all_neg) v = *(const f32x4*)(pmin + src);
-    else {
-        const f32x4 a = *(const f32x4*)(pmax + src), b = *(const f32x4*)(pmin + src);
-#pragma unroll
-        for (int e = 0; e < 4; ++e) v[e] = ga[e] >= 0.f ? a[e] : b[e];
-    }
-    f32x4 o = __builtin_elementwise_fma((v - mu) * rs, ga, be);
-#pragma unroll
-    for (int e = 0; e < 4; ++e) o[e] = fmaxf(o[e], 0.f);
-    return o;
+    if (sign > 0) v = *(const f32x4*)(pmax + src);
+    else if (sign < 0) v = *(const f32x4*)(pmin + src);
+    else v = mft_pooled_select4(*(const f32x4*)(pmax + src), *(const f32x4*)(pmin + src), ga);
+    return mft_pooled_bn_relu4(v, mu, rs, ga, be);
 }
 
 __global__ __launch_bounds__(256) void bn_relu_pooled_gather_kernel(const float* __restrict__ pmax, const float* __restrict__ pmin,
@@ -922,7 +891,7 @@
     __syncthreads();
     for (int c = threadIdx.x; c < C; c += 256) {
         float mu, rs;
-        combine_moments_lds(smean, sm2, C, c, rows_per_img, imgs_per_group, eps, mu, rs);
+        mft_combine_moments_lds(smean, sm2, C, c, rows_per_img, imgs_per_group, eps, mu, rs);
         tab[c] = mu; tab[C + c] = rs;
         if (blockIdx.x == 0 && mean) { mean[(long long)g * C + c] = mu; rstd[(long long)g * C + c] = rs; }
     }
diff --git a/meta-fine-tuning_amd/csrc/bn_fold.h b/meta-fine-tuning_amd/csrc/bn_fold.h
--- a/meta-fine-tuning_amd/csrc/bn_fold.h
+++ b/meta-fine-tuning_amd/csrc/bn_fold.h
@@ -89,3 +89,46 @@
     scale = rstd * gamma;
     shift = __builtin_elementwise_fma(-mean, scale, beta);
 }
+
+template <class MeanOf, class M2Of>
+__device__ __forceinline__ void mft_combine_moments_impl(MeanOf mean_of, M2Of m2_of, int rows_per_img, int imgs_per_group, float eps,
+                                                         float& mean, float& rstd) {
+    float mu = 0.f;
+    for (int i = 0; i < imgs_per_group; ++i) mu += mean_of(i);
+    mu /= (float)imgs_per_group;
+    float m2 = 0.f, dev = 0.f;
+    for (int i = 0; i < imgs_per_group; ++i) {
+        const float d = mean_of(i) - mu;
+        m2 += m2_of(i);
+        dev += d * d;
+    }
+    const float var = (m2 + (float)rows_per_img * dev) / ((float)rows_per_img * (float)imgs_per_group);
+    mean = mu;
+    rstd = 1.0f / sqrtf(var + eps);
+}
+
+__device__ __forceinline__ void mft_combine_moments_lds(const float* smean, const float* sm2, int C, int c, int rows_per_img,
+                                                        int imgs_per_group, float eps, float& mean, float& rstd) {
+    mft_combine_moments_impl([&](int i) { return smean[i * C + c]; }, [&](int i) { return sm2[i * C + c]; }, rows_per_img,
+                             imgs_per_group, eps, mean, rstd);
+}
+
+__device__ __forceinline__ int mft_pooled_sign4(const f32x4 ga) {
+    const bool all_pos = ga[0] >= 0.f && ga[1] >= 0.f && ga[2] >= 0.f && ga[3] >= 0.f;
+    const bool all_neg = ga[0] < 0.f && ga[1] < 0.f && ga[2] < 0.f && ga[3] < 0.f;
+    return all_pos ? 1 : (all_neg ? -1 : 0);
+}
+
+__device__ __forceinline__ f32x4 mft_pooled_select4(const f32x4 a, const f32x4 b, const f32x4 ga) {
+    f32x4 v;
+#pragma unroll
+    for (int e = 0; e < 4; ++e) v[e] = ga[e] >= 0.f ? a[e] : b[e];
+    return v;
+}
+
+__device__ __forceinline__ f32x4 mft_pooled_bn_relu4(const f32x4 v, const f32x4 mu, const f32x4 rs, const f32x4 ga, const f32x4 be) {
+    f32x4 o = __builtin_elementwise_fma((v - mu) * rs, ga, be);
+#pragma unroll
+    for (int e = 0; e < 4; ++e) o[e] = fmaxf(o[e], 0.f);
+    return o;
+}
diff --git a/meta-fine-tuning_amd/csrc/conv_x3.hip b/meta-fine-tuning_amd/csrc/conv_x3.hip
--- a/meta-fine-tuning_amd/csrc/conv_x3.hip
+++ b/meta-fine-tuning_amd/csrc/conv_x3.hip
@@ -32,6 +32,10 @@
     const float* bn_ws; const float* bn_gamma; const float* bn_beta;
     float bn_eps;
     int bn_max_tiles;
+    const float* st_base; unsigned st_bytes; int st_max_off, st_min_off;
+    const int* st_idx; const float* st_mean_img; const float* st_m2_img;
+    int st_rows_per_img, st_ipg;
+    float* st_act; unsigned st_act_bytes;
 };
 
 constexpr int X3_RS = 40;
@@ -69,7 +73,7 @@
 constexpr float X3_H2_LO_SCALE = 1.0f / 2048.f;
 
 template <int BM, int BN, bool AP, bool DB, int HOIST = 0, int DBG = 0, bool XS = false, int NP = 3>
-__global__ __launch_bounds__(256) __attribute__((amdgpu_waves_per_eu(NP == 2 ? 3 : 1))) void conv_x3_kernel(X3Args p) {
+__device__ __forceinline__ void conv_x3_body(const X3Args& p, int tile_id, const int nwg) {
     static_assert(NP == 3 || (NP == 2 && !AP && !DB && HOIST == 0 && DBG == 0 && !XS), "f16x2: the plain single-buffer form only");
     constexpr int NACC = NP == 3 ? 1 : 2;
     constexpr int TM = BM / 64;
@@ -93,9 +97,8 @@
     const int wm = wave >> 1, wn = wave & 1;
     const int r = lane & 31, h = lane >> 5;
     const bool g_swz = !XS && p.row_swz != 0;
-    int tile_id = blockIdx.x;
     if (p.xcd_swizzle) {
-        const int nwg = gridDim.x, q = nwg >> 3, rmd = nwg & 7;
+        const int q = nwg >> 3, rmd = nwg & 7;
         const int xcd = tile_id & 7, slot = tile_id >> 3;
         tile_id = xcd * q + (xcd < rmd ? xcd : rmd) + slot;
     }
@@ -429,13 +432,27 @@
     }
 }
 
+template <int BM, int BN, bool AP, bool DB, int HOIST = 0, int DBG = 0, bool XS = false, int NP = 3>
+__global__ __launch_bounds__(256) __attribute__((amdgpu_waves_per_eu(NP == 2 ? 3 : 1))) void conv_x3_kernel(X3Args p) {
+    conv_x3_body<BM, BN, AP, DB, HOIST, DBG, XS, NP>(p, blockIdx.x, gridDim.x);
+}
+
+template <int BM, int BN, int NP>
+__global__ __launch_bounds__(256) __attribute__((amdgpu_waves_per_eu(NP == 2 ? 3 : 1))) void conv_x3_pair_kernel(X3Args p0, X3Args p1,
+                                                                                                              int tiles0) {
+    const int b = blockIdx.x;
+    if (b < tiles0) conv_x3_body<BM, BN, false, false, 0, 0, false, NP>(p0, b, tiles0);
+    else conv_x3_body<BM, BN, false, false, 0, 0, false, NP>(p1, b - tiles0, (int)gridDim.x - tiles0);
+}
+
 #ifdef MFT_EXPERIMENTS
 #include "../../tools/experiments/conv_x3_pingpong.inc"
 #endif
 
-template <int BM, int BN, bool BNIN, int NP = 3, bool BDB = true>
+template <int BM, int BN, bool BNIN, int NP = 3, bool BDB = true, bool STEM = false>
 __device__ __forceinline__ void conv_x3_s1_body(const X3Args& p) {
     static_assert(NP == 3 || NP == 2, "3 bf16 pieces (six products) or 2 fp16 pieces (three products)");
+    static_assert(!(BNIN && STEM), "one loader-side BatchNorm");
     constexpr int NACC = NP == 3 ? 1 : 2;
     constexpr int TM = BM / 64, TN = BN / 64;
     constexpr int PA = BM / 32, PB = BN / 64;
@@ -463,8 +480,8 @@
     const int m0 = mt * BM, n0 = nt * BN;
     const int W = p.W, H = p.H;
     const int fr0 = m0 / W;
-    const int g0 = BNIN ? m0 / p.rows_per_group : 0;
-    const bool bn_two = BNIN && (m0 + (BM < p.M - m0 ? BM : p.M - m0) - 1) / p.rows_per_group > g0;
+    const int g0 = (BNIN || STEM) ? m0 / p.rows_per_group : 0;
+    const bool bn_two = (BNIN || STEM) && (m0 + (BM < p.M - m0 ? BM : p.M - m0) - 1) / p.rows_per_group > g0;
     if constexpr (BNIN) {
         char* stage = reinterpret_cast<char*>(smem);
         const size_t gstride = mft_x3_stage_bytes(p.bn_max_tiles, p.Cin);
@@ -484,11 +501,44 @@
         }
         __syncthreads();
     }
+    if constexpr (STEM) {
+        const int C = p.Cin, ipg = p.st_ipg;
+        float* smean = reinterpret_cast<float*>(smem);
+        float* sm2 = smean + 2 * ipg * C;
+        const int* id = p.st_idx + (long long)g0 * ipg;
+        const int n_stage = (bn_two ? 2 : 1) * ipg * C;
+        for (int i = tid; i < n_stage; i += 256) {
+            const int im = i / C, c = i - im * C;
+            const long long src = (long long)id[im] * C + c;
+            smean[i] = p.st_mean_img[src];
+            sm2[i] = p.st_m2_img[src];
+        }
+        __syncthreads();
+        for (int i = tid; i < 2 * C; i += 256) {
+            const int gi = i >= C ? 1 : 0, c = i - gi * C;
+            if (gi == 0 || bn_two) {
+                float mu, rs;
+                mft_combine_moments_lds(smean + gi * ipg * C, sm2 + gi * ipg * C, C, c, p.st_rows_per_img, ipg, p.bn_eps, mu, rs);
+                bn_tab[(gi * 2 + 0) * C + c] = mu;
+                bn_tab[(gi * 2 + 1) * C + c] = rs;
+            }
+        }
+        for (int i = tid; i < C; i += 256) {
+            bn_tab[4 * C + i] = p.bn_gamma[i];
+            bn_tab[5 * C + i] = p.bn_beta[i];
+        }
+        __syncthreads();
+    }
     const int g_id = tid >> 5, g_rr = (tid >> 3) & 3;
     const int lrow = p.row_swz ? g_rr * 4 + (g_id & 3) + 16 * (g_id >> 2) : tid >> 3;
     const int c4 = (tid & 7) * 4;
-    const __amdgpu_buffer_rsrc_t rA = __builtin_amdgcn_make_buffer_rsrc((void*)p.in, 0, p.in_bytes, 0x00020000);
+    const __amdgpu_buffer_rsrc_t rA = STEM ? __builtin_amdgcn_make_buffer_rsrc((void*)p.st_base, 0, p.st_bytes, 0x00020000)
+                                           : __builtin_amdgcn_make_buffer_rsrc((void*)p.in, 0, p.in_bytes, 0x00020000);
     const __amdgpu_buffer_rsrc_t rB = __builtin_amdgcn_make_buffer_rsrc((void*)p.w3, 0, p.w_bytes, 0x00020000);
+    auto stem_row = [&](int m) -> int {
+        const int hw = H * W, n = m / hw;
+        return p.st_idx[n] * hw + (m - n * hw);
+    };
     int a_off[PA], a_oh[PA], a_lds[PA], a_tab[PA];
     bool a_ok[PA];
 #pragma unroll
@@ -497,18 +547,29 @@
         const int fr = m / W;
         a_ok[j] = m < p.M;
         a_oh[j] = fr - (fr / H) * H;
-        a_off[j] = ((a_ok[j] ? m : 0) * p.ldi + c4) * 4;
+        if constexpr (STEM) a_off[j] = ((a_ok[j] ? stem_row(m) : 0) * p.ldi + c4) * 4;
+        else a_off[j] = ((a_ok[j] ? m : 0) * p.ldi + c4) * 4;
         a_lds[j] = (t + 1) * RS + c4;
         a_tab[j] = BNIN ? ((a_ok[j] ? m / p.rows_per_group - g0 : 0) * 2 * p.Cin + c4) : 0;
     }
+    unsigned st_ok = 0;
+    if constexpr (STEM) {
+#pragma unroll
+        for (int kh = 0; kh < 3; ++kh)
+#pragma unroll
+            for (int j = 0; j < PA; ++j) st_ok |= (a_ok[j] && (unsigned)(a_oh[j] + kh - 1) < (unsigned)H) ? 1u << (kh * 8 + j) : 0u;
+    }
+    const int st_split = STEM ? (g0 + 1) * p.rows_per_group - m0 - lrow : 0;
+    const __amdgpu_buffer_rsrc_t rAct = __builtin_amdgcn_make_buffer_rsrc((void*)p.st_act, 0, STEM ? p.st_act_bytes : 0, 0x00020000);
+    const int act_off = ((m0 + lrow) * p.Cin + c4) * 4;
     const int hside = (tid >> 3) & 1;
     const int mh = hside ? m0 + BM : m0 - 1;
     const int frh = (mh > 0 ? mh : 0) / W;
     const bool h_ok = tid < 16 && (hside ? (mh < p.M && mh - frh * W != 0) : (m0 > 0 && m0 - fr0 * W != 0));
     const int h_oh = frh - (frh / H) * H;
-    const int h_off = ((h_ok ? mh : 0) * p.ldi + c4) * 4;
+    const int h_off = ((h_ok ? (STEM ? stem_row(mh) : mh) : 0) * p.ldi + c4) * 4;
     const int h_lds = (hside ? BM + 1 : 0) * RS + c4;
-    const int h_tab = BNIN ? (((hside && h_ok) ? (m0 + BM - 1) / p.rows_per_group - g0 : 0) * 2 * p.Cin + c4) : 0;
+    const int h_tab = (BNIN || STEM) ? (((hside && h_ok) ? (m0 + BM - 1) / p.rows_per_group - g0 : 0) * 2 * p.Cin + c4) : 0;
 
     const int bseg = tid & 3;
     const int brow = p.row_swz ? ((tid >> 2) & 3) * 4 + ((tid >> 4) & 3) + 16 * (tid >> 6) : tid >> 2;
@@ -553,6 +614,32 @@
     auto load_a = [&](int ms, Stage& S) {
         const int kh = ms / n_ci, ci0 = (ms - kh * n_ci) * 32;
         const int shift = ((kh - 1) * W * p.ldi + ci0) * 4;
+        if constexpr (STEM) {
+            const f32x4 ga = *(const f32x4*)(bn_tab + 4 * p.Cin + ci0 + c4);
+            const int sg = mft_pooled_sign4(ga);
+            const bool okh = h_ok && (unsigned)(h_oh + kh - 1) < (unsigned)H;
+            if (sg != 0) {
+                const int pl = shift + (sg > 0 ? p.st_max_off : p.st_min_off);
+#pragma unroll
+                for (int j = 0; j < PA; ++j) {
+                    const bool ok = a_ok[j] && (unsigned)(a_oh[j] + kh - 1) < (unsigned)H;
+                    S.ra[j] = __builtin_bit_cast(f32x4, __builtin_amdgcn_raw_buffer_load_b128(rA, ok ? (unsigned)(a_off[j] + pl) : 0x80000000u, 0, 0));
+                }
+                S.rh = __builtin_bit_cast(f32x4, __builtin_amdgcn_raw_buffer_load_b128(rA, okh ? (unsigned)(h_off + pl) : 0x80000000u, 0, 0));
+            } else {
+#pragma unroll
+                for (int e = 0; e < 4; ++e) {
+                    const int pl = shift + 4 * e + (ga[e] >= 0.f ? p.st_max_off : p.st_min_off);
+#pragma unroll
+                    for (int j = 0; j < PA; ++j) {
+                        const bool ok = a_ok[j] && (unsigned)(a_oh[j] + kh - 1) < (unsigned)H;
+                        S.ra[j][e] = __builtin_bit_cast(float, __builtin_amdgcn_raw_buffer_load_b32(rA, ok ? (unsigned)(a_off[j] + pl) : 0x80000000u, 0, 0));
+                    }
+                    S.rh[e] = __builtin_bit_cast(float, __builtin_amdgcn_raw_buffer_load_b32(rA, okh ? (unsigned)(h_off + pl) : 0x80000000u, 0, 0));
+                }
+            }
+            return;
+        }
 #pragma unroll
         for (int j = 0; j < PA; ++j) {
             const bool ok = a_ok[j] && (unsigned)(a_oh[j] + kh - 1) < (unsigned)H;
@@ -591,7 +678,27 @@
         return o;
     };
     auto store_a = [&](const Stage& S, int ms) {
-        if constexpr (BNIN) {
+        if constexpr (STEM) {
+            const int kh = ms / n_ci, ci0 = (ms - kh * n_ci) * 32, C = p.Cin;
+            const bool okh = h_ok && (unsigned)(h_oh + kh - 1) < (unsigned)H;
+            auto act = [&](const f32x4 v, int tab, bool ok) {
+                const f32x4 ga = *(const f32x4*)(bn_tab + 4 * C + ci0 + c4), be = *(const f32x4*)(bn_tab + 5 * C + ci0 + c4);
+                f32x4 o = mft_pooled_bn_relu4(v, *(const f32x4*)(bn_tab + tab + ci0), *(const f32x4*)(bn_tab + tab + C + ci0), ga, be);
+#pragma unroll
+                for (int e = 0; e < 4; ++e) o[e] = ok ? o[e] : 0.f;
+                return o;
+            };
+            const bool wr = kh == 1 && nt == 0 && p.st_act_bytes != 0;
+#pragma unroll
+            for (int j = 0; j < PA; ++j) {
+                const f32x4 o = act(S.ra[j], (bn_two && 32 * j >= st_split) ? 2 * C + c4 : c4, a_ok[j] && (unsigned)(a_oh[j] + kh - 1) < (unsigned)H);
+                put_a(o, a_lds[j]);
+                if (wr)
+                    __builtin_amdgcn_raw_buffer_store_b128(__builtin_bit_cast(u32x4, o), rAct, a_ok[j] ? (unsigned)act_off : 0x80000000u,
+                                                           (32 * j * C + ci0) * 4, 0);
+            }
+            if (tid < 16) put_a(act(S.rh, bn_two ? h_tab : c4, okh), h_lds);
+        } else if constexpr (BNIN) {
             const int kh = ms / n_ci, ci0 = (ms - kh * n_ci) * 32;
             const bool okh = h_ok && (unsigned)(h_oh + kh - 1) < (unsigned)H;
             if (!bn_two) {
@@ -787,6 +894,11 @@
     conv_x3_s1_body<BM, BN, true, NP, BDB>(p);
 }
 
+template <int BM, int BN, int NP = 3, bool BDB = true>
+__global__ __launch_bounds__(256) __attribute__((amdgpu_waves_per_eu(3, 3))) void conv_x3_s1_stem_kernel(X3Args p) {
+    conv_x3_s1_body<BM, BN, false, NP, BDB, true>(p);
+}
+
 __global__ void x3_stats_finalize_kernel(const float* __restrict__ ws, int C, int M, int R, int BM, float eps,
                                          float* __restrict__ mean, float* __restrict__ rstd) {
     const int c = blockIdx.x * blockDim.x + threadIdx.x;
@@ -858,6 +970,19 @@
 int g_x3_row_swz = 1;
 int g_x3_xcd = 1;
 int g_x3_min_lds_kb = 0;
+
+template <int BM, int BN>
+int launch_x3_pair(X3Args p0, X3Args p1, hipStream_t s, int np) {
+    const int tiles_m = (p0.M + BM - 1) / BM;
+    p0.tiles_n = p1.tiles_n = p0.Cout / BN;
+    p0.xcd_swizzle = p1.xcd_swizzle = g_x3_xcd;
+    p0.row_swz = p1.row_swz = np == 2 ? (g_x3_row_swz != 0) : g_x3_row_swz;
+    const int tiles0 = tiles_m * p0.tiles_n;
+    const size_t lds = (size_t)np * (BM + BN) * X3_RS * sizeof(unsigned short);
+    if (np == 2) hipLaunchKernelGGL((conv_x3_pair_kernel<BM, BN, 2>), dim3((unsigned)(2 * tiles0)), dim3(256), lds, s, p0, p1, tiles0);
+    else hipLaunchKernelGGL((conv_x3_pair_kernel<BM, BN, 3>), dim3((unsigned)(2 * tiles0)), dim3(256), lds, s, p0, p1, tiles0);
+    return mft_launch_status();
+}
 
 template <int BM, int BN, bool AP, bool DB>
 int launch_x3(X3Args p, hipStream_t s, int np = 3) {
@@ -924,9 +1049,10 @@
 
 int g_x3_bdb = 1;
 
-inline size_t x3_s1_lds(int BM, int BN, int W, int bn_cin, int np = 3) {
+inline size_t x3_s1_lds(int BM, int BN, int W, int bn_cin, int np = 3, int tab_rows = 4) {
     (void)W;
-    return (size_t)np * (BM + 18 + ((np == 2 && g_x3_bdb) ? 2 : 1) * BN) * X3_RS * sizeof(unsigned short) + (size_t)4 * bn_cin * sizeof(float);
+    return (size_t)np * (BM + 18 + ((np == 2 && g_x3_bdb) ? 2 : 1) * BN) * X3_RS * sizeof(unsigned short) +
+           (size_t)tab_rows * bn_cin * sizeof(float);
 }
 
 template <int BM, int BN>
@@ -936,9 +1062,13 @@
     p.xcd_swizzle = g_x3_xcd;
     p.row_swz = g_x3_row_swz != 0;
     p.s1_rows = BM + 18;
-    const size_t lds = x3_s1_lds(BM, BN, p.W, p.bn_ws ? p.Cin : 0, np);
+    const size_t lds = p.st_base ? x3_s1_lds(BM, BN, p.W, p.Cin, np, 6) : x3_s1_lds(BM, BN, p.W, p.bn_ws ? p.Cin : 0, np);
     const dim3 grid((unsigned)(tiles_m * p.tiles_n));
-    if (np == 2 && g_x3_bdb) {
+    if (p.st_base) {
+        if (np == 2 && g_x3_bdb) hipLaunchKernelGGL((conv_x3_s1_stem_kernel<BM, BN, 2, true>), grid, dim3(256), lds, s, p);
+        else if (np == 2) hipLaunchKernelGGL((conv_x3_s1_stem_kernel<BM, BN, 2, false>), grid, dim3(256), lds, s, p);
+        else hipLaunchKernelGGL((conv_x3_s1_stem_kernel<BM, BN>), grid, dim3(256), lds, s, p);
+    } else if (np == 2 && g_x3_bdb) {
         if (p.bn_ws) hipLaunchKernelGGL((conv_x3_s1_bnin_kernel<BM, BN, 2, true>), grid, dim3(256), lds, s, p);
         else hipLaunchKernelGGL((conv_x3_s1_kernel<BM, BN, 2, true>), grid, dim3(256), lds, s, p);
     } else if (np == 2) {
@@ -1018,16 +1148,31 @@
     return 0;
 }
 
+struct X3Stem {
+    bool set = false;
+    const float* pmax; const float* pmin; const int* idx; const float* mean_img; const float* m2_img;
+    int n_slots, rows_per_img; const float* gamma; const float* beta; float* act;
+};
+struct X3Companion {
+    bool set = false;
+    const unsigned short* w; long long plane; float* out; int ldo, KH, KW, stride, pad; float* stats_ws;
+};
+static thread_local X3Stem t_x3_stem;
+static thread_local X3Companion t_x3_comp;
+
 static int x3_dispatch(const float* in, int ldi, const unsigned short* w3, long long plane_elems, float* out, int ldo,
                        int n_img, int H, int W, int Cin, int Cout, int KH, int KW, int stride, int pad, float* stats_ws,
                        int rows_per_group, void* stream, const unsigned short* in3 = nullptr, long long in_plane_elems = 0,
                        const float* bn_ws = nullptr, const float* bn_gamma = nullptr, const float* bn_beta = nullptr,
-                       float bn_eps = 0.f, int np = 3) {
+                       float bn_eps = 0.f, int np = 3, const X3Stem* stem = nullptr, int imgs_per_group = 0,
+                       const X3Companion* comp = nullptr) {
     if (n_img <= 0 || Cin % 32 != 0 || Cout % 64 != 0 || ldi % 4 != 0 || (np != 3 && np != 2)) return MFT_EINVAL;
     if (np == 2 && (in3 != nullptr || g_x3_tile > 1 || g_x3_db || g_x3_pp || g_x3_dbg || g_x3_hoist || g_x3_row_swz == 2 || g_x3_min_lds_kb ||
                     g_x3_patch))
         return MFT_EINVAL;
     X3Args p;
+    p.st_base = nullptr; p.st_bytes = 0; p.st_max_off = p.st_min_off = 0; p.st_idx = nullptr; p.st_mean_img = p.st_m2_img = nullptr;
+    p.st_rows_per_img = p.st_ipg = 0; p.st_act = nullptr; p.st_act_bytes = 0;
     p.bn_ws = bn_ws; p.bn_gamma = bn_gamma; p.bn_beta = bn_beta; p.bn_eps = bn_eps;
     p.bn_max_tiles = bn_ws ? mft_x3_max_group_tiles(rows_per_group, 128) : 0;
     if (bn_ws != nullptr && (in3 != nullptr || !bn_gamma || !bn_beta || rows_per_group < 128 || KH != 3 || KW != 3 || stride != 1 ||
@@ -1051,6 +1196,31 @@
     hipStream_t s = (hipStream_t)stream;
     int G = 0, R = 0;
     double eff = 0.0;
+    if (stem != nullptr) {
+        const bool s1 = g_x3_s1 && g_x3_tile <= 1 && KH == 3 && KW == 3 && stride == 1 && pad == 1 && !g_x3_db && !g_x3_pp && !g_x3_dbg &&
+                        g_x3_hoist == 0 && g_x3_row_swz != 2 && g_x3_min_lds_kb == 0;
+        if (!s1 || comp != nullptr || bn_ws != nullptr || stats_ws == nullptr || rows_per_group < 128 || imgs_per_group < 1 || ldi != Cin ||
+            Cin % 4 != 0 || !stem->pmax || !stem->pmin || !stem->idx || !stem->mean_img || !stem->m2_img || !stem->gamma || !stem->beta ||
+            stem->rows_per_img < 1 || x3_s1_lds(128, 64, W, Cin, np, 6) > X3_S1_LDS_3PER_CU ||
+            (size_t)4 * imgs_per_group * Cin * sizeof(float) > (size_t)np * (128 + 18) * X3_RS * sizeof(unsigned short) ||
+            np * plane_elems * 2 >= 0x7fff0000LL || M * Cin * 4 >= 0x7fff0000LL)
+            return MFT_EINVAL;
+        const char* lo = (const char*)(stem->pmax < stem->pmin ? stem->pmax : stem->pmin);
+        const char* hi = (const char*)(stem->pmax < stem->pmin ? stem->pmin : stem->pmax);
+        const long long gap = hi - lo, half = (long long)stem->n_slots * H * W * Cin * 4;
+        if (stem->n_slots < 1 || gap < half || gap + half >= 0x7fff0000LL) return MFT_EINVAL;
+        p.st_base = (const float*)lo;
+        p.st_bytes = (unsigned)(gap + half);
+        p.st_max_off = stem->pmax < stem->pmin ? 0 : (int)gap;
+        p.st_min_off = stem->pmax < stem->pmin ? (int)gap : 0;
+        p.st_idx = stem->idx; p.st_mean_img = stem->mean_img; p.st_m2_img = stem->m2_img;
+        p.st_rows_per_img = stem->rows_per_img; p.st_ipg = imgs_per_group; p.st_act = stem->act;
+        p.st_act_bytes = stem->act ? (unsigned)(M * Cin * 4) : 0u;
+        p.bn_gamma = stem->gamma; p.bn_beta = stem->beta; p.bn_eps = bn_eps;
+        p.in = nullptr; p.in_bytes = 0;
+        p.w_bytes = (unsigned)(np * plane_elems * 2);
+        return launch_x3_s1<128, 64>(p, s, np);
+    }
     if (in3 != nullptr) {
         const long long need = (long long)n_img * H * W * ldi;
         if (ldi % 8 != 0 || in_plane_elems < need || 3 * in_plane_elems * 2 >= 0x7fff0000LL || 3 * plane_elems * 2 >= 0x7fff0000LL)
@@ -1106,6 +1276,20 @@
                         g_x3_hoist == 0 && g_x3_row_swz != 2 && g_x3_min_lds_kb == 0 &&
                         x3_s1_lds(128, 64, W, 0, np) <= 64 * 1024;
         if (bn_ws != nullptr && !s1) return MFT_EINVAL;
+        if (comp != nullptr) {
+            const int OH2 = (H + 2 * comp->pad - comp->KH) / comp->stride + 1, OW2 = (W + 2 * comp->pad - comp->KW) / comp->stride + 1;
+            if (s1 || tile != 1 || g_x3_db || g_x3_pp || g_x3_dbg || g_x3_hoist || g_x3_row_swz == 2 || g_x3_min_lds_kb || ni != n_img ||
+                stats_ws == nullptr || comp->stats_ws == nullptr || !comp->w || !comp->out || OH2 != p.OH || OW2 != p.OW ||
+                np * comp->plane * 2 >= 0x7fff0000LL)
+                return MFT_EINVAL;
+            X3Args q2 = q;
+            q2.w3 = comp->w; q2.plane = comp->plane; q2.out = comp->out; q2.ldo = comp->ldo;
+            q2.KH = comp->KH; q2.KW = comp->KW; q2.stride = comp->stride; q2.pad = comp->pad;
+            q2.Kpad = comp->KH * comp->KW * Cin;
+            q2.w_bytes = (unsigned)(np * comp->plane * 2);
+            q2.stats_ws = comp->stats_ws;
+            return launch_x3_pair<128, 64>(q, q2, s, np);
+        }
         const int rc = s1 ? launch_x3_s1<128, 64>(q, s, np)
                        : np == 2 ? launch_x3<128, 64, false, false>(q, s, 2)
                        : (tile == 2 && Cout % 128 == 0) ? launch_x3<128, 128, false, false>(q, s)
@@ -1150,17 +1334,41 @@
                       float* out, int ldo, int n_img, int H, int W, int Cin, int Cout, int KH, int KW,
                       int stride, int pad, int imgs_per_group, float eps, float* stats_ws,
                       float* mean, float* rstd, void* stream) {
+    const X3Stem stem = t_x3_stem;
+    const X3Companion comp = t_x3_comp;
+    t_x3_stem.set = t_x3_comp.set = false;
     if (imgs_per_group <= 0 || n_img % imgs_per_group != 0 || stats_ws == nullptr) return MFT_EINVAL;
     const int OH = (H + 2 * pad - KH) / stride + 1, OW = (W + 2 * pad - KW) / stride + 1;
     const int R = imgs_per_group * OH * OW;
+    if ((stem.set || comp.set) && (mean != nullptr || rstd != nullptr || g_x3_tile == 3)) return MFT_EINVAL;
     const int rc = x3_dispatch(in, ldi, w3, plane_elems, out, ldo, n_img, H, W, Cin, Cout, KH, KW, stride, pad, stats_ws, R,
-                               stream, nullptr, 0, nullptr, nullptr, nullptr, 0.f, np);
+                               stream, nullptr, 0, nullptr, nullptr, nullptr, eps, np, stem.set ? &stem : nullptr, imgs_per_group,
+                               comp.set ? &comp : nullptr);
     if (rc != 0) return rc;
     if (mean == nullptr && rstd == nullptr) return g_x3_tile == 3 ? MFT_EINVAL : 0;
     const int groups = n_img / imgs_per_group;
     hipLaunchKernelGGL(x3_stats_finalize_kernel, dim3((Cout + 63) / 64, groups), dim3(64), 0, (hipStream_t)stream,
                        (const float*)stats_ws, Cout, n_img * OH * OW, R, g_x3_tile == 3 ? 64 : 128, eps, mean, rstd);
     return mft_launch_status();
+}
+
+extern "C" int mft_conv2d_x3_next_stem(const float* pmax, const float* pmin, int n_slots, const int* src_idx, const float* mean_img,
+                                       const float* m2_img, int rows_per_img, const float* gamma, const float* beta, float* act) {
+    if (!pmax || !pmin || n_slots < 1 || !src_idx || !mean_img || !m2_img || !gamma || !beta || rows_per_img < 1) return MFT_EINVAL;
+    t_x3_stem.set = true;
+    t_x3_stem.n_slots = n_slots;
+    t_x3_stem.pmax = pmax; t_x3_stem.pmin = pmin; t_x3_stem.idx = src_idx; t_x3_stem.mean_img = mean_img; t_x3_stem.m2_img = m2_img;
+    t_x3_stem.rows_per_img = rows_per_img; t_x3_stem.gamma = gamma; t_x3_stem.beta = beta; t_x3_stem.act = act;
+    return 0;
+}
+
+extern "C" int mft_conv2d_x3_next_companion(const unsigned short* w, long long plane_elems, float* out, int ldo, int KH, int KW,
+                                            int stride, int pad, float* stats_ws) {
+    if (!w || !out || !stats_ws || plane_elems <= 0) return MFT_EINVAL;
+    t_x3_comp.set = true;
+    t_x3_comp.w = w; t_x3_comp.plane = plane_elems; t_x3_comp.out = out; t_x3_comp.ldo = ldo;
+    t_x3_comp.KH = KH; t_x3_comp.KW = KW; t_x3_comp.stride = stride; t_x3_comp.pad = pad; t_x3_comp.stats_ws = stats_ws;
+    return 0;
 }
 
 extern "C" int mft_conv2d_nhwc_x3_bnstats(const float* in, int ldi, const unsigned short* w3, long long plane_elems,
diff --git a/meta-fine-tuning_amd/functional.py b/meta-fine-tuning_amd/functional.py
--- a/meta-fine-tuning_amd/functional.py
+++ b/meta-fine-tuning_amd/functional.py
@@ -12,6 +12,8 @@
 X3_PLANES = settings.current().x3_planes
 X3_FUSED_STATS = settings.current().x3_fused_stats
 X3_FOLD_BN = settings.current().x3_fold_bn
+X3_STEM_C1 = settings.current().x3_stem_c1
+X3_PAIR_SHORTCUT = settings.current().x3_pair_shortcut
 TRUNK_F16X2 = settings.current().trunk_f16x2
 TRAIN_X3 = settings.current().train_x3
 TRAIN_X3_MIN_ROWS = settings.current().train_x3_min_rows
@@ -258,8 +260,8 @@
         if self.pooled:
             self.c0 = None
             self._buf = None if self.fused_fill else torch.empty((self.chunk, self.OH, self.OH, 64), device=device)
-            self.pmax = torch.empty((n_slots, self.PH, self.PH, 64), device=device)
-            self.pmin = torch.empty((n_slots, self.PH, self.PH, 64), device=device)
+            self._pm = torch.empty((2, n_slots, self.PH, self.PH, 64), device=device)
+            self.pmax, self.pmin = self._pm[0], self._pm[1]
         else:
             self.c0 = torch.empty((n_slots, self.OH, self.OH, 64), device=device)
 
@@ -356,7 +358,15 @@
                 _, ap = r
                 OHb = (shape[1] + 2 - 3) // stride + 1
                 shape = (n, OHb, OHb, cout)
-        if fold:
+        a, first = None, 4
+        if (fold and X3_STEM_C1 and X3_FUSED_STATS and upto > 4 and ipg * PH * PH >= 128
+                and all(("trunk.4" + nm) in W.planes("trunk.4", ipg, PH) for nm in (".C1", ".C2"))):
+            a = _frozen_block_folded(W, "trunk.4", None, arena, ipg, 64, 64, 1, tag + ".trunk.4",
+                                     stem=(cache, idx, g, b, arena.get(tag + ".p0", (n, PH, PH, 64))))
+            first = 5 if a is not None else 4
+        if a is not None:
+            pass
+        elif fold:
             a = cache.gather_moments(idx, n, g, b, ipg, arena.get(tag + ".p0", (n, PH, PH, 64)))
         else:
             a = cache.gather(idx, n, m, s, g, b, ipg, arena.get(tag + ".p0", (n, PH, PH, 64)))
@@ -366,9 +376,12 @@
         c0 = ops.conv2d(x, W.conv["trunk.0"], 64, 7, 7, 2, 3, out=arena.get(tag + ".c0", (n, (x.shape[1] + 6 - 7) // 2 + 1, (x.shape[2] + 6 - 7) // 2 + 1, 64)))
         m, s = _bn_stats4(arena, tag + ".bn0", c0, ipg, groups, run("trunk.1"), fix("trunk.1"))
         a = ops.bn_relu_maxpool(c0, m, s, g, b, imgs_per_group=ipg)
+        first = 4
     for idx in (4, 5, 6, 7):
         if idx >= upto:
             break
+        if idx < first:
+            continue
         cin, cout, stride = STAGES[idx]
         p = "trunk.%d" % idx
         a = simple_block(W, p, a, arena, ipg, cin, cout, stride, running, tag + "." + p, fixed=fixed)
@@ -537,8 +550,13 @@
 _X3WS_FITS = {}
 
 
-def _frozen_block_folded(W, p, x, arena, ipg, cin, cout, stride, tag):
-    n, H, _, _ = x.shape
+def _frozen_block_folded(W, p, x, arena, ipg, cin, cout, stride, tag, stem=None):
+    if stem is not None:
+        cache, sidx, sg, sb, sact = stem
+        xshape = (sidx.numel(), cache.PH, cache.PH, cin)
+    else:
+        xshape = tuple(x.shape)
+    n, H = xshape[0], xshape[1]
     groups = n // ipg
     OH = (H + 2 - 3) // stride + 1
     rows = ipg * OH * OH
@@ -551,13 +569,29 @@
     (g1, b1), (g2, b2) = W.bn[p + ".BN1"], W.bn[p + ".BN2"]
     w3 = W.conv3
 
+    def statws(stag, k, s, pd):
+        return arena.get(stag + ".statws", (int(lib.mft_conv2d_x3_stats_ws_floats(n, H, H, cout, k, k, s, pd)),))
+
     def partials(name, inp, k, s, pd, obuf, stag):
-        ws = arena.get(stag + ".statws", (int(lib.mft_conv2d_x3_stats_ws_floats(n, inp.shape[1], inp.shape[1], cout, k, k, s, pd)),))
-        r = ops.conv2d_x3_bnstats(inp, w3[p + name], cout, k, k, s, pd, ipg, obuf, ws, None, None)
+        ws = statws(stag, k, s, pd)
+        r = ops.conv2d_x3_bnstats(inp, w3[p + name], cout, k, k, s, pd, ipg, obuf, ws, None, None, xshape=xshape)
         return None if r is None else ws
 
     c1 = arena.get(tag + ".c1", (n, OH, OH, cout))
-    ws1 = partials(".C1", x, 3, stride, 1, c1, tag + ".bn1")
+    ws1 = wss = None
+    if stem is not None:
+        ops.conv2d_x3_next_stem(cache.pmax, cache.pmin, sidx, cache.mean, cache.m2, cache.OH * cache.OH, sg, sb, sact)
+        ws1 = partials(".C1", None, 3, stride, 1, c1, tag + ".bn1")
+        x = sact
+    elif cin != cout and X3_PAIR_SHORTCUT:
+        sc = arena.get(tag + ".sc", (n, OH, OH, cout))
+        wss = statws(tag + ".bns", 1, stride, 0)
+        ops.conv2d_x3_next_companion(w3[p + ".shortcut"], sc, 1, 1, stride, 0, wss)
+        ws1 = partials(".C1", x, 3, stride, 1, c1, tag + ".bn1")
+        if ws1 is None:
+            wss = None
+    if ws1 is None and stem is None:
+        ws1 = partials(".C1", x, 3, stride, 1, c1, tag + ".bn1")
     if ws1 is None:
         return None
     c2 = arena.get(tag + ".c2", (n, OH, OH, cout))
@@ -571,7 +605,8 @@
     if cin != cout:
         gs, bs = W.bn[p + ".BNshortcut"]
         sc = arena.get(tag + ".sc", (n, OH, OH, cout))
-        wss = partials(".shortcut", x, 1, stride, 0, sc, tag + ".bns")
+        if wss is None:
+            wss = partials(".shortcut", x, 1, stride, 0, sc, tag + ".bns")
         if wss is None:
             raise RuntimeError("frozen block %s: shortcut outside the bf16x3 domain after C1 was inside it" % p)
         ops.bn_apply_x3ws(c2.view(-1, cout), cout, rows, groups, ws2, g2, b2, out, act=ops.ACT_RELU, res=sc.view(-1, cout),
diff --git a/meta-fine-tuning_amd/ops.py b/meta-fine-tuning_amd/ops.py
--- a/meta-fine-tuning_amd/ops.py
+++ b/meta-fine-tuning_amd/ops.py
@@ -244,9 +244,20 @@
     return out
 
 
-def conv2d_x3_bnstats(x, w3, Cout, KH, KW, stride, pad, imgs_per_group, out, ws, mean, rstd, eps=BN_EPS):
-    _f32c(x)
-    n, H, W, Cin = x.shape
+def conv2d_x3_next_stem(pmax, pmin, idx, mean_img, m2_img, rows_per_img, gamma, beta, act):
+    _lib.check(_lib.lib().mft_conv2d_x3_next_stem(_p(pmax), _p(pmin), pmax.shape[0], _p(idx), _p(mean_img), _p(m2_img), rows_per_img,
+                                                  _p(gamma), _p(beta), _p(act)), "mft_conv2d_x3_next_stem")
+
+
+def conv2d_x3_next_companion(w3, out, KH, KW, stride, pad, ws):
+    _lib.check(_lib.lib().mft_conv2d_x3_next_companion(_p(w3), w3.shape[1] * w3.shape[2], _p(out), out.shape[-1], KH, KW, stride, pad,
+                                                       _p(ws)), "mft_conv2d_x3_next_companion")
+
+
+def conv2d_x3_bnstats(x, w3, Cout, KH, KW, stride, pad, imgs_per_group, out, ws, mean, rstd, eps=BN_EPS, xshape=None):
+    if x is not None:
+        _f32c(x)
+    n, H, W, Cin = x.shape if x is not None else xshape
     fn, name = _x3_fn(w3, "_bnstats")
     rc = fn(_p(x), Cin, _p(w3), w3.shape[1] * w3.shape[2], _p(out), Cout, n, H, W, Cin, Cout, KH, KW, stride, pad, imgs_per_group, eps,
             _p(ws), _p(mean), _p(rstd), _stream())
diff --git a/meta-fine-tuning_amd/settings.py b/meta-fine-tuning_amd/settings.py
--- a/meta-fine-tuning_amd/settings.py
+++ b/meta-fine-tuning_amd/settings.py
@@ -39,6 +39,8 @@
     ("x3_planes", "MFT_X3_PLANES", _flag, False, "trunk activations pre-split into bf16x3 planes (measured slower)"),
     ("x3_fused_stats", "MFT_X3_FUSED_STATS", _flag, True, "BatchNorm statistics from the split-precision convolution epilogue"),
     ("x3_fold_bn", "MFT_X3_FOLD_BN", _flag, True, "frozen blocks without helper launches (per-tile partials merged by the consumers)"),
+    ("x3_stem_c1", "MFT_X3_STEM_C1", _flag, True, "trunk.4.C1 reads the pooled stem cache in its own loader (0: the gather launch writes the activation first)"),
+    ("x3_pair_shortcut", "MFT_X3_PAIR_SHORTCUT", _flag, True, "C1 and the 1x1 shortcut of trunk.5 / trunk.6 in one launch (0: two launches; bit-identical)"),
     ("trunk_f16x2", "MFT_TRUNK_F16X2", _flag, True, "frozen trunk.4-6 on two fp16 pieces per operand (0: three bf16 pieces)"),
     ("fuse_next_c2_only", "MFT_FUSE_NEXT_C2_ONLY", _flag, False, "only trunk.7.C2's launch fused (measured slower)"),
     ("stem_pooled", "MFT_STEM_POOLED", _flag, True, "stem cache keeps per-window (max, min) instead of the full-resolution output"),
@@ -88,6 +90,8 @@
     x3_planes: bool = False
     x3_fused_stats: bool = True
     x3_fold_bn: bool = True
+    x3_stem_c1: bool = True
+    x3_pair_shortcut: bool = True
     trunk_f16x2: bool = True
     fuse_next_c2_only: bool = False
     stem_pooled: bool = True
@@ -152,7 +156,7 @@
 
 IMPORT_TIME = frozenset((
     "debug_skip_trunk", "adapt_graph", "adapt_batched_trunk", "fused_dgrad", "fused_last_block", "x3_planes", "x3_fused_stats",
-    "x3_fold_bn", "trunk_f16x2", "train_x3", "train_x3_min_rows", "fuse_next_c2_only", "fused_pair_mlp", "pair_f16x2", "pair_rk_rows", "gemm_rk_rows", "pair_mlp_gb", "wgrad_batch",
+    "x3_fold_bn", "x3_stem_c1", "x3_pair_shortcut", "trunk_f16x2", "train_x3", "train_x3_min_rows", "fuse_next_c2_only", "fused_pair_mlp", "pair_f16x2", "pair_rk_rows", "gemm_rk_rows", "pair_mlp_gb", "wgrad_batch",
     "train_graph", "small_groups", "wf_xcd",
 ))
 assert IMPORT_TIME <= set(k[0] for k in KNOBS), IMPORT_TIME - set(k[0] for k in KNOBS)
```

Result: no change. 90.41 (median of 6 runs) (+1.0%).
